# MKLab-ITI/gnn-tf

Measured on AMD Instinct MI355X. Metric: propagated edges/sec (APPNP K=10), higher is better.
Workload: dtype f32; 1 GPU; rmat_n80000000_nnz1000000000_C128_appnp_K10 (BASELINE config5); global_rows=80000000, stored_entries_total=1000000000, rows_per_rank=80000000, stored_entries_per_rank=1000000000, features=128, partition=none, kernel=spmm_group32

## Files before the change

gnn-tf_amd/csrc/gnx_gcnii.hip:

```cpp
#include "gnx_spmm_device.h"

namespace {

__device__ __forceinline__ uint64_t drop_stream(const DropFuse &f) { return f.stream + (f.offset ? *f.offset : 0); }

template <int VEC>
__device__ __forceinline__ void drop_values(const DropFuse &f, uint64_t stream, int64_t row, int64_t c, float (&x)[VEC]) {
#pragma unroll
    for (int v = 0; v < VEC; ++v)
        x[v] = (f.thr == 0 || hash_u24(f.seed, stream, (uint64_t)row, (uint64_t)(c + v), 0) >= f.thr) ? x[v] * f.scale : 0.f;
}

template <bool SPEC> struct SpectralArgs {};
template <> struct SpectralArgs<true> {
    const float *bias;
    uint32_t *gate;
};

template <bool EDGE> struct EdgeArgs {};
template <> struct EdgeArgs<true> {
    DropFuse feat;
};
template <bool EDGE>
__device__ __forceinline__ const DropFuse &feature_mask(const SpmmArgs &p, const EdgeArgs<EDGE> &ed) {
// ... 20 lines not shown
__device__ __forceinline__ void tile_times_Ms(float *__restrict__ T, const float *__restrict__ Ms, int lane, int act,
                                              const float *__restrict__ bias = nullptr) {
    constexpr int C = 16 * NT, STRIDE = C + 4;
    const int cc = lane & 15, g = lane >> 4;
    [[maybe_unused]] float bv[NT];
    if constexpr (BIAS) {
#pragma unroll
        for (int nt = 0; nt < NT; ++nt) bv[nt] = bias[16 * nt + cc];
    }
    f32x4 d[NT];
#pragma unroll
    for (int nt = 0; nt < NT; ++nt) d[nt] = f32x4{0.f, 0.f, 0.f, 0.f};
#pragma unroll 4
    for (int kk = 0; kk < C / 4; ++kk) {
        const float a = T[cc * STRIDE + 4 * kk + g];
        const float *__restrict__ mrow = Ms + (4 * kk + g) * STRIDE + cc;
#pragma unroll
        for (int nt = 0; nt < NT; ++nt) d[nt] = __builtin_amdgcn_mfma_f32_16x16x4f32(a, mrow[16 * nt], d[nt], 0, 0, 0);
    }
    __builtin_amdgcn_wave_barrier();
#pragma unroll
    for (int nt = 0; nt < NT; ++nt)
#pragma unroll
        for (int r = 0; r < 4; ++r) {
            float v = d[nt][r];
            if constexpr (BIAS) v += bv[nt];
            if (act == GNX_ACT_RELU) v = fmaxf(v, 0.f);
            T[(4 * g + r) * STRIDE + 16 * nt + cc] = v;
        }
    __builtin_amdgcn_wave_barrier();
}

template <bool ENTRIES, int G, int U>
__device__ __forceinline__ void edge_gather(const SpmmArgs &p, const float *__restrict__ Xc, int64_t row, int64_t beg, int64_t end,
                                            float (&acc)[4]) {
    static_assert(G % U == 0, "a round of G entries is whole batches of U");
    const int sub = (int)(threadIdx.x % G);
    for (int64_t base = beg; base < end; base += G) {
        int mycol = 0;
        float myw = 0.f;
        if (base + sub < end) {
            mycol = p.colidx[base + sub];
            myw = dropped_weight_at<ENTRIES>(p.fuse, p.vals[base + sub], base + sub, row, mycol);
        }
        const int n = (int)(end - base < G ? end - base : G);
        for (int k = 0; k < n; k += U) {
            float x[U][4];
            float w[U];
#pragma unroll
            for (int u = 0; u < U; ++u) {
                const int j = __shfl(mycol, k + u, G);
                w[u] = __shfl(myw, k + u, G);
                if (w[u] != 0.f) vload<4>(x[u], Xc + (int64_t)j * p.ldx);
                else {
#pragma unroll
                    for (int v = 0; v < 4; ++v) x[u][v] = 0.f;
                }
            }
#pragma unroll
            for (int u = 0; u < U; ++u)
#pragma unroll
                for (int v = 0; v < 4; ++v) acc[v] = fmaf(w[u], x[u][v], acc[v]);
        }
    }
}

template <typename R, int U, bool EDGE = false, bool ENTRIES = false, int G = 0>
__device__ __forceinline__ void mixed_row(const typename R::Args &p, int64_t row, int64_t beg, int64_t end, int c, float (&acc)[4]) {
    const typename R::Elem *__restrict__ Xc = R::X(p) + c;
    if constexpr (EDGE) {
        edge_gather<ENTRIES, G, U>(p, Xc, row, beg, end, acc);
    } else {
        for (int64_t e = beg; e < end; e += U) {
            float x[U][4];
            float w[U];
#pragma unroll
            for (int u = 0; u < U; ++u) {
                if (e + u < end) {
                    const int j = p.colidx[e + u];
                    w[u] = p.vals[e + u];
                    R::template load<4>(x[u], Xc + (int64_t)j * p.ldx);
                } else {
                    w[u] = 0.f;
#pragma unroll
                    for (int v = 0; v < 4; ++v) x[u][v] = 0.f;
                }
            }
#pragma unroll
            for (int u = 0; u < U; ++u)
#pragma unroll
                for (int v = 0; v < 4; ++v) acc[v] = fmaf(w[u], x[u][v], acc[v]);
        }
    }
    float h0[4];
    vload<4>(h0, p.H0 + row * p.ldh0 + c);
#pragma unroll
    for (int v = 0; v < 4; ++v) acc[v] = fmaf(acc[v], p.beta, h0[v] * p.alpha);
}

template <typename R, int NT, int U, int WPB, bool DROP = false, bool SPEC = false, bool EDGE = false, bool ENTRIES = false>
__global__ __launch_bounds__(64 * WPB) void k_spmm_gcnii(const typename R::Args p, const float *__restrict__ M, int64_t ldm, float *__restrict__ mixed,
                                                         const SpectralArgs<SPEC> sp = SpectralArgs<SPEC>{},
                                                         const EdgeArgs<EDGE> ed = EdgeArgs<EDGE>{}) {
    static_assert(!EDGE || (!SPEC && !R::BF16), "the edge-dropout form exists for the plain layer over f32 rows");
    constexpr int C = 16 * NT, G = 4 * NT, RPP = 64 / G, PASSES = 16 / RPP, STRIDE = C + 4;
    __shared__ float Ms[C * STRIDE];
    __shared__ float Ts[WPB][16 * STRIDE];
    const int lane = threadIdx.x & 63;
    const int wave = threadIdx.x >> 6;
    for (int idx = threadIdx.x; idx < C * C; idx += 64 * WPB) Ms[(idx / C) * STRIDE + idx % C] = M[(int64_t)(idx / C) * ldm + idx % C];
    __syncthreads();
    const int64_t tile = (int64_t)blockIdx.x * WPB + wave;
    if (tile * 16 >= p.n_rows) return;
    float *__restrict__ T = Ts[wave];
    const int sub = lane % G, c = sub * 4;
    int64_t rows[PASSES];
    bool live[PASSES];
#pragma unroll
    for (int ps = 0; ps < PASSES; ++ps) {
        const int rr = ps * RPP + lane / G;
        const int64_t slot = tile * 16 + rr;
        int64_t row = -1;
        int64_t beg = 0, end = 0;
        if (slot < p.n_rows) {
            row = p.row_order ? (int64_t)p.row_order[slot] : slot;
            beg = p.rowptr[row]; end = p.rowptr[row + 1];
        }
        live[ps] = row >= 0 && end - beg <= p.long_row;
        rows[ps] = row;
        float acc[4] = {0.f, 0.f, 0.f, 0.f};
        if (live[ps]) {
            mixed_row<R, U, EDGE, ENTRIES, G>(p, row, beg, end, c, acc);
            if (mixed) vstore<4>(mixed + row * (int64_t)C + c, acc);
        }
        vstore<4>(T + rr * STRIDE + c, acc);
    }
    __builtin_amdgcn_wave_barrier();
    if constexpr (SPEC) {
        constexpr int GW = G < 8 ? G : 8, WORDS = (C + 31) / 32;
        tile_times_Ms<NT, true>(T, Ms, lane, p.act, sp.bias);
        float b[4];
        vload<4>(b, sp.bias + c);
        uint64_t stream = 0;
        if constexpr (DROP) stream = drop_stream(p.fuse);
#pragma unroll
        for (int ps = 0; ps < PASSES; ++ps) {
            const int rr = ps * RPP + lane / G;
            float o[4];
            vload<4>(o, T + rr * STRIDE + c);
            uint32_t word = spectral_finish<4, DROP>(p.fuse, stream, rows[ps], c, b, o) << (c & 31);
#pragma unroll
            for (int m = 1; m < GW; m <<= 1) word |= (uint32_t)__shfl_xor((int)word, m);
            if (!live[ps]) continue;
            R::template store<4>(p, rows[ps] * p.ldo, c, o, false);
            if (sp.gate != nullptr && sub % GW == 0) sp.gate[rows[ps] * WORDS + (c >> 5)] = word;
        }
        return;
    }
    tile_times_Ms<NT>(T, Ms, lane, p.act);
#pragma unroll
    for (int ps = 0; ps < PASSES; ++ps) {
        if (!live[ps]) continue;
        const int rr = ps * RPP + lane / G;
        float o[4];
        vload<4>(o, T + rr * STRIDE + c);
        if constexpr (DROP) {
            const DropFuse &fd = feature_mask<EDGE>(p, ed);
            drop_values<4>(fd, drop_stream(fd), rows[ps], c, o);
        }
        R::template store<4>(p, rows[ps] * p.ldo, c, o, false);
    }
}

template <typename R, int NT, int U, int WPB, bool EDGE = false, bool ENTRIES = false>
__global__ __launch_bounds__(64 * WPB) void k_spmm_gcnii_back(const typename R::Args p, const float *__restrict__ N, int64_t ldn, const float *S_in,
                                                              float s_alpha, float *S_out) {
    static_assert(!EDGE || !R::BF16, "the edge-dropout form exists for f32 rows");
    constexpr int C = 16 * NT, G = 4 * NT, RPP = 64 / G, PASSES = 16 / RPP, STRIDE = C + 4;
    __shared__ float Ms[C * STRIDE];
    __shared__ float Ts[WPB][16 * STRIDE];
    const int lane = threadIdx.x & 63;
    const int wave = threadIdx.x >> 6;
    for (int idx = threadIdx.x; idx < C * C; idx += 64 * WPB) Ms[(idx / C) * STRIDE + idx % C] = N[(int64_t)(idx / C) * ldn + idx % C];
    __syncthreads();
    const int64_t tile = (int64_t)blockIdx.x * WPB + wave;
    if (tile * 16 >= p.n_rows) return;
    float *__restrict__ T = Ts[wave];
    const int sub = lane % G, c = sub * 4;
    int64_t rows[PASSES];
    bool live[PASSES];
#pragma unroll
    for (int ps = 0; ps < PASSES; ++ps) {
        const int rr = ps * RPP + lane / G;
        const int64_t slot = tile * 16 + rr;
        int64_t row = -1;
        int64_t beg = 0, end = 0;
        if (slot < p.n_rows) {
            row = p.row_order ? (int64_t)p.row_order[slot] : slot;
            beg = p.rowptr[row]; end = p.rowptr[row + 1];
        }
        live[ps] = row >= 0 && end - beg <= p.long_row;
        rows[ps] = row;
        float acc[4] = {0.f, 0.f, 0.f, 0.f};
        if (live[ps]) {
            const typename R::Elem *__restrict__ Xc;
            if constexpr (R::BF16) Xc = p.Xb + c;
            else Xc = p.X + c;
            if constexpr (EDGE) {
                edge_gather<ENTRIES, G, U>(p, Xc, row, beg, end, acc);
            } else {
                for (int64_t e = beg; e < end; e += U) {
                    float x[U][4];
                    float w[U];
#pragma unroll
                    for (int u = 0; u < U; ++u) {
                        if (e + u < end) {
                            const int j = p.colidx[e + u];
                            w[u] = p.vals[e + u];
                            if constexpr (R::BF16) bload<4>(x[u], Xc + (int64_t)j * p.ldx);
                            else vload<4>(x[u], Xc + (int64_t)j * p.ldx);
                        } else {
                            w[u] = 0.f;
#pragma unroll
                            for (int v = 0; v < 4; ++v) x[u][v] = 0.f;
                        }
                    }
#pragma unroll
                    for (int u = 0; u < U; ++u)
#pragma unroll
                        for (int v = 0; v < 4; ++v) acc[v] = fmaf(w[u], x[u][v], acc[v]);
                }
            }
#pragma unroll
            for (int v = 0; v < 4; ++v) acc[v] *= p.beta;
        }
        vstore<4>(T + rr * STRIDE + c, acc);
    }
    __builtin_amdgcn_wave_barrier();
    tile_times_Ms<NT>(T, Ms, lane, GNX_ACT_NONE);
#pragma unroll
    for (int ps = 0; ps < PASSES; ++ps) {
        if (!live[ps]) continue;
        const int rr = ps * RPP + lane / G;
        float o[4];
        vload<4>(o, T + rr * STRIDE + c);
        vstore<4>(p.out + rows[ps] * p.ldo + c, o);
    }
    if (S_out == nullptr) return;
    __builtin_amdgcn_wave_barrier();
#pragma unroll
    for (int ps = 0; ps < PASSES; ++ps) {
        const int rr = ps * RPP + lane / G;
        float x[4] = {0.f, 0.f, 0.f, 0.f};
        if (rows[ps] >= 0) {
            vload<4>(x, p.X + rows[ps] * p.ldx + c);
#pragma unroll
            for (int v = 0; v < 4; ++v) x[v] *= p.alpha;
        }
        vstore<4>(T + rr * STRIDE + c, x);
    }
    __builtin_amdgcn_wave_barrier();
    tile_times_Ms<NT>(T, Ms, lane, GNX_ACT_NONE);
#pragma unroll
    for (int ps = 0; ps < PASSES; ++ps) {
        if (rows[ps] < 0) continue;
        const int rr = ps * RPP + lane / G;
        const int64_t at = rows[ps] * (int64_t)C + c;
        float o[4];
        vload<4>(o, T + rr * STRIDE + c);
        if (S_in) {
            float s[4];
            vload<4>(s, S_in + at);
#pragma unroll
            for (int v = 0; v < 4; ++v) o[v] = fmaf(s_alpha, s[v], o[v]);
        }
        vstore<4>(S_out + at, o);
    }
}

template <typename R, int NT, int U, int WPB>
__global__ __launch_bounds__(64 * WPB) void k_gcnii_wgrad(const typename R::Args p, const float *__restrict__ Gm, const float *__restrict__ hub,
                                                          float *__restrict__ work) {
    constexpr int C = 16 * NT, G = 4 * NT, RPP = 64 / G, PASSES = 16 / RPP, STRIDE = C + 4;
    static_assert(WPB * 16 * STRIDE >= C * C, "the block's partial reuses the tiles");
    __shared__ __attribute__((aligned(16))) float Ts[WPB * 16 * STRIDE];
    const int lane = threadIdx.x & 63;
    const int wave = threadIdx.x >> 6;
    const int cc = lane & 15, g = lane >> 4, c = (lane % G) * 4;
    float *T = Ts + wave * 16 * STRIDE;
    f32x4 d[NT][NT];
#pragma unroll
    for (int mt = 0; mt < NT; ++mt)
#pragma unroll
        for (int nt = 0; nt < NT; ++nt) d[mt][nt] = f32x4{0.f, 0.f, 0.f, 0.f};
    const int64_t n_tiles = (p.n_rows + 15) / 16, step = (int64_t)gridDim.x * WPB;
    for (int64_t tile = (int64_t)blockIdx.x * WPB + wave; tile < n_tiles; tile += step) {
#pragma unroll
        for (int ps = 0; ps < PASSES; ++ps) {
            const int rr = ps * RPP + lane / G;
            const int64_t slot = tile * 16 + rr;
            float acc[4] = {0.f, 0.f, 0.f, 0.f};
            if (slot < p.n_rows) {
                const int64_t row = p.row_order ? (int64_t)p.row_order[slot] : slot;
                const int64_t beg = p.rowptr[row], end = p.rowptr[row + 1];
                if (end - beg <= p.long_row) mixed_row<R, U>(p, row, beg, end, c, acc);
                else vload<4>(acc, hub + row * (int64_t)C + c);
            }
            vstore<4>(T + rr * STRIDE + c, acc);
        }
        float b[4][NT];
#pragma unroll
        for (int kk = 0; kk < 4; ++kk) {
            const int64_t slot = tile * 16 + 4 * kk + g;
#pragma unroll
            for (int nt = 0; nt < NT; ++nt) b[kk][nt] = 0.f;
            if (slot < p.n_rows) {
                const int64_t row = p.row_order ? (int64_t)p.row_order[slot] : slot;
                vload<NT>(b[kk], Gm + row * (int64_t)C + NT * cc);
            }
        }
        __builtin_amdgcn_wave_barrier();
#pragma unroll
        for (int kk = 0; kk < 4; ++kk) {
// ... 721 lines not shown
```

gnn-tf_amd/csrc/gnx_graph.hip:

```cpp
#include <cstring>
#include <string.h>

#include "gnx_internal.h"
#include <algorithm>
#include <memory>
#include <type_traits>
#include <utility>

#include <rocprim/rocprim.hpp>

namespace gnx {

static thread_local char g_err[512] = "";

void set_error(const char *fmt, ...) {
    va_list ap;
    va_start(ap, fmt);
    vsnprintf(g_err, sizeof(g_err), fmt, ap);
    va_end(ap);
}

static unsigned bits_for(uint64_t max_key_exclusive) {
    unsigned b = 1;
    while (b < 64 && (max_key_exclusive >> b) != 0) ++b;
// ... 45 lines not shown
                                   int64_t *__restrict__ ptr) {
    int64_t r = (int64_t)blockIdx.x * blockDim.x + threadIdx.x;
    if (r > n_rows) return;
    int64_t lo = 0, hi = nnz;
    while (lo < hi) {
        int64_t mid = (lo + hi) >> 1;
        if ((int64_t)sorted_rows[mid] < r) lo = mid + 1; else hi = mid;
    }
    ptr[r] = lo;
}

__global__ void k_rows_from_ptr(const int64_t *__restrict__ rowptr, int64_t n_rows, int32_t *__restrict__ rowidx) {
    int64_t r = (int64_t)blockIdx.x * blockDim.x + threadIdx.x;
    if (r >= n_rows) return;
    for (int64_t e = rowptr[r]; e < rowptr[r + 1]; ++e) rowidx[e] = (int32_t)r;
}

__global__ void k_check_csr(const int64_t *__restrict__ rowptr, const int32_t *__restrict__ colidx, int64_t n_rows,
                            int64_t n_cols, int64_t nnz, int *__restrict__ bad) {
    int64_t r = (int64_t)blockIdx.x * blockDim.x + threadIdx.x;
    if (r >= n_rows) return;
    int64_t b = rowptr[r], e = rowptr[r + 1];
    if (b > e || b < 0 || e > nnz || (r == 0 && b != 0) || (r == n_rows - 1 && e != nnz)) { atomicExch(bad, 1); return; }
    for (int64_t k = b; k < e; ++k) {
        int32_t c = colidx[k];
        if (c < 0 || c >= n_cols || (k > b && colidx[k - 1] >= c)) { atomicExch(bad, 1); return; }
    }
}

__global__ void k_flag_long(const int64_t *__restrict__ rowptr, int64_t n_rows, int long_row, int long_chunk,
                            int32_t *__restrict__ flag, int64_t *__restrict__ cnt) {
    int64_t r = (int64_t)blockIdx.x * blockDim.x + threadIdx.x;
    if (r >= n_rows) return;
    int64_t d = rowptr[r + 1] - rowptr[r];
    bool lg = d > long_row;
    flag[r] = lg ? 1 : 0;
    cnt[r] = lg ? (d + long_chunk - 1) / long_chunk : 0;
}

__global__ void k_order_keys(const int64_t *__restrict__ rowptr, int64_t n_rows, int clamp, uint16_t *__restrict__ keys,
                             int32_t *__restrict__ ids) {
    int64_t r = (int64_t)blockIdx.x * blockDim.x + threadIdx.x;
    if (r >= n_rows) return;
    int64_t d = rowptr[r + 1] - rowptr[r];
    keys[r] = (uint16_t)(clamp - (d < clamp ? d : clamp));
    ids[r] = (int32_t)r;
}

__global__ void k_order_keys_windowed(const int64_t *__restrict__ rowptr, int64_t n_rows, int clamp, int64_t window, uint32_t n_windows,
                                      unsigned bin_bits, uint32_t *__restrict__ keys, int32_t *__restrict__ ids) {
    int64_t r = (int64_t)blockIdx.x * blockDim.x + threadIdx.x;
    if (r >= n_rows) return;
    int64_t d = rowptr[r + 1] - rowptr[r];
    const uint32_t w = d == 0 ? n_windows : (uint32_t)(r / window);
    keys[r] = (w << bin_bits) | (uint32_t)(clamp - (d < clamp ? d : clamp));
    ids[r] = (int32_t)r;
}

__global__ void k_slot_ptrs(const int64_t *__restrict__ rowptr, const int32_t *__restrict__ row_order, int64_t n_rows,
                            int64_t *__restrict__ slot_beg, int32_t *__restrict__ slot_cnt) {
    int64_t sidx = (int64_t)blockIdx.x * blockDim.x + threadIdx.x;
    if (sidx >= n_rows) return;
    const int64_t r = row_order[sidx], b = rowptr[r], e = rowptr[r + 1];
    slot_beg[sidx] = b;
    slot_cnt[sidx] = (int32_t)(e - b < 0x7fffffff ? e - b : 0x7fffffff);
}

__global__ void k_count_nonempty(const int64_t *__restrict__ rowptr, int64_t n_rows, unsigned long long *__restrict__ count) {
    int64_t r = (int64_t)blockIdx.x * blockDim.x + threadIdx.x;
    const bool has = r < n_rows && rowptr[r + 1] > rowptr[r];
    const unsigned long long votes = __popcll(__ballot(has));
    if ((threadIdx.x & 63) == 0 && votes) atomicAdd(count, votes);
}

__global__ void k_mark_referenced(const int32_t *__restrict__ colidx, int64_t nnz, uint8_t *__restrict__ flag) {
    int64_t k = (int64_t)blockIdx.x * blockDim.x + threadIdx.x;
    if (k < nnz) flag[colidx[k]] = 1;
}

__global__ void k_count_empty_referenced(const int64_t *__restrict__ rowptr, int64_t n, const uint8_t *__restrict__ flag, int *__restrict__ count) {
    int64_t r = (int64_t)blockIdx.x * blockDim.x + threadIdx.x;
    if (r < n && rowptr[r + 1] == rowptr[r] && flag[r]) atomicAdd(count, 1);
}

__global__ void k_fill_long(const int64_t *__restrict__ rowptr, int64_t n_rows, int long_row, int long_chunk,
                            const int32_t *__restrict__ pos,
                            const int64_t *__restrict__ cpos, int32_t *__restrict__ long_rows,
                            int64_t *__restrict__ long_chunk_ptr, int32_t *__restrict__ chunk_long) {
    int64_t r = (int64_t)blockIdx.x * blockDim.x + threadIdx.x;
    if (r >= n_rows) return;
    int64_t d = rowptr[r + 1] - rowptr[r];
    if (d <= long_row) return;
    const int32_t p = pos[r];
    const int64_t c0 = cpos[r];
    const int64_t nc = (d + long_chunk - 1) / long_chunk;
    long_rows[p] = (int32_t)r;
    long_chunk_ptr[p] = c0;
    for (int64_t c = 0; c < nc; ++c) chunk_long[c0 + c] = p;
}

__global__ void k_chunk_keys(const int64_t *__restrict__ rowptr, const int32_t *__restrict__ colidx,
                             const int32_t *__restrict__ long_rows, const int64_t *__restrict__ long_chunk_ptr,
                             const int32_t *__restrict__ chunk_long, int64_t n_chunks, int long_chunk,
                             uint32_t *__restrict__ keys, int32_t *__restrict__ ids) {
    int64_t c = (int64_t)blockIdx.x * blockDim.x + threadIdx.x;
    if (c >= n_chunks) return;
    const int32_t li = chunk_long[c];
    const int64_t beg = rowptr[long_rows[li]] + (c - long_chunk_ptr[li]) * long_chunk;
    keys[c] = (uint32_t)colidx[beg];
    ids[c] = (int32_t)c;
}

__global__ void k_make_tkeys(const int32_t *__restrict__ rowidx, const int32_t *__restrict__ colidx, int64_t nnz,
                             int64_t n_rows, uint64_t *__restrict__ keys, int32_t *__restrict__ payload) {
    int64_t k = (int64_t)blockIdx.x * blockDim.x + threadIdx.x;
    if (k >= nnz) return;
    keys[k] = (uint64_t)colidx[k] * (uint64_t)n_rows + (uint64_t)rowidx[k];
    payload[k] = (int32_t)k;
}

__global__ void k_invert_order(const int32_t *__restrict__ order, int64_t n, int32_t *__restrict__ newid) {
    int64_t i = (int64_t)blockIdx.x * blockDim.x + threadIdx.x;
    if (i < n) newid[order[i]] = (int32_t)i;
}

__global__ void k_make_rkeys(const int32_t *__restrict__ rowidx, const int32_t *__restrict__ colidx, const int32_t *__restrict__ newid,
                             int64_t nnz, int64_t n, uint64_t *__restrict__ keys, int32_t *__restrict__ payload) {
    int64_t k = (int64_t)blockIdx.x * blockDim.x + threadIdx.x;
    if (k >= nnz) return;
    keys[k] = (uint64_t)newid[rowidx[k]] * (uint64_t)n + (uint64_t)newid[colidx[k]];
    payload[k] = (int32_t)k;
}

__global__ void k_min_neighbour_rank(const int32_t *__restrict__ rowidx, const int32_t *__restrict__ colidx, const int32_t *__restrict__ rank,
                                     int64_t nnz, int32_t *__restrict__ key) {
    int64_t k = (int64_t)blockIdx.x * blockDim.x + threadIdx.x;
    if (k < nnz) atomicMin(&key[rowidx[k]], rank[colidx[k]]);
}

__global__ void k_relabel_keys(const int64_t *__restrict__ rowptr, const int32_t *__restrict__ key, int64_t n, int clamp,
                               uint64_t *__restrict__ keys, int32_t *__restrict__ ids) {
    int64_t r = (int64_t)blockIdx.x * blockDim.x + threadIdx.x;
    if (r >= n) return;
    const int64_t d = rowptr[r + 1] - rowptr[r];
    const uint64_t bin = (uint64_t)(clamp - (d < clamp ? d : clamp));
    keys[r] = (bin << 32) | (uint64_t)(uint32_t)key[r];
    ids[r] = (int32_t)r;
}

__global__ void k_gather_columns(const int32_t *__restrict__ colidx, const int32_t *__restrict__ rank, int64_t nnz,
                                 int32_t *__restrict__ gcol) {
    int64_t k = (int64_t)blockIdx.x * blockDim.x + threadIdx.x;
    if (k < nnz) gcol[k] = rank[colidx[k]];
}

__global__ void k_permute_vals(const float *__restrict__ vals, const int32_t *__restrict__ perm, int64_t n,
                               float *__restrict__ out) {
    int64_t k = (int64_t)blockIdx.x * blockDim.x + threadIdx.x;
    if (k < n) out[k] = vals[perm[k]];
}

__global__ void k_split_tkeys(const uint64_t *__restrict__ keys, int64_t nnz, int64_t n_rows,
                              int32_t *__restrict__ t_row , int32_t *__restrict__ t_col ) {
    int64_t k = (int64_t)blockIdx.x * blockDim.x + threadIdx.x;
    if (k >= nnz) return;
    t_row[k] = (int32_t)(keys[k] / (uint64_t)n_rows);
    t_col[k] = (int32_t)(keys[k] % (uint64_t)n_rows);
}

#define GNX_TRY(...)                                                                    \
    do {                                                                                \
        const int _rc = (__VA_ARGS__);                                                  \
        if (_rc != GNX_OK) return _rc;                                                  \
    } while (0)

template <class Call>
static int with_temporary(const char *what, Call call, hipStream_t s) {
    DevArray<char> tmp;
    size_t bytes = 0;
    hipError_t e = call(nullptr, bytes);
    if (e == hipSuccess) e = tmp.alloc(bytes);
    if (e == hipSuccess) e = call(tmp.get(), bytes);
    if (e == hipSuccess) e = hipStreamSynchronize(s);
    if (e != hipSuccess) {
        set_error("rocprim::%s failed: %s", what, hipGetErrorString(e));
        return GNX_ERR_HIP;
    }
    return GNX_OK;
}

template <class K, class V>
static int sort_pairs(K *keys_in, K *keys_out, V *vals_in, std::remove_const_t<V> *vals_out, int64_t n, unsigned end_bit, hipStream_t s) {
    return with_temporary("radix_sort_pairs", [&](void *tmp, size_t &bytes) {
        return rocprim::radix_sort_pairs(tmp, bytes, keys_in, keys_out, vals_in, vals_out, (size_t)n, 0u, end_bit, s);
    }, s);
}

static int sort_keys(int32_t *keys_in, int32_t *keys_out, int64_t n, unsigned end_bit, hipStream_t s) {
    return with_temporary("radix_sort_keys", [&](void *tmp, size_t &bytes) {
        return rocprim::radix_sort_keys(tmp, bytes, keys_in, keys_out, (size_t)n, 0u, end_bit, s);
    }, s);
}

template <class T>
static int exclusive_scan(T *in, T *out, int64_t n, hipStream_t s) {
    return with_temporary("exclusive_scan", [&](void *tmp, size_t &bytes) {
        return rocprim::exclusive_scan(tmp, bytes, in, out, (T)0, (size_t)n, rocprim::plus<T>(), s);
    }, s);
}

static int inclusive_scan(int32_t *in, int32_t *out, int64_t n, hipStream_t s) {
    return with_temporary("inclusive_scan", [&](void *tmp, size_t &bytes) {
        return rocprim::inclusive_scan(tmp, bytes, in, out, (size_t)n, rocprim::plus<int32_t>(), s);
    }, s);
}

template <class T>
static int fetch(T &host, const T *dev, hipStream_t s) {
    GNX_HIP(hipMemcpyAsync(&host, dev, sizeof(T), hipMemcpyDeviceToHost, s));
    GNX_HIP(hipStreamSynchronize(s));
    return GNX_OK;
}

template <class K, class MakeKeys>
static int order_rows(Csr &m, unsigned key_bits, MakeKeys make_keys, hipStream_t s) {
    DevArray<K> k0, k1;
    DevArray<int32_t> ids;
    GNX_HIP(k0.alloc(m.n_rows)); GNX_HIP(k1.alloc(m.n_rows)); GNX_HIP(ids.alloc(m.n_rows));
    GNX_HIP(m.row_order.alloc(m.n_rows));
    make_keys(k0.get(), ids.get());
    return sort_pairs<K, int32_t>(k0, k1, ids, m.row_order, m.n_rows, key_bits, s);
}

int build_long_plan(Csr &m, hipStream_t s) {
    m.n_long = 0; m.n_chunks = 0;
    const bool small = m.n_rows >= TINY_ROWS && m.n_rows < SMALL_ROWS;
    m.long_row = small ? SMALL_LONG_ROW : LONG_ROW;
    m.long_chunk = small ? SMALL_LONG_ROW : LONG_CHUNK;
    const int order_clamp = m.long_row < 65535 ? m.long_row : 65535;
    if (m.n_rows == 0) return GNX_OK;
    const dim3 row_blocks(blocks_for(m.n_rows)), threads(256);
    const unsigned bin_bits = bits_for((uint64_t)order_clamp + 1);
    if (m.order_window > 0) {
        const uint64_t n_windows = (uint64_t)((m.n_rows + m.order_window - 1) / m.order_window);
        const unsigned key_bits = bin_bits + bits_for(n_windows + 1);
        GNX_CHECK_ARG(key_bits <= 32, "row window: %lld windows of %lld rows do not fit the order key", (long long)n_windows,
                      (long long)m.order_window);
        GNX_TRY(order_rows<uint32_t>(m, key_bits, [&](uint32_t *keys, int32_t *ids) {
            hipLaunchKernelGGL(k_order_keys_windowed, row_blocks, threads, 0, s, m.rowptr, m.n_rows, order_clamp, m.order_window,
                               (uint32_t)n_windows, bin_bits, keys, ids);
        }, s));
    } else {
        GNX_TRY(order_rows<uint16_t>(m, bin_bits, [&](uint16_t *keys, int32_t *ids) {
            hipLaunchKernelGGL(k_order_keys, row_blocks, threads, 0, s, m.rowptr, m.n_rows, order_clamp, keys, ids);
        }, s));
    }
    if (m.n_rows >= SMALL_ROWS) {
        GNX_HIP(m.slot_beg.alloc(m.n_rows));
        GNX_HIP(m.slot_cnt.alloc(m.n_rows));
        hipLaunchKernelGGL(k_slot_ptrs, row_blocks, threads, 0, s, m.rowptr, m.row_order, m.n_rows, m.slot_beg, m.slot_cnt);
    }
    {
        DevArray<unsigned long long> count;
        GNX_HIP(count.alloc(1));
        GNX_HIP(hipMemsetAsync(count, 0, sizeof(unsigned long long), s));
        hipLaunchKernelGGL(k_count_nonempty, row_blocks, threads, 0, s, m.rowptr, m.n_rows, count);
        unsigned long long host = 0;
        GNX_TRY(fetch(host, count.get(), s));
        m.n_nonempty = (int64_t)host;
    }
    m.empty_rows_unreferenced = false;
    if (m.n_nonempty < m.n_rows) {
        if (m.n_nonempty > 0) {
            GNX_HIP(m.nonempty_rows.alloc(m.n_nonempty));
            GNX_TRY(sort_keys(m.row_order, m.nonempty_rows, m.n_nonempty, bits_for((uint64_t)m.n_rows), s));
        }
        if (m.n_rows == m.n_cols) {
            DevArray<uint8_t> flag;
            DevArray<int> count;
            GNX_HIP(flag.alloc(m.n_rows)); GNX_HIP(count.alloc(1));
            GNX_HIP(hipMemsetAsync(flag, 0, m.n_rows, s));
            GNX_HIP(hipMemsetAsync(count, 0, sizeof(int), s));
            if (m.nnz > 0) hipLaunchKernelGGL(k_mark_referenced, dim3(blocks_for(m.nnz)), threads, 0, s, m.colidx, m.nnz, flag);
            hipLaunchKernelGGL(k_count_empty_referenced, row_blocks, threads, 0, s, m.rowptr, m.n_rows, flag, count);
            int host_count = 1;
            GNX_TRY(fetch(host_count, count.get(), s));
            m.empty_rows_unreferenced = host_count == 0;
        }
    }
    if (m.nnz == 0) return GNX_OK;
    DevArray<int32_t> flag, pos;
    DevArray<int64_t> cnt, cpos;
    GNX_HIP(flag.alloc(m.n_rows));
    GNX_HIP(cnt.alloc(m.n_rows));
    GNX_HIP(pos.alloc(m.n_rows));
    GNX_HIP(cpos.alloc(m.n_rows));
    hipLaunchKernelGGL(k_flag_long, row_blocks, threads, 0, s, m.rowptr, m.n_rows, m.long_row, m.long_chunk, flag, cnt);
    GNX_TRY(exclusive_scan<int32_t>(flag, pos, m.n_rows, s));
    GNX_TRY(exclusive_scan<int64_t>(cnt, cpos, m.n_rows, s));
    int32_t last_flag = 0, last_pos = 0;
    int64_t last_cnt = 0, last_cpos = 0;
    GNX_TRY(fetch(last_flag, flag + (m.n_rows - 1), s));
    GNX_TRY(fetch(last_pos, pos + (m.n_rows - 1), s));
    GNX_TRY(fetch(last_cnt, cnt + (m.n_rows - 1), s));
    GNX_TRY(fetch(last_cpos, cpos + (m.n_rows - 1), s));
    m.n_long = (int64_t)last_flag + last_pos;
    m.n_chunks = last_cnt + last_cpos;
    if (m.n_long == 0) return GNX_OK;
    GNX_HIP(m.long_rows.alloc(m.n_long));
    GNX_HIP(m.long_chunk_ptr.alloc(m.n_long + 1));
    GNX_HIP(m.chunk_long.alloc(m.n_chunks));
    hipLaunchKernelGGL(k_fill_long, row_blocks, threads, 0, s, m.rowptr, m.n_rows, m.long_row, m.long_chunk, pos, cpos, m.long_rows,
                       m.long_chunk_ptr, m.chunk_long);
    GNX_HIP(hipMemcpyAsync(m.long_chunk_ptr + m.n_long, &m.n_chunks, 8, hipMemcpyHostToDevice, s));
    DevArray<uint32_t> k0, k1;
    DevArray<int32_t> ids;
    GNX_HIP(k0.alloc(m.n_chunks)); GNX_HIP(k1.alloc(m.n_chunks)); GNX_HIP(ids.alloc(m.n_chunks));
    GNX_HIP(m.chunk_order.alloc(m.n_chunks));
    hipLaunchKernelGGL(k_chunk_keys, dim3(blocks_for(m.n_chunks)), threads, 0, s, m.rowptr, m.colidx, m.long_rows, m.long_chunk_ptr,
                       m.chunk_long, m.n_chunks, m.long_chunk, k0, ids);
    return sort_pairs<uint32_t, int32_t>(k0, k1, ids, m.chunk_order, m.n_chunks, 32u, s);
}

bool stream_is_capturing(hipStream_t s) {
    hipStreamCaptureStatus st = hipStreamCaptureStatusNone;
    if (hipStreamIsCapturing(s, &st) != hipSuccess) { (void)hipGetLastError(); return false; }
    return st != hipStreamCaptureStatusNone;
}

#define GNX_NOT_WHILE_CAPTURING(s, what)                                                                                         \
    do {                                                                                                                         \
        if (stream_is_capturing(s)) {                                                                                            \
            set_error("%s would have to be allocated while the stream is being captured into a hipGraph: call "                  \
                      "gnx_graph_reserve(handle, C, flags) -- or run the same call once eagerly -- before the capture begins", what); \
            return GNX_ERR_UNSUPPORTED;                                                                                          \
        }                                                                                                                        \
    } while (0)

static int grow_slab(DevArray<float> &slab, size_t &held_bytes, size_t bytes) {
    held_bytes = 0;
    GNX_HIP(slab.alloc((bytes + sizeof(float) - 1) / sizeof(float)));
    held_bytes = bytes;
    return GNX_OK;
}

int ensure_partial(gnx_graph *g, size_t bytes, hipStream_t s) {
    if (bytes <= g->partial_bytes) return GNX_OK;
    GNX_NOT_WHILE_CAPTURING(s, "the long-row slab of this handle");
    return grow_slab(g->partial, g->partial_bytes, bytes);
}

int ensure_relabel_features(gnx_graph *g, size_t bytes, hipStream_t s) {
    if (bytes <= g->r_feat_bytes) return GNX_OK;
    GNX_NOT_WHILE_CAPTURING(s, "the feature scratch of this handle's relabelled copy");
    return grow_slab(g->r_feat, g->r_feat_bytes, bytes);
}

static void drop_transpose(gnx_graph *g) { static_cast<TransposedPart &>(*g) = TransposedPart(); }
static void drop_relabel(gnx_graph *g) { static_cast<RelabelledPart &>(*g) = RelabelledPart(); }
static void drop_gather_order(gnx_graph *g) { static_cast<GatherOrderPart &>(*g) = GatherOrderPart(); }

int ensure_transpose(gnx_graph *g, hipStream_t s) {
    if (g->has_t) return GNX_OK;
    GNX_NOT_WHILE_CAPTURING(s, "the transposed structure of this handle");
    const Csr &a = g->a;
    TransposedPart part;
    Csr &t = part.t;
    t.n_rows = a.n_cols; t.n_cols = a.n_rows; t.nnz = a.nnz;
    t.order_window = a.n_rows == a.n_cols ? a.order_window : 0;
    GNX_HIP(t.rowptr.alloc(t.n_rows + 1));
    GNX_HIP(t.colidx.alloc(t.nnz));
    GNX_HIP(part.t_perm.alloc(t.nnz));
    GNX_HIP(part.t_vals.alloc(t.nnz));
    GNX_HIP(part.t_raw.alloc(t.nnz));
    DevArray<uint64_t> k0, k1;
    DevArray<int32_t> p0;
    if (t.nnz == 0) {
        GNX_HIP(hipMemsetAsync(t.rowptr, 0, (t.n_rows + 1) * sizeof(int64_t), s));
    } else {
        const dim3 entry_blocks(blocks_for(t.nnz)), threads(256);
        GNX_HIP(k0.alloc(t.nnz)); GNX_HIP(k1.alloc(t.nnz));
        GNX_HIP(p0.alloc(t.nnz));
        GNX_HIP(part.t_rowidx.alloc(t.nnz));
        hipLaunchKernelGGL(k_make_tkeys, entry_blocks, threads, 0, s, g->rowidx, a.colidx, a.nnz, a.n_rows, k0, p0);
        GNX_TRY(sort_pairs<uint64_t, int32_t>(k0, k1, p0, part.t_perm, t.nnz, bits_for((uint64_t)a.n_rows * (uint64_t)a.n_cols), s));
        hipLaunchKernelGGL(k_split_tkeys, entry_blocks, threads, 0, s, k1, t.nnz, a.n_rows, part.t_rowidx, t.colidx);
        hipLaunchKernelGGL(k_lower_bound_rows, dim3(blocks_for(t.n_rows + 1)), threads, 0, s, part.t_rowidx, t.nnz, t.n_rows, t.rowptr);
        hipLaunchKernelGGL(k_permute_vals, entry_blocks, threads, 0, s, g->raw_vals, part.t_perm, t.nnz, part.t_raw);
    }
    GNX_HIP(hipStreamSynchronize(s));
    GNX_TRY(build_long_plan(t, s));
    part.has_t = true;
    static_cast<TransposedPart &>(*g) = std::move(part);
    return GNX_OK;
}

int ensure_gather_order(gnx_graph *g, hipStream_t s) {
    if (g->go_order) return GNX_OK;
    GNX_NOT_WHILE_CAPTURING(s, "the gather order of this handle");
    const Csr &a = g->a;
    GNX_CHECK_ARG(a.n_rows == a.n_cols && a.row_order != nullptr && a.n_rows > 0, "the gather order needs a non-empty square graph");
    const int64_t n = a.n_rows, nnz = a.nnz;
    const dim3 row_blocks(blocks_for(n)), threads(256);
    DevArray<int32_t> order, rank, key, ids;
    DevArray<uint64_t> k0, k1;
    GNX_HIP(order.alloc(n)); GNX_HIP(rank.alloc(n)); GNX_HIP(key.alloc(n)); GNX_HIP(ids.alloc(n));
    GNX_HIP(k0.alloc(n)); GNX_HIP(k1.alloc(n));
    hipLaunchKernelGGL(k_invert_order, row_blocks, threads, 0, s, a.row_order, n, rank);
    GNX_HIP(hipMemsetAsync(key, 0x7f, n * 4, s));
    if (nnz > 0)
        hipLaunchKernelGGL(k_min_neighbour_rank, dim3(blocks_for(nnz)), threads, 0, s, g->rowidx, a.colidx, rank, nnz, key);
    const int clamp = a.long_row < 65535 ? a.long_row : 65535;
    hipLaunchKernelGGL(k_relabel_keys, row_blocks, threads, 0, s, a.rowptr, key, n, clamp, k0, ids);
    GNX_TRY(sort_pairs<uint64_t, int32_t>(k0, k1, ids, order, n, 32u + bits_for((uint64_t)clamp + 1), s));
    hipLaunchKernelGGL(k_invert_order, row_blocks, threads, 0, s, order, n, rank);
    GNX_HIP(hipStreamSynchronize(s));
    GNX_HIP(hipGetLastError());
    g->go_order = std::move(order);
    g->go_rank = std::move(rank);
    return GNX_OK;
}

int ensure_relabel(gnx_graph *g, hipStream_t s) {
    if (g->has_r) return GNX_OK;
    GNX_NOT_WHILE_CAPTURING(s, "the relabelled copy of this handle");
    const Csr &a = g->a;
    GNX_CHECK_ARG(a.n_rows == a.n_cols && a.row_order != nullptr && a.nnz > 0, "relabelling needs a non-empty square graph");
    GNX_TRY(ensure_gather_order(g, s));
    const int64_t n = a.n_rows, nnz = a.nnz;
    const dim3 entry_blocks(blocks_for(nnz)), threads(256);
    RelabelledPart part;
    Csr &r = part.r;
    r.n_rows = n; r.n_cols = n; r.nnz = nnz;
    GNX_HIP(r.rowptr.alloc(n + 1));
    GNX_HIP(r.colidx.alloc(nnz));
    GNX_HIP(part.r_perm.alloc(nnz));
    GNX_HIP(part.r_vals.alloc(nnz));
    DevArray<uint64_t> k0, k1;
    DevArray<int32_t> p0, rrow;
    GNX_HIP(k0.alloc(nnz)); GNX_HIP(k1.alloc(nnz)); GNX_HIP(p0.alloc(nnz)); GNX_HIP(rrow.alloc(nnz));
    hipLaunchKernelGGL(k_make_rkeys, entry_blocks, threads, 0, s, g->rowidx, a.colidx, g->go_rank, nnz, n, k0, p0);
    GNX_TRY(sort_pairs<uint64_t, int32_t>(k0, k1, p0, part.r_perm, nnz, bits_for((uint64_t)n * (uint64_t)n), s));
    hipLaunchKernelGGL(k_split_tkeys, entry_blocks, threads, 0, s, k1, nnz, n, rrow, r.colidx);
    hipLaunchKernelGGL(k_lower_bound_rows, dim3(blocks_for(n + 1)), threads, 0, s, rrow, nnz, n, r.rowptr);
    GNX_HIP(hipStreamSynchronize(s));
    GNX_TRY(build_long_plan(r, s));
    part.has_r = true;
    static_cast<RelabelledPart &>(*g) = std::move(part);
    return GNX_OK;
}

int ensure_train_gather(gnx_graph *g, const char *fn, hipStream_t s) {
    if (g->blk_col_gid != nullptr) {
        set_error("%s: the handle is a vertex block (gnx_graph_set_block): the gather order exists for stand-alone graphs only", fn);
        return GNX_ERR_UNSUPPORTED;
    }
    if (g->has_dups) {
        set_error("%s: the graph holds duplicate COO entries: the gather order exists for handles without duplicates only", fn);
        return GNX_ERR_UNSUPPORTED;
    }
    if (g->a.order_window != 0) {
        set_error("%s: the handle has a row window (gnx_graph_set_row_window): its numbering carries locality already, the gather "
                  "order is not built", fn);
        return GNX_ERR_UNSUPPORTED;
    }
    GNX_CHECK_ARG(g->a.n_rows == g->a.n_cols, "%s: needs a square graph", fn);
    if (g->a_gcol != nullptr) return GNX_OK;
    if (g->a.n_rows == 0) return GNX_OK;
    GNX_NOT_WHILE_CAPTURING(s, "the gather-order columns of this handle (GNX_RESERVE_TRAIN_GATHER)");
    GNX_TRY(ensure_transpose(g, s));
    GNX_TRY(ensure_gather_order(g, s));
    const int64_t nnz = g->a.nnz;
    DevArray<int32_t> ac, tc;
    GNX_HIP(ac.alloc(nnz)); GNX_HIP(tc.alloc(nnz));
    if (nnz > 0) {
        hipLaunchKernelGGL(k_gather_columns, dim3(blocks_for(nnz)), dim3(256), 0, s, g->a.colidx, g->go_rank, nnz, ac);
        hipLaunchKernelGGL(k_gather_columns, dim3(blocks_for(nnz)), dim3(256), 0, s, g->t.colidx, g->go_rank, nnz, tc);
    }
    GNX_HIP(hipStreamSynchronize(s));
    GNX_HIP(hipGetLastError());
    g->t_gcol = std::move(tc);
    g->a_gcol = std::move(ac);
    return GNX_OK;
}

static int finish_graph(gnx_graph *g, hipStream_t s) {
    GNX_TRY(build_long_plan(g->a, s));
    GNX_HIP(hipGetLastError());
    return GNX_OK;
}

}

using namespace gnx;

extern "C" {

const char *gnx_last_error(void) { return g_err; }
int gnx_version(void) { return GNX_VERSION_NUM; }

int gnx_graph_destroy(gnx_graph_t g) {
    delete g;
    return GNX_OK;
}

int gnx_graph_reserve(gnx_graph_t g, int64_t C, int flags, void *stream) {
    GNX_CHECK_ARG(g != nullptr, "gnx_graph_reserve: NULL handle");
    GNX_CHECK_ARG(C >= 1 && (flags & ~(GNX_RESERVE_TRANSPOSED | GNX_RESERVE_K_LOOP | GNX_RESERVE_TRAIN_GATHER)) == 0,
                  "gnx_graph_reserve: bad width / flags");
    if (flags & GNX_RESERVE_TRAIN_GATHER) flags |= GNX_RESERVE_TRANSPOSED;
    hipStream_t s = (hipStream_t)stream;
    GNX_CHECK_ARG(!stream_is_capturing(s), "gnx_graph_reserve: the stream is being captured -- reserve before the capture begins");
    int64_t chunks = g->a.n_chunks;
    if (flags & GNX_RESERVE_TRANSPOSED) {
        GNX_TRY(ensure_transpose(g, s));
        chunks = std::max(chunks, g->t.n_chunks);
        if (!g->t_mask && !g->has_dups && g->t.nnz > 0)
            GNX_HIP(g->t_mask.alloc(g->t.nnz));
    }
    if ((flags & GNX_RESERVE_K_LOOP) && g->a.order_window == 0 && C <= RELABEL_MAX_C && g->a.n_rows == g->a.n_cols &&
        g->a.n_rows >= (1 << 20) && g->a.nnz >= g->a.n_rows) {
        GNX_TRY(ensure_relabel(g, s));
        GNX_TRY(ensure_relabel_features(g, (size_t)g->a.n_rows * (size_t)C * sizeof(float), s));
        chunks = std::max(chunks, g->r.n_chunks);
    }
    if (flags & GNX_RESERVE_TRAIN_GATHER) GNX_TRY(ensure_train_gather(g, "gnx_graph_reserve(GNX_RESERVE_TRAIN_GATHER)", s));
    if (chunks > 0) return ensure_partial(g, (size_t)chunks * (size_t)C * sizeof(float), s);
    return GNX_OK;
}

int gnx_graph_gather_order(gnx_graph_t g, const int32_t **d_order, const int32_t **d_rank) {
    GNX_CHECK_ARG(g != nullptr, "gnx_graph_gather_order: NULL handle");
    if (g->a.order_window != 0) {
        set_error("gnx_graph_gather_order: the handle has a row window (gnx_graph_set_row_window): the gather order is not built");
        return GNX_ERR_UNSUPPORTED;
    }
    GNX_TRY(ensure_gather_order(g, nullptr));
    if (d_order) *d_order = g->go_order;
    if (d_rank) *d_rank = g->go_rank;
    return GNX_OK;
}

int gnx_graph_set_row_window(gnx_graph_t g, int64_t window_rows, void *stream) {
    GNX_CHECK_ARG(g != nullptr, "gnx_graph_set_row_window: NULL handle");
    GNX_CHECK_ARG(window_rows >= 0, "gnx_graph_set_row_window: negative window");
    hipStream_t s = (hipStream_t)stream;
    GNX_CHECK_ARG(!stream_is_capturing(s), "gnx_graph_set_row_window: the stream is being captured -- set the window before the capture begins");
    if (g->a.order_window == window_rows) return GNX_OK;
    GNX_HIP(hipDeviceSynchronize());
    const int64_t before = g->a.order_window;
    g->a.drop_plan();
    g->a.order_window = window_rows;
    int rc = build_long_plan(g->a, s);
    if (rc != GNX_OK) {
        g->a.drop_plan();
        g->a.order_window = before;
        const int rc2 = build_long_plan(g->a, s);
        return rc2 != GNX_OK ? rc2 : rc;
    }
    if (g->has_t) {
        g->t.drop_plan();
        g->t.order_window = g->a.n_rows == g->a.n_cols ? window_rows : 0;
        rc = build_long_plan(g->t, s);
        if (rc != GNX_OK) {
            drop_transpose(g);
            return rc;
        }
    }
    if (g->has_r) drop_relabel(g);
    drop_gather_order(g);
    GNX_HIP(hipGetLastError());
    return GNX_OK;
}

int gnx_graph_create_coo(int64_t n_rows, int64_t n_cols, int64_t nnz, const int64_t *d_indices, const float *d_values,
                         void *stream, gnx_graph_t *out) {
    GNX_CHECK_ARG(out != nullptr, "gnx_graph_create_coo: out is NULL");
    *out = nullptr;
    GNX_CHECK_ARG(n_rows >= 0 && n_cols >= 0 && nnz >= 0, "gnx_graph_create_coo: negative size");
    GNX_CHECK_ARG(n_rows < INT32_MAX && n_cols < INT32_MAX, "gnx_graph_create_coo: more than 2^31-1 rows/cols per handle");
    GNX_CHECK_ARG(nnz < INT32_MAX, "gnx_graph_create_coo: more than 2^31-1 entries per handle");
    GNX_CHECK_ARG(nnz == 0 || (d_indices && d_values), "gnx_graph_create_coo: NULL indices/values");
    hipStream_t s = (hipStream_t)stream;
    std::unique_ptr<gnx_graph> g(new gnx_graph());
    Csr &a = g->a;
    a.n_rows = n_rows; a.n_cols = n_cols;
    g->nnz_entries = nnz;
    GNX_HIP(a.rowptr.alloc(n_rows + 1));
    if (nnz == 0) {
        a.nnz = 0;
        GNX_HIP(hipMemsetAsync(a.rowptr, 0, (n_rows + 1) * sizeof(int64_t), s));
        GNX_HIP(a.colidx.alloc(0));
        GNX_HIP(g->raw_vals.alloc(0));
        GNX_HIP(g->rowidx.alloc(0));
        GNX_HIP(hipStreamSynchronize(s));
        GNX_TRY(finish_graph(g.get(), s));
        *out = g.release();
        return GNX_OK;
    }
    const dim3 entry_blocks(blocks_for(nnz)), threads(256);
    DevArray<uint64_t> k0, k1;
    DevArray<float> v1;
    DevArray<int> bad;
    GNX_HIP(k0.alloc(nnz)); GNX_HIP(k1.alloc(nnz));
    GNX_HIP(v1.alloc(nnz));
    GNX_HIP(bad.alloc(1));
    GNX_HIP(hipMemsetAsync(bad, 0, 4, s));
    hipLaunchKernelGGL(k_make_keys, entry_blocks, threads, 0, s, d_indices, nnz, n_rows, n_cols, k0, bad);
    GNX_TRY(sort_pairs<uint64_t, const float>(k0, k1, d_values, v1, nnz, bits_for((uint64_t)n_rows * (uint64_t)n_cols), s));
    int32_t *d_head = reinterpret_cast<int32_t *>(k0.get());
    int32_t *d_scan = d_head + nnz;
    hipLaunchKernelGGL(k_heads, entry_blocks, threads, 0, s, k1, nnz, d_head);
    GNX_TRY(inclusive_scan(d_head, d_scan, nnz, s));
    int h_bad = 0; int32_t h_nslots = 0;
    GNX_TRY(fetch(h_bad, bad.get(), s));
    GNX_TRY(fetch(h_nslots, d_scan + (nnz - 1), s));
    GNX_CHECK_ARG(h_bad == 0, "gnx_graph_create_coo: an index lies outside the %lld x %lld shape", (long long)n_rows,
                  (long long)n_cols);
    a.nnz = h_nslots;
    g->has_dups = (a.nnz != nnz);
    GNX_HIP(a.colidx.alloc(a.nnz));
    GNX_HIP(g->rowidx.alloc(a.nnz));
    if (g->has_dups) GNX_HIP(g->slot_ptr.alloc(a.nnz + 1));
    hipLaunchKernelGGL(k_fill_slots, entry_blocks, threads, 0, s, k1, d_scan, nnz, n_cols, a.colidx, g->rowidx, g->slot_ptr);
    if (g->has_dups) {
        GNX_HIP(hipMemcpyAsync(g->slot_ptr + a.nnz, &nnz, 8, hipMemcpyHostToDevice, s));
        g->e_vals = std::move(v1);
        GNX_HIP(g->raw_vals.alloc(a.nnz));
        hipLaunchKernelGGL(k_sum_slots, dim3(blocks_for(a.nnz)), threads, 0, s, g->e_vals, g->slot_ptr, a.nnz, g->raw_vals);
    } else {
        g->raw_vals = std::move(v1);
    }
    hipLaunchKernelGGL(k_lower_bound_rows, dim3(blocks_for(n_rows + 1)), threads, 0, s, g->rowidx, a.nnz, n_rows, a.rowptr);
    GNX_HIP(hipStreamSynchronize(s));
    GNX_TRY(finish_graph(g.get(), s));
    *out = g.release();
    return GNX_OK;
}

int gnx_graph_create_csr(int64_t n_rows, int64_t n_cols, int64_t nnz, const int64_t *d_rowptr, const int32_t *d_colidx,
                         const float *d_values, void *stream, gnx_graph_t *out) {
    GNX_CHECK_ARG(out != nullptr, "gnx_graph_create_csr: out is NULL");
    *out = nullptr;
    GNX_CHECK_ARG(n_rows >= 0 && n_cols >= 0 && nnz >= 0, "gnx_graph_create_csr: negative size");
    GNX_CHECK_ARG(n_rows < INT32_MAX && n_cols < INT32_MAX && nnz < INT32_MAX, "gnx_graph_create_csr: size over 2^31-1");
    GNX_CHECK_ARG(d_rowptr && (nnz == 0 || (d_colidx && d_values)), "gnx_graph_create_csr: NULL array");
    hipStream_t s = (hipStream_t)stream;
    std::unique_ptr<gnx_graph> g(new gnx_graph());
    Csr &a = g->a;
    a.n_rows = n_rows; a.n_cols = n_cols; a.nnz = nnz; g->nnz_entries = nnz;
    GNX_HIP(a.rowptr.alloc(n_rows + 1));
    GNX_HIP(a.colidx.alloc(nnz));
    GNX_HIP(g->raw_vals.alloc(nnz));
    GNX_HIP(g->rowidx.alloc(nnz));
    GNX_HIP(hipMemcpyAsync(a.rowptr, d_rowptr, (n_rows + 1) * sizeof(int64_t), hipMemcpyDeviceToDevice, s));
    if (nnz) {
        GNX_HIP(hipMemcpyAsync(a.colidx, d_colidx, nnz * sizeof(int32_t), hipMemcpyDeviceToDevice, s));
        GNX_HIP(hipMemcpyAsync(g->raw_vals, d_values, nnz * sizeof(float), hipMemcpyDeviceToDevice, s));
    }
    DevArray<int> bad;
    GNX_HIP(bad.alloc(1));
    GNX_HIP(hipMemsetAsync(bad, 0, 4, s));
    if (n_rows) {
        hipLaunchKernelGGL(k_check_csr, dim3(blocks_for(n_rows)), dim3(256), 0, s, a.rowptr, a.colidx, n_rows, n_cols, nnz, bad);
        hipLaunchKernelGGL(k_rows_from_ptr, dim3(blocks_for(n_rows)), dim3(256), 0, s, a.rowptr, n_rows, g->rowidx);
    }
    int h_bad = 0;
    GNX_TRY(fetch(h_bad, bad.get(), s));
    GNX_CHECK_ARG(h_bad == 0, "gnx_graph_create_csr: rowptr/colidx are not a valid sorted CSR for this shape");
    GNX_TRY(finish_graph(g.get(), s));
    *out = g.release();
    return GNX_OK;
}

int gnx_graph_info(gnx_graph_t g, int64_t *n_rows, int64_t *n_cols, int64_t *nnz_entries, int64_t *nnz_coalesced) {
    GNX_CHECK_ARG(g != nullptr, "gnx_graph_info: NULL handle");
    if (n_rows) *n_rows = g->a.n_rows;
    if (n_cols) *n_cols = g->a.n_cols;
    if (nnz_entries) *nnz_entries = g->nnz_entries;
    if (nnz_coalesced) *nnz_coalesced = g->a.nnz;
    return GNX_OK;
}

int gnx_graph_hub_rows(gnx_graph_t g, int64_t *n_hub_rows, int64_t *threshold) {
    GNX_CHECK_ARG(g != nullptr, "gnx_graph_hub_rows: NULL handle");
    if (n_hub_rows) *n_hub_rows = g->a.n_long;
    if (threshold) *threshold = g->a.long_row;
    return GNX_OK;
}

int gnx_graph_csr(gnx_graph_t g, const int64_t **d_rowptr, const int32_t **d_colidx, const float **d_raw_values) {
    GNX_CHECK_ARG(g != nullptr, "gnx_graph_csr: NULL handle");
    if (d_rowptr) *d_rowptr = g->a.rowptr;
    if (d_colidx) *d_colidx = g->a.colidx;
    if (d_raw_values) *d_raw_values = g->raw_vals;
    return GNX_OK;
}

int gnx_graph_export(gnx_graph_t g, int64_t *d_rowptr_out, int32_t *d_colidx_out, float *d_raw_values_out,
                     int32_t *d_rowidx_out, void *stream) {
    GNX_CHECK_ARG(g != nullptr, "gnx_graph_export: NULL handle");
    hipStream_t s = (hipStream_t)stream;
    const Csr &a = g->a;
    if (d_rowptr_out) GNX_HIP(hipMemcpyAsync(d_rowptr_out, a.rowptr, (a.n_rows + 1) * sizeof(int64_t), hipMemcpyDeviceToDevice, s));
    if (a.nnz > 0) {
        if (d_colidx_out) GNX_HIP(hipMemcpyAsync(d_colidx_out, a.colidx, a.nnz * sizeof(int32_t), hipMemcpyDeviceToDevice, s));
        if (d_raw_values_out) GNX_HIP(hipMemcpyAsync(d_raw_values_out, g->raw_vals, a.nnz * sizeof(float), hipMemcpyDeviceToDevice, s));
        if (d_rowidx_out) GNX_HIP(hipMemcpyAsync(d_rowidx_out, g->rowidx, a.nnz * sizeof(int32_t), hipMemcpyDeviceToDevice, s));
    }
    return GNX_OK;
}

const char *gnx_graph_last_kernel(gnx_graph_t g) { return g ? g->last_kernel : ""; }

}
```

gnn-tf_amd/csrc/gnx_internal.h:

```cpp
#pragma once

#include <hip/hip_runtime.h>
#include <atomic>
#include <stdint.h>
#include <stdarg.h>
#include <stdio.h>

#include "../../include/gnx.h"

#define GNX_VERSION_NUM GNX_ABI_VERSION

namespace gnx {

void set_error(const char *fmt, ...);

#define GNX_HIP(expr)                                                                   \
    do {                                                                                \
        hipError_t _e = (expr);                                                         \
        if (_e != hipSuccess) {                                                         \
            gnx::set_error("%s failed: %s (%s:%d)", #expr, hipGetErrorString(_e), __FILE__, __LINE__); \
            return GNX_ERR_HIP;                                                         \
        }                                                                               \
    } while (0)

#define GNX_CHECK_ARG(cond, ...)                                                        \
    do {                                                                                \
        if (!(cond)) {                                                                  \
            gnx::set_error(__VA_ARGS__);                                                \
            return GNX_ERR_INVALID;                                                     \
        }                                                                               \
    } while (0)

#ifndef GNX_LONG_ROW
#define GNX_LONG_ROW 512
#endif
#ifndef GNX_LONG_CHUNK
#define GNX_LONG_CHUNK GNX_LONG_ROW
#endif
constexpr int LONG_ROW = GNX_LONG_ROW;
constexpr int LONG_CHUNK = GNX_LONG_CHUNK;
constexpr int SMALL_ROWS = 1 << 20;
constexpr int TINY_ROWS = 1 << 15;
constexpr int RELABEL_MAX_C = 16;
constexpr int SMALL_LONG_ROW = GNX_LONG_ROW < 128 ? GNX_LONG_ROW : 128;

template <class T>
struct DevArray {
    DevArray() = default;
    DevArray(DevArray &&o) noexcept : p(o.release()) {}
    DevArray &operator=(DevArray &&o) noexcept {
        if (this != &o) { reset(); p = o.release(); }
        return *this;
    }
    ~DevArray() { reset(); }
    hipError_t alloc(size_t count) {
        reset();
        const size_t bytes = count * sizeof(T);
        const hipError_t e = hipMalloc((void **)&p, bytes < 16 ? 16 : bytes);
        if (e != hipSuccess) p = nullptr;
        return e;
    }
    void reset() {
        if (p) (void)hipFree(p);
        p = nullptr;
    }
    T *release() { T *q = p; p = nullptr; return q; }
    T *get() const { return p; }
    operator T *() const { return p; }
private:
    T *p = nullptr;
};

struct Plan {
    int64_t n_long = 0, n_chunks = 0;
    int long_row = LONG_ROW, long_chunk = LONG_CHUNK;
    DevArray<int32_t> long_rows;
    DevArray<int64_t> long_chunk_ptr;
    DevArray<int32_t> chunk_long;
    DevArray<int32_t> chunk_order;
    DevArray<int32_t> row_order;
    DevArray<int64_t> slot_beg;
    DevArray<int32_t> slot_cnt;
    int64_t n_nonempty = 0;
    DevArray<int32_t> nonempty_rows;
    bool empty_rows_unreferenced = false;
};

struct Csr : Plan {
    int64_t n_rows = 0, n_cols = 0, nnz = 0;
    DevArray<int64_t> rowptr;
    DevArray<int32_t> colidx;
    int64_t order_window = 0;
    void drop_plan() { static_cast<Plan &>(*this) = Plan(); }
};


struct TransposedPart {
    bool has_t = false;
    Csr t;
    DevArray<int32_t> t_perm;
    DevArray<float> t_vals;
    DevArray<float> t_raw;
    DevArray<int32_t> t_rowidx;
    DevArray<uint16_t> t_mask;
};

struct RelabelledPart {
    bool has_r = false;
    Csr r;
    DevArray<int32_t> r_perm;
    DevArray<float> r_vals;
};

struct GatherOrderPart {
    DevArray<int32_t> go_order;
    DevArray<int32_t> go_rank;
    DevArray<int32_t> a_gcol;
    DevArray<int32_t> t_gcol;
};

}

struct gnx_graph : gnx::TransposedPart, gnx::RelabelledPart, gnx::GatherOrderPart {
    gnx::Csr a;
    gnx::DevArray<float> raw_vals;
    gnx::DevArray<int32_t> rowidx;
    int64_t nnz_entries = 0;
    bool has_dups = false;
    gnx::DevArray<float> e_vals;
    gnx::DevArray<int64_t> slot_ptr;
    bool entry_drop = false;
    gnx::DevArray<uint8_t> ed_mult, t_ed_mult;
    gnx::DevArray<float> ed_vals, t_ed_vals;
    gnx::DevArray<float> partial;
    size_t partial_bytes = 0;
    gnx::DevArray<float> deg;
    const uint64_t *stream_offset = nullptr;
    int64_t blk_row0_global = 0, blk_row0_buf = 0;
    gnx::DevArray<int32_t> blk_col_gid;
    gnx::DevArray<float> r_feat;
    size_t r_feat_bytes = 0;
    const char *last_kernel = "";
};

namespace gnx {

int build_long_plan(Csr &m, hipStream_t s);
int ensure_transpose(gnx_graph *g, hipStream_t s);
int ensure_partial(gnx_graph *g, size_t bytes, hipStream_t s);
bool stream_is_capturing(hipStream_t s);
int ensure_relabel(gnx_graph *g, hipStream_t s);
int ensure_gather_order(gnx_graph *g, hipStream_t s);
int ensure_train_gather(gnx_graph *g, const char *fn, hipStream_t s);
int ensure_relabel_features(gnx_graph *g, size_t bytes, hipStream_t s);

inline unsigned blocks_for(int64_t n, int per_block = 256) { return (unsigned)((n + per_block - 1) / per_block); }

inline uint32_t drop_threshold(double p) { return (uint32_t)(p * 16777216.0); }
inline float drop_scale(float p) { return 1.0f / (1.0f - p); }

__device__ __forceinline__ uint64_t rng_fin(uint64_t z) {
    z ^= z >> 30; z *= 0xBF58476D1CE4E5B9ull;
    z ^= z >> 27; z *= 0x94D049BB133111EBull;
    z ^= z >> 31;
    return z;
}
__device__ __forceinline__ uint64_t hash_key(uint64_t seed, uint64_t stream, uint64_t row, uint64_t col) {
    const uint64_t k = seed ^ (stream * 0xD1342543DE82EF95ull);
    uint64_t x = rng_fin(k + row * 0x9E3779B97F4A7C15ull);
    return x ^ (col * 0xC2B2AE3D27D4EB4Full);
}
__device__ __forceinline__ uint32_t hash_rank(uint64_t key, uint64_t dup) {
    return (uint32_t)(rng_fin(key + dup * 0x165667B19E3779F9ull) >> 40);
}
__device__ __forceinline__ uint32_t hash_u24(uint64_t seed, uint64_t stream, uint64_t row, uint64_t col, uint64_t dup) {
    return hash_rank(hash_key(seed, stream, row, col), dup);
}

__device__ __forceinline__ float kept_term(float acc, float value, float scale) {
#pragma clang fp contract(off)
    const float term = value * scale;
    return acc + term;
}

constexpr uint32_t ENTRY_GENERAL = 255;

__device__ __forceinline__ float slot_kept_sum(uint64_t key, uint32_t thr, float scale, uint32_t m, float uval,
                                               const float *__restrict__ e_vals, const int64_t *__restrict__ slot_ptr, int64_t slot) {
    float acc = 0.f;
    if (m != ENTRY_GENERAL) {
        for (uint32_t i = 0; i < m; ++i)
            if (hash_rank(key, i) >= thr) acc = kept_term(acc, uval, scale);
    } else {
        const int64_t b = slot_ptr[slot], e = slot_ptr[slot + 1];
        for (int64_t i = b; i < e; ++i)
            if (hash_rank(key, (uint64_t)(i - b)) >= thr) acc = kept_term(acc, e_vals[i], scale);
    }
    return acc;
}

struct DropFuse {
    const float *D;
    uint64_t seed, stream;
    const uint64_t *offset;
    uint32_t thr;
    float scale;
    int transposed;
    int col_prescaled;
    int64_t row0_key, row0_D;
    const int32_t *gid;
    const uint8_t *mult;
    const float *e_vals;
    const int64_t *slot_ptr;
    const int32_t *perm;
};

__device__ __forceinline__ float dropped_weight(const DropFuse &f, float raw, int64_t r, int64_t c) {
    const int64_t ar = f.transposed ? c : r, ac = f.transposed ? r : c;
    const uint64_t stream = f.stream + (f.offset ? *f.offset : 0);
    const uint64_t kc = f.gid ? (uint64_t)f.gid[ac] : (uint64_t)ac;
    if (hash_u24(f.seed, stream, (uint64_t)(ar + f.row0_key), kc, 0) < f.thr) return 0.f;
    if (f.col_prescaled && f.transposed)
        return (raw * f.scale) * f.D[ac];
    const float w = f.D[ar + f.row0_D] * (raw * f.scale);
    return f.col_prescaled ? w : w * f.D[ac];
}

__device__ __forceinline__ float dropped_weight_entries(const DropFuse &f, float uval, int64_t pos, int64_t r, int64_t c) {
    const int64_t ar = f.transposed ? c : r, ac = f.transposed ? r : c;
    const uint64_t stream = f.stream + (f.offset ? *f.offset : 0);
    const uint64_t kc = f.gid ? (uint64_t)f.gid[ac] : (uint64_t)ac;
    const uint32_t m = f.mult[pos];
    const int64_t slot = (m == ENTRY_GENERAL && f.perm) ? (int64_t)f.perm[pos] : pos;
    const float v = slot_kept_sum(hash_key(f.seed, stream, (uint64_t)(ar + f.row0_key), kc), f.thr, f.scale, m, uval, f.e_vals,
                                  f.slot_ptr, slot);
    if (v == 0.f) return 0.f;
    if (f.col_prescaled && f.transposed) return v * f.D[ac];
    const float w = f.D[ar + f.row0_D] * v;
    return f.col_prescaled ? w : w * f.D[ac];
}

template <bool ENTRIES>
__device__ __forceinline__ float dropped_weight_at(const DropFuse &f, float raw, int64_t pos, int64_t r, int64_t c) {
    if constexpr (ENTRIES) return dropped_weight_entries(f, raw, pos, r, c);
    else return dropped_weight(f, raw, r, c);
}

struct SpmmArgs {
    const int64_t *rowptr;
    const int32_t *colidx;
    const float *vals;
    const float *diag;
    const float *X;
    int64_t ldx;
    const float *H0;
    int64_t ldh0;
    float beta, alpha;
    int act;
    float *out;
    int64_t ldo;
    const int32_t *out_rows;
    bool map_h0;
    const float *out_scale;
    float *out2;
    int64_t ldo2;
    float beta2;
    const float *out2_scale;
    int64_t n_rows;
    int64_t n_nonempty;
    int64_t slot0;
    int C;
    const int32_t *long_rows;
    const int64_t *long_chunk_ptr;
    const int32_t *chunk_long;
    const int32_t *chunk_order;
    const int32_t *row_order;
    const int64_t *slot_beg;
    const int32_t *slot_cnt;
    const int32_t *nonempty_rows;
    const int32_t *row_list;
    float *partial;
    int64_t n_long, n_chunks;
    int long_row, long_chunk;
    int tune;
    bool skip_empty;
    int64_t xcd_rows;
    uint32_t xcd_chunk;
    DropFuse fuse;
};

struct PerDeviceOnce {
    std::atomic<uint64_t> done{0};
    static int device() { int d = 0; if (hipGetDevice(&d) != hipSuccess) { (void)hipGetLastError(); d = -1; } return d; }
    bool need(int dev) const { return dev < 0 || dev >= 64 || !((done.load(std::memory_order_acquire) >> dev) & 1u); }
    void set(int dev) { if (dev >= 0 && dev < 64) done.fetch_or(uint64_t(1) << dev, std::memory_order_release); }
};

int launch_spmm(gnx_graph *g, const Csr &m, SpmmArgs &p, hipStream_t s);
void launch_long_rows(const SpmmArgs &p, hipStream_t s);
int launch_spmm_bf16_f32_order(gnx_graph *g, const Csr &m, const SpmmArgs &p, const uint16_t *Xb, float *out, hipStream_t s);
void launch_long_rows_bf16(const SpmmArgs &p, const uint16_t *Xb, float *out, hipStream_t s);
const char *launch_spmm_dropped(const SpmmArgs &p, int vec, hipStream_t s);
void launch_long_rows_dropped(const SpmmArgs &p, hipStream_t s);
int refuse_duplicates(const gnx_graph *g, const char *fn);
void set_values(const gnx_graph *g, bool transposed, SpmmArgs &p);
void set_drop_fuse(const gnx_graph *g, float dropout_p, uint64_t seed, uint64_t stream_id, const float *d_D, int transposed,
                   int x_prescaled, SpmmArgs &p);
// ... 9 lines not shown
```

gnn-tf_amd/csrc/gnx_spmm.hip:

```cpp
#include "gnx_spmm_eval.h"

namespace {

__global__ void k_gather_vals(const float *__restrict__ vals, const int32_t *__restrict__ perm, int64_t n,
                              float *__restrict__ out) {
    const int64_t k = (int64_t)blockIdx.x * blockDim.x + threadIdx.x;
    if (k < n) out[k] = vals[perm[k]];
}

__global__ __launch_bounds__(256) void k_gather_rows32(const float *__restrict__ X, int64_t ldx, const int32_t *__restrict__ idx, int64_t n_idx,
                                                        int C, float *__restrict__ out, int64_t ldo) {
    const int64_t total = n_idx * C, stride = (int64_t)gridDim.x * blockDim.x;
    for (int64_t e = (int64_t)blockIdx.x * blockDim.x + threadIdx.x; e < total; e += stride) {
        const int64_t r = e / C;
        const int c = (int)(e % C);
        out[r * ldo + c] = X[(int64_t)idx[r] * ldx + c];
    }
}

}

namespace gnx {

#ifdef GNX_TUNING
int tune_override = -1;
#endif

int launch_spmm(gnx_graph *g, const Csr &m, SpmmArgs &p, hipStream_t s) {
    return launch_bound(g, m, p, s, [&](SpmmArgs &q) {
#ifdef GNX_TUNING
        static const int tune = [] { const char *e = getenv("GNX_TUNE"); return e ? atoi(e) : 0; }();
        q.tune = tune_override >= 0 ? tune_override : tune;
        if (q.tune & 16384) q.ldx = 0;
#endif
        return q.fuse.D != nullptr ? launch_spmm_dropped(q, F32Rows::vec(q), s) : launch_eval<F32Rows>(q, s);
    });
}

void launch_long_rows(const SpmmArgs &p, hipStream_t s) {
    with_vec<F32Rows>(F32Rows::vec(p), [&](auto V) { launch_long<F32Rows, V()>(p, s); });
}

}

extern "C" {

#ifdef GNX_TUNING
int gnx_debug_set_tune(int t) { tune_override = t; return 0; }
#endif

int gnx_spmm(gnx_graph_t g, const float *d_vals, const float *d_diag, const float *d_X, int64_t ldx, int64_t C,
             const float *d_H0, int64_t ldh0, float beta, float alpha, int act, float *d_out, int64_t ldo, void *stream) {
    int rc = check_common("gnx_spmm", g, d_X, ldx, C, d_H0, ldh0, d_out, ldo);
    if (rc != GNX_OK) return rc;
    GNX_CHECK_ARG((act & ~GNX_ACT_SKIP_EMPTY) == GNX_ACT_NONE || (act & ~GNX_ACT_SKIP_EMPTY) == GNX_ACT_RELU, "gnx_spmm: invalid activation %d", act);
    GNX_CHECK_ARG(d_diag == nullptr || g->a.n_rows == g->a.n_cols, "gnx_spmm: diag needs a square graph");
    SpmmArgs p{};
    p.vals = d_vals ? d_vals : g->raw_vals;
    p.diag = d_diag;
    set_operands<F32Rows>(p, d_X, ldx, d_H0, ldh0, beta, alpha, act, d_out, 0, ldo, C);
    return launch_spmm(g, g->a, p, (hipStream_t)stream);
}

int gnx_spmm_t(gnx_graph_t g, const float *d_vals, const float *d_diag, const float *d_X, int64_t ldx, int64_t C,
               const float *d_H0, int64_t ldh0, float beta, float alpha, int act, float *d_out, int64_t ldo, void *stream) {
    int rc = check_common("gnx_spmm_t", g, d_X, ldx, C, d_H0, ldh0, d_out, ldo);
    if (rc != GNX_OK) return rc;
    GNX_CHECK_ARG(act == GNX_ACT_NONE || act == GNX_ACT_RELU, "gnx_spmm_t: invalid activation %d", act);
    GNX_CHECK_ARG(d_diag == nullptr || g->a.n_rows == g->a.n_cols, "gnx_spmm_t: diag needs a square graph");
    hipStream_t s = (hipStream_t)stream;
    rc = ensure_transpose(g, s);
    if (rc != GNX_OK) return rc;
    const float *src = d_vals ? d_vals : g->raw_vals;
    if (g->a.nnz > 0)
        hipLaunchKernelGGL(k_gather_vals, dim3(blocks_for(g->a.nnz, 256)), dim3(256), 0, s, src, g->t_perm, g->a.nnz, g->t_vals);
    SpmmArgs p{};
    p.vals = g->t_vals;
    p.diag = d_diag;
    set_operands<F32Rows>(p, d_X, ldx, d_H0, ldh0, beta, alpha, act, d_out, 0, ldo, C);
    return launch_spmm(g, g->t, p, s);
}

int gnx_spmm_scatter(gnx_graph_t g, const float *d_vals, const float *d_diag, const float *d_X, int64_t ldx, int64_t C,
                     const float *d_H0, int64_t ldh0, float beta, float alpha, int act, const int32_t *d_out_rows,
                     float *d_out, int64_t ldo, void *stream) {
    int rc = check_common("gnx_spmm_scatter", g, d_X, ldx, C, d_H0, ldh0, d_out, ldo);
    if (rc != GNX_OK) return rc;
    GNX_CHECK_ARG(act == GNX_ACT_NONE || act == GNX_ACT_RELU, "gnx_spmm_scatter: invalid activation %d", act);
    GNX_CHECK_ARG(d_diag == nullptr || g->a.n_rows == g->a.n_cols, "gnx_spmm_scatter: diag needs a square graph");
    SpmmArgs p{};
    p.vals = d_vals ? d_vals : g->raw_vals;
    p.diag = d_diag; p.out_rows = d_out_rows;
    set_operands<F32Rows>(p, d_X, ldx, d_H0, ldh0, beta, alpha, act, d_out, 0, ldo, C);
    return launch_spmm(g, g->a, p, (hipStream_t)stream);
}

int gnx_spmm_rows(gnx_graph_t g, const float *d_vals, const float *d_X, int64_t ldx, int64_t C, const float *d_H0, int64_t ldh0,
                  float beta, float alpha, int act, const int32_t *d_rows, float *d_out, int64_t ldo, void *stream) {
    int rc = check_common("gnx_spmm_rows", g, d_X, ldx, C, d_H0, ldh0, d_out, ldo);
    if (rc != GNX_OK) return rc;
    GNX_CHECK_ARG((act & ~GNX_ACT_SKIP_EMPTY) == GNX_ACT_NONE || (act & ~GNX_ACT_SKIP_EMPTY) == GNX_ACT_RELU, "gnx_spmm_rows: invalid activation %d", act);
    GNX_CHECK_ARG(d_rows != nullptr || g->a.n_rows == 0, "gnx_spmm_rows: NULL row map");
    SpmmArgs p{};
    p.vals = d_vals ? d_vals : g->raw_vals;
    p.out_rows = d_rows; p.map_h0 = true;
    set_operands<F32Rows>(p, d_X, ldx, d_H0, ldh0, beta, alpha, act, d_out, 0, ldo, C);
    return launch_spmm(g, g->a, p, (hipStream_t)stream);
}

int gnx_graph_permute_values_t(gnx_graph_t g, const float *d_vals, float *d_vals_t_out, void *stream) {
    GNX_CHECK_ARG(g != nullptr, "gnx_graph_permute_values_t: NULL handle");
    hipStream_t s = (hipStream_t)stream;
    int rc = ensure_transpose(g, s);
    if (rc != GNX_OK) return rc;
    if (g->a.nnz == 0) return GNX_OK;
    GNX_CHECK_ARG(d_vals_t_out != nullptr, "gnx_graph_permute_values_t: NULL output");
    hipLaunchKernelGGL(k_gather_vals, dim3(blocks_for(g->a.nnz, 256)), dim3(256), 0, s, d_vals ? d_vals : g->raw_vals, g->t_perm,
                       g->a.nnz, d_vals_t_out);
    GNX_HIP(hipGetLastError());
    return GNX_OK;
}

int gnx_spmm_tv(gnx_graph_t g, const float *d_vals_t, const float *d_diag, const float *d_X, int64_t ldx, int64_t C,
                const float *d_H0, int64_t ldh0, float beta, float alpha, int act, float *d_out, int64_t ldo, void *stream) {
    int rc = check_common("gnx_spmm_tv", g, d_X, ldx, C, d_H0, ldh0, d_out, ldo);
    if (rc != GNX_OK) return rc;
    GNX_CHECK_ARG(act == GNX_ACT_NONE || act == GNX_ACT_RELU, "gnx_spmm_tv: invalid activation %d", act);
    GNX_CHECK_ARG(d_diag == nullptr || g->a.n_rows == g->a.n_cols, "gnx_spmm_tv: diag needs a square graph");
    GNX_CHECK_ARG(g->a.nnz == 0 || d_vals_t != nullptr, "gnx_spmm_tv: NULL values");
    hipStream_t s = (hipStream_t)stream;
    rc = ensure_transpose(g, s);
    if (rc != GNX_OK) return rc;
    SpmmArgs p{};
    p.vals = d_vals_t;
    p.diag = d_diag;
    set_operands<F32Rows>(p, d_X, ldx, d_H0, ldh0, beta, alpha, act, d_out, 0, ldo, C);
    return launch_spmm(g, g->t, p, s);
}

int gnx_ppr_step(gnx_graph_t g, const float *d_vals, const float *d_diag, const float *d_H, const float *d_H0, float a,
                 int64_t C, int act, float *d_out, void *stream) {
    GNX_CHECK_ARG(d_H0 != nullptr, "gnx_ppr_step: NULL H0");
    return gnx_spmm(g, d_vals, d_diag, d_H, C, C, d_H0, C, (float)(1.0 - (double)a), a, act, d_out, C, stream);
}

int gnx_appnp_propagate(gnx_graph_t g, const float *d_vals, const float *d_diag, const float *d_H0, float a, int K,
                        int64_t C, float *d_out, float *d_work, void *stream) {
    return gnx_appnp_propagate_act(g, d_vals, d_diag, d_H0, a, K, C, GNX_ACT_NONE, d_out, d_work, stream);
}

int gnx_appnp_propagate_act(gnx_graph_t g, const float *d_vals, const float *d_diag, const float *d_H0, float a, int K,
                            int64_t C, int act, float *d_out, float *d_work, void *stream) {
    GNX_CHECK_ARG(g != nullptr, "gnx_appnp_propagate: NULL handle");
    GNX_CHECK_ARG(act == GNX_ACT_NONE || act == GNX_ACT_RELU, "gnx_appnp_propagate: invalid activation %d", act);
    GNX_CHECK_ARG(K >= 0, "gnx_appnp_propagate: negative iteration count");
    GNX_CHECK_ARG(g->a.n_rows == g->a.n_cols, "gnx_appnp_propagate: needs a square graph");
    GNX_CHECK_ARG(d_H0 && d_out && (K < 2 || d_work), "gnx_appnp_propagate: NULL buffer");
    GNX_CHECK_ARG(d_out != d_H0 && d_work != d_H0 && d_out != d_work, "gnx_appnp_propagate: H0, out and work must be distinct");
    if (K == 0) {
        GNX_HIP(hipMemcpyAsync(d_out, d_H0, (size_t)g->a.n_rows * C * sizeof(float), hipMemcpyDeviceToDevice, (hipStream_t)stream));
        return GNX_OK;
    }
    const int64_t n = g->a.n_rows;
    hipStream_t s = (hipStream_t)stream;
    if (C <= RELABEL_MAX_C && n >= (1 << 20) && g->a.nnz >= n && d_diag == nullptr && g->a.order_window == 0) {
        int rc = ensure_relabel(g, s);
        if (rc != GNX_OK) return rc;
        rc = ensure_relabel_features(g, (size_t)n * C * sizeof(float), s);
        if (rc != GNX_OK) return rc;
        hipLaunchKernelGGL(k_gather_vals, dim3(blocks_for(g->a.nnz, 256)), dim3(256), 0, s, d_vals ? d_vals : g->raw_vals, g->r_perm, g->a.nnz,
                           g->r_vals);
        GNX_HIP(hipGetLastError());
        hipLaunchKernelGGL(k_gather_rows32, dim3((unsigned)std::min<int64_t>(blocks_for(n * C, 256), 1 << 22)), dim3(256), 0, s, d_H0, C,
                           g->go_order, n, (int)C, g->r_feat, C);
        GNX_HIP(hipGetLastError());
        const float *src = g->r_feat;
        for (int k = 0; k < K; ++k) {
            const bool last = k == K - 1;
            float *dst = last ? d_out : (((K - 2 - k) % 2 == 0) ? d_work : d_out);
            SpmmArgs p{};
            p.vals = g->r_vals;
            const int act_k = (!last && (k >= 2 || g->r.empty_rows_unreferenced)) ? (act | GNX_ACT_SKIP_EMPTY) : act;
            set_operands<F32Rows>(p, src, C, g->r_feat, C, (float)(1.0 - (double)a), a, act_k, dst, 0, C, C);
            p.out_rows = last ? g->go_order : nullptr;
            rc = launch_spmm(g, g->r, p, s);
            if (rc != GNX_OK) return rc;
            src = dst;
// ... 17 lines not shown
```

gnn-tf_amd/csrc/gnx_spmm_device.h:

```cpp
#pragma once
#include <stdlib.h>
#include <algorithm>
#include <type_traits>

#include "gnx_internal.h"

using namespace gnx;

namespace {

template <int VEC> struct VecT;
template <> struct VecT<1> { using type = float; };
template <> struct VecT<2> { using type = float2; };
template <> struct VecT<4> { using type = float4; };

template <int VEC>
__device__ __forceinline__ void vload(float (&x)[VEC], const float *__restrict__ p) {
    if constexpr (VEC == 8) {
        vload<4>(*reinterpret_cast<float(*)[4]>(&x[0]), p);
        vload<4>(*reinterpret_cast<float(*)[4]>(&x[4]), p + 4);
    } else {
        using T = typename VecT<VEC>::type;
        const T v = *reinterpret_cast<const T *>(p);
        __builtin_memcpy(x, &v, sizeof(T));
    }
}
template <int VEC>
__device__ __forceinline__ void vstore(float *__restrict__ p, const float (&x)[VEC]) {
    if constexpr (VEC == 8) {
        vstore<4>(p, *reinterpret_cast<const float(*)[4]>(&x[0]));
        vstore<4>(p + 4, *reinterpret_cast<const float(*)[4]>(&x[4]));
    } else {
        using T = typename VecT<VEC>::type;
        T v;
        __builtin_memcpy(&v, x, sizeof(T));
        *reinterpret_cast<T *>(p) = v;
    }
}

typedef float f32x4 __attribute__((ext_vector_type(4)));
typedef float f32x2 __attribute__((ext_vector_type(2)));
template <int VEC> struct NatT;
template <> struct NatT<1> { using type = float; };
template <> struct NatT<2> { using type = f32x2; };
template <> struct NatT<4> { using type = f32x4; };

template <int VEC>
__device__ __forceinline__ void vload_nt(float (&x)[VEC], const float *__restrict__ p) {
    if constexpr (VEC == 8) {
        vload_nt<4>(*reinterpret_cast<float(*)[4]>(&x[0]), p);
        vload_nt<4>(*reinterpret_cast<float(*)[4]>(&x[4]), p + 4);
    } else {
        using T = typename NatT<VEC>::type;
        const T v = __builtin_nontemporal_load(reinterpret_cast<const T *>(p));
        __builtin_memcpy(x, &v, sizeof(T));
    }
}
template <int VEC>
__device__ __forceinline__ void vstore_nt(float *__restrict__ p, const float (&x)[VEC]) {
    if constexpr (VEC == 8) {
        vstore_nt<4>(p, *reinterpret_cast<const float(*)[4]>(&x[0]));
        vstore_nt<4>(p + 4, *reinterpret_cast<const float(*)[4]>(&x[4]));
    } else {
        using T = typename NatT<VEC>::type;
        T v;
        __builtin_memcpy(&v, x, sizeof(T));
        __builtin_nontemporal_store(v, reinterpret_cast<T *>(p));
    }
}

template <int VEC> struct BfRaw;
template <> struct BfRaw<1> { using type = uint16_t; };
template <> struct BfRaw<2> { using type = uint32_t; };
template <> struct BfRaw<4> { using type = uint2; };
template <> struct BfRaw<8> { using type = uint4; };

template <int VEC>
__device__ __forceinline__ void bload(float (&x)[VEC], const uint16_t *__restrict__ p) {
    if constexpr (VEC == 1) {
        x[0] = __uint_as_float((uint32_t)*p << 16);
    } else {
        using T = typename BfRaw<VEC>::type;
        const T v = *reinterpret_cast<const T *>(p);
        uint32_t w[VEC / 2];
        __builtin_memcpy(w, &v, sizeof(T));
#pragma unroll
        for (int i = 0; i < VEC / 2; ++i) {
            x[2 * i] = __uint_as_float(w[i] << 16);
            x[2 * i + 1] = __uint_as_float(w[i] & 0xFFFF0000u);
        }
    }
}

__device__ __forceinline__ uint16_t to_bf16(float x) { return __builtin_bit_cast(uint16_t, (__bf16)x); }

template <int VEC>
__device__ __forceinline__ void bstore(uint16_t *__restrict__ p, const float (&x)[VEC]) {
    uint16_t h[VEC];
#pragma unroll
    for (int v = 0; v < VEC; ++v) h[v] = to_bf16(x[v]);
    using T = typename BfRaw<VEC>::type;
    T t;
    __builtin_memcpy(&t, h, sizeof(T));
    *reinterpret_cast<T *>(p) = t;
}

inline bool aligned(const void *p, size_t a) { return p == nullptr || ((uintptr_t)p % a) == 0; }

[[maybe_unused]] int pick_vec(const SpmmArgs &p, int max_vec, const void *X, size_t x_size, const void *out, size_t out_size, const void *out2,
             size_t out2_size) {
    for (int vec = max_vec; vec > 1; vec >>= 1) {
        if (p.C % vec == 0 && p.ldx % vec == 0 && p.ldo % vec == 0 && (p.H0 == nullptr || p.ldh0 % vec == 0) &&
            (out2 == nullptr || p.ldo2 % vec == 0) && aligned(X, std::min<size_t>(x_size * vec, 16)) &&
            aligned(out, std::min<size_t>(out_size * vec, 16)) && aligned(p.H0, std::min<size_t>(4 * vec, 16)) &&
            aligned(out2, std::min<size_t>(out2_size * vec, 16)))
            return vec;
    }
    return 1;
}

struct F32Rows {
    using Args = SpmmArgs;
    using Elem = float;
    using Out = float;
    using Out2 = float;
    static constexpr int MAX_VEC = 4;
    static constexpr bool EXPERIMENTS = true;
    static constexpr int BF16 = 0;
    static constexpr bool NAMES_LONG = false;
    static constexpr bool GATHER_ORDER = false;
    __device__ static const float *X(const Args &p) { return p.X; }
    template <int VEC>
    __device__ static void load(float (&x)[VEC], const float *__restrict__ q) { vload<VEC>(x, q); }
    __device__ static const float *diag(const Args &p) { return p.diag; }
    __device__ static const int32_t *out_rows(const Args &p) { return p.out_rows; }
    __device__ static bool has_out2(const Args &p) { return p.out2 != nullptr; }
    __device__ static const float *out_scale(const Args &p) { return p.out_scale; }
    template <int VEC>
    __device__ static void store(const Args &p, int64_t at, int c, const float (&o)[VEC], bool nt) {
        if (nt) vstore_nt<VEC>(p.out + at + c, o);
        else vstore<VEC>(p.out + at + c, o);
    }
    template <int VEC>
    __device__ static void store2(const Args &p, int64_t at, int c, const float (&o)[VEC]) { vstore<VEC>(p.out2 + at + c, o); }
    static int vec(const Args &p) { return pick_vec(p, MAX_VEC, p.X, 4, p.out, 4, nullptr, 0); }
    static void bind_X(Args &p, const float *X) { p.X = X; }
    static void bind_out(Args &p, float *out, int ) { p.out = out; }
    static void bind_out2(Args &p, float *out2) { p.out2 = out2; }
};

struct OrdArgs : SpmmArgs {
    const int32_t *gcol;
    const int32_t *out2_rows;
};

struct F32RowsOrd : F32Rows {
    using Args = OrdArgs;
    static constexpr bool EXPERIMENTS = false;
    static constexpr bool NAMES_LONG = true;
    static constexpr bool GATHER_ORDER = true;
};

struct BfArgs : SpmmArgs {
    const uint16_t *Xb;
    void *outv;
    int out_bf16;
    uint16_t *out2b;
};

template <bool TRAIN>
struct Bf16RowsT {
    using Args = BfArgs;
    using Elem = uint16_t;
    using Out = void;
    using Out2 = uint16_t;
    static constexpr int MAX_VEC = 8;
    static constexpr bool EXPERIMENTS = false;
    static constexpr int BF16 = 1;
    static constexpr bool NAMES_LONG = true;
    static constexpr bool GATHER_ORDER = false;
    __device__ static const uint16_t *X(const Args &p) { return p.Xb; }
    template <int VEC>
    __device__ static void load(float (&x)[VEC], const uint16_t *__restrict__ q) { bload<VEC>(x, q); }
    __device__ static const float *diag(const Args &p) { return TRAIN ? nullptr : p.diag; }
    __device__ static const int32_t *out_rows(const Args &p) { return TRAIN ? nullptr : p.out_rows; }
    __device__ static bool has_out2(const Args &p) { return TRAIN && p.out2b != nullptr; }
    __device__ static const float *out_scale(const Args &p) { return TRAIN ? p.out_scale : nullptr; }
    template <int VEC>
    __device__ static void store(const Args &p, int64_t at, int c, const float (&o)[VEC], bool) {
        if (p.out_bf16) bstore<VEC>(static_cast<uint16_t *>(p.outv) + at + c, o);
        else vstore<VEC>(static_cast<float *>(p.outv) + at + c, o);
    }
    template <int VEC>
    __device__ static void store2(const Args &p, int64_t at, int c, const float (&o)[VEC]) { bstore<VEC>(p.out2b + at + c, o); }
    static int vec(const Args &p) { return pick_vec(p, MAX_VEC, p.Xb, 2, p.outv, p.out_bf16 ? 2 : 4, p.out2b, 2); }
    static void bind_X(Args &p, const uint16_t *X) { p.Xb = X; }
    static void bind_out(Args &p, void *out, int out_bf16) { p.outv = out; p.out_bf16 = out_bf16; }
    static void bind_out2(Args &p, uint16_t *out2) { p.out2b = out2; }
};

__device__ __forceinline__ int readlane_i(int v, int lane) { return __builtin_amdgcn_readlane(v, lane); }
__device__ __forceinline__ float readlane_f(float v, int lane) {
    return __int_as_float(__builtin_amdgcn_readlane(__float_as_int(v), lane));
}

template <typename R>
__device__ __forceinline__ const int32_t *gather_cols(const typename R::Args &p) {
    if constexpr (R::GATHER_ORDER) return p.gcol ? p.gcol : p.colidx;
    else return nullptr;
}

template <typename R, int VEC, int U, bool FUSE = false, bool ENTRIES = false, bool GCOL = false>
__device__ __forceinline__ void wave_accumulate(const int32_t *__restrict__ colidx, const float *__restrict__ vals,
                                                const typename R::Elem *__restrict__ X, int64_t ldx, int64_t beg, int64_t end,
                                                int c, int lane, float (&acc)[VEC], bool nt_index = false,
                                                const DropFuse *fuse = nullptr, int64_t row = 0,
                                                const int32_t *__restrict__ gcol = nullptr) {
    for (int64_t base = beg; base < end; base += 64) {
        const int n = (int)((end - base) < 64 ? (end - base) : 64);
        int mycol = 0;
        [[maybe_unused]] int mygcol = 0;
        float myval = 0.f;
        if (lane < n) {
            if (nt_index) {
                mycol = __builtin_nontemporal_load(colidx + base + lane);
                myval = __builtin_nontemporal_load(vals + base + lane);
            } else {
                mycol = colidx[base + lane];
                myval = vals[base + lane];
            }
            if constexpr (GCOL) mygcol = gcol[base + lane];
            if (FUSE) myval = dropped_weight_at<ENTRIES>(*fuse, myval, base + lane, row, mycol);
        }
        int i = 0;
        if (FUSE) {
            uint64_t keep = __ballot(myval != 0.f);
            while (keep) {
                float x[U][VEC];
                int idx[U];
#pragma unroll
                for (int u = 0; u < U; ++u) {
                    idx[u] = keep ? (int)__builtin_ctzll(keep) : -1;
                    if (keep) keep &= keep - 1;
                    if (idx[u] >= 0) {
                        int j;
                        if constexpr (GCOL) j = readlane_i(mygcol, idx[u]);
                        else j = readlane_i(mycol, idx[u]);
                        R::template load<VEC>(x[u], X + (int64_t)j * ldx + c);
                    }
                }
#pragma unroll
                for (int u = 0; u < U; ++u) {
                    if (idx[u] >= 0) {
                        const float w = readlane_f(myval, idx[u]);
#pragma unroll
                        for (int v = 0; v < VEC; ++v) acc[v] = fmaf(w, x[u][v], acc[v]);
                    }
                }
            }
            continue;
        }
        for (; i + U <= n; i += U) {
            float x[U][VEC];
#pragma unroll
            for (int u = 0; u < U; ++u) {
                const int j = readlane_i(mycol, i + u);
                R::template load<VEC>(x[u], X + (int64_t)j * ldx + c);
            }
#pragma unroll
            for (int u = 0; u < U; ++u) {
                const float w = readlane_f(myval, i + u);
#pragma unroll
                for (int v = 0; v < VEC; ++v) acc[v] = fmaf(w, x[u][v], acc[v]);
            }
        }
        if (i < n) {
            float x[U][VEC];
#pragma unroll
            for (int u = 0; u < U - 1; ++u) {
                if (i + u < n) {
                    const int j = readlane_i(mycol, i + u);
                    R::template load<VEC>(x[u], X + (int64_t)j * ldx + c);
                }
            }
#pragma unroll
            for (int u = 0; u < U - 1; ++u) {
                if (i + u < n) {
                    const float w = readlane_f(myval, i + u);
#pragma unroll
                    for (int v = 0; v < VEC; ++v) acc[v] = fmaf(w, x[u][v], acc[v]);
                }
            }
        }
    }
}

template <typename R, int VEC>
__device__ __forceinline__ void epilogue_store(const typename R::Args &p, int64_t row, int c, bool active, float (&acc)[VEC],
                                               bool nt = false) {
    if (!active) return;
    if (R::diag(p)) {
        const float d = R::diag(p)[row];
        float xr[VEC];
        R::template load<VEC>(xr, R::X(p) + row * p.ldx + c);
#pragma unroll
        for (int v = 0; v < VEC; ++v) acc[v] = fmaf(d, xr[v], acc[v]);
    }
    if (R::has_out2(p)) {
        const float f2 = p.out2_scale ? p.out2_scale[row] : 1.f;
        float o2[VEC];
#pragma unroll
        for (int v = 0; v < VEC; ++v) o2[v] = (acc[v] * p.beta2) * f2;
        int64_t row2 = row;
        if constexpr (R::GATHER_ORDER) {
            if (p.out2_rows) row2 = (int64_t)p.out2_rows[row];
        }
        R::template store2<VEC>(p, row2 * p.ldo2, c, o2);
    }
    float o[VEC];
    const int64_t orow = R::out_rows(p) ? (int64_t)R::out_rows(p)[row] : row;
    if (p.H0) {
        const int64_t hrow = p.map_h0 ? orow : row;
        float h0[VEC];
        if (nt) vload_nt<VEC>(h0, p.H0 + hrow * p.ldh0 + c);
        else vload<VEC>(h0, p.H0 + hrow * p.ldh0 + c);
#pragma unroll
        for (int v = 0; v < VEC; ++v) o[v] = fmaf(acc[v], p.beta, h0[v] * p.alpha);
    } else {
#pragma unroll
        for (int v = 0; v < VEC; ++v) o[v] = acc[v] * p.beta;
    }
    if (p.act == GNX_ACT_RELU) {
#pragma unroll
        for (int v = 0; v < VEC; ++v) o[v] = fmaxf(o[v], 0.f);
    }
    if (R::out_scale(p)) {
        const float os = R::out_scale(p)[row];
#pragma unroll
        for (int v = 0; v < VEC; ++v) o[v] *= os;
    }
    R::template store<VEC>(p, orow * p.ldo, c, o, nt);
}

__device__ __forceinline__ int64_t xcd_block(const SpmmArgs &p) {
    const uint32_t b = blockIdx.x;
    if (p.xcd_rows <= 0) return (int64_t)b;
    const uint32_t x = b & 7u, i = b >> 3, ch = p.xcd_chunk;
    return ((int64_t)(i / ch) * 8 + x) * ch + i % ch;
}

struct RowSpan { int64_t row, beg, end; };
template <bool WAVE>
__device__ __forceinline__ RowSpan slot_row(const SpmmArgs &p, int64_t slot, bool degree_order = false) {
    if (WAVE) {
        const int64_t row = p.row_list ? (int64_t)__builtin_amdgcn_readfirstlane(p.row_list[slot])
                                       : (degree_order ? (int64_t)__builtin_amdgcn_readfirstlane(p.row_order[slot]) : slot);
        return {row, p.rowptr[row], p.rowptr[row + 1]};
    }
    const int64_t row = p.row_order ? (int64_t)p.row_order[slot] : slot;
    if (p.slot_beg) { const int64_t beg = p.slot_beg[slot]; return {row, beg, beg + p.slot_cnt[slot]}; }
    return {row, p.rowptr[row], p.rowptr[row + 1]};
}

struct ChunkSpan { int64_t chunk, row, beg, end; };
__device__ __forceinline__ ChunkSpan slot_chunk(const SpmmArgs &p, int64_t cslot) {
    const int64_t chunk = p.chunk_order ? (int64_t)p.chunk_order[cslot] : cslot;
    const int32_t li = p.chunk_long[chunk];
    const int64_t row = p.long_rows[li];
    const int64_t beg = p.rowptr[row] + (chunk - p.long_chunk_ptr[li]) * p.long_chunk;
    const int64_t rend = p.rowptr[row + 1];
    return {chunk, row, beg, beg + p.long_chunk < rend ? beg + p.long_chunk : rend};
}

template <typename R, int VEC>
__global__ __launch_bounds__(256) void k_spmm_long_reduce(const typename R::Args p) {
    const int lane = threadIdx.x & 63;
    const int wib = __builtin_amdgcn_readfirstlane((int)(threadIdx.x >> 6));
    const int64_t li = (int64_t)blockIdx.x * 4 + wib;
    if (li >= p.n_long) return;
    const int64_t row = p.long_rows[li];
    const int64_t cb = p.long_chunk_ptr[li], ce = p.long_chunk_ptr[li + 1];
    for (int c0 = 0; c0 < p.C; c0 += 64 * VEC) {
        const int c = c0 + lane * VEC;
        const bool active = c < p.C;
        float acc[VEC];
#pragma unroll
        for (int v = 0; v < VEC; ++v) acc[v] = 0.f;
        if (active) {
            for (int64_t k = cb; k < ce; ++k) {
                float x[VEC];
                vload<VEC>(x, p.partial + k * (int64_t)p.C + c);
#pragma unroll
                for (int v = 0; v < VEC; ++v) acc[v] += x[v];
            }
        }
        epilogue_store<R, VEC>(p, row, c, active, acc);
    }
}

#define GNX_LAUNCH(kern, grid, ...) hipLaunchKernelGGL(kern, dim3(grid), dim3(256), 0, s, __VA_ARGS__)

template <typename Args, typename Kern>
void launch_row_pieces(Kern kern, const Args &p, int rows_per_block, int threads, hipStream_t s) {
    const int64_t per_launch = (((int64_t)1 << 31) / threads) * rows_per_block;
    for (int64_t r0 = 0; r0 < p.n_rows; r0 += per_launch) {
        Args q = p;
        q.slot0 = r0;
        const int64_t rows = p.n_rows - r0 < per_launch ? p.n_rows - r0 : per_launch;
        q.n_rows = r0 + rows;
        unsigned grid = blocks_for(rows, rows_per_block);
        if (q.xcd_rows > 0 && rows < 64 * q.xcd_rows) q.xcd_rows = 0;
        if (q.xcd_rows > 0) {
            q.xcd_chunk = (uint32_t)((q.xcd_rows + rows_per_block - 1) / rows_per_block);
            const unsigned span = 8u * q.xcd_chunk;
            grid = (grid + span - 1) / span * span;
        }
        hipLaunchKernelGGL(kern, dim3(grid), dim3(threads), 0, s, q);
    }
}
#define GNX_ROW_PIECES(kern, rows_per_block, threads) launch_row_pieces(kern, p, rows_per_block, threads, s)

[[maybe_unused]] int bind_csr(gnx_graph *g, const Csr &m, SpmmArgs &p, hipStream_t s) {
    p.rowptr = m.rowptr; p.colidx = m.colidx; p.n_rows = m.n_rows; p.n_nonempty = m.n_nonempty; p.nonempty_rows = m.nonempty_rows; p.row_list = nullptr;
    p.slot_beg = m.slot_beg; p.slot_cnt = m.slot_cnt;
    p.long_rows = m.long_rows; p.long_chunk_ptr = m.long_chunk_ptr; p.chunk_long = m.chunk_long;
    p.row_order = m.row_order;
    p.xcd_rows = m.order_window;
    p.chunk_order = m.chunk_order;
    p.tune = 0;
    p.n_long = m.n_long; p.n_chunks = m.n_chunks; p.long_row = m.long_row; p.long_chunk = m.long_chunk;
    p.partial = nullptr;
    p.skip_empty = (p.act & GNX_ACT_SKIP_EMPTY) != 0 && p.diag == nullptr;
    p.act &= ~GNX_ACT_SKIP_EMPTY;
    if (m.n_rows > 0 && m.n_long > 0) {
        int rc = ensure_partial(g, (size_t)m.n_chunks * (size_t)p.C * sizeof(float), s);
        if (rc != GNX_OK) return rc;
        p.partial = g->partial;
    }
    return GNX_OK;
}

template <typename Args, typename Pick>
int launch_bound(gnx_graph *g, const Csr &m, Args &p, hipStream_t s, Pick pick) {
    int rc = bind_csr(g, m, p, s);
    if (rc != GNX_OK) return rc;
    if (m.n_rows == 0) return GNX_OK;
    g->last_kernel = pick(p);
    GNX_HIP(hipGetLastError());
    return GNX_OK;
}

[[maybe_unused]] void trim_empty_rows(SpmmArgs &p, int lanes) {
    if (!p.skip_empty || p.n_nonempty >= p.n_rows) return;
    if (lanes <= 32 && p.row_order != nullptr) p.n_rows = p.n_nonempty;
    else if (lanes > 32 && p.nonempty_rows != nullptr) { p.row_list = p.nonempty_rows; p.n_rows = p.n_nonempty; }
}

template <int N> using IntC = std::integral_constant<int, N>;

template <typename R, typename F>
auto with_vec(int vec, F &&f) {
    if constexpr (R::MAX_VEC == 8) {
        if (vec == 8) return f(IntC<8>{});
    }
    if (vec == 4) return f(IntC<4>{});
    if (vec == 2) return f(IntC<2>{});
    return f(IntC<1>{});
}

enum RowClass { ROWS_NONE, ROWS_WAVE, ROWS_G32, ROWS_G16, ROWS_G8, ROWS_G4 };

template <bool G4, typename F>
RowClass with_group(int lanes, F &&f) {
    if (lanes > 16) { f(IntC<32>{}); return ROWS_G32; }
    if (lanes > 8)  { f(IntC<16>{}); return ROWS_G16; }
    if constexpr (G4) {
        if (lanes <= 4) { f(IntC<4>{}); return ROWS_G4; }
    }
    f(IntC<8>{});
    return ROWS_G8;
}

enum NameHubs { HUBS_NONE, HUBS_LONG, HUBS_CHUNKS };
enum NameMode { MODE_EVAL, MODE_DROP, MODE_DROP_ENTRIES };
#define GNX_NAMES6(mid, tail) {"spmm_none" mid tail, "spmm_wave" mid tail, "spmm_group32" mid tail, "spmm_group16" mid tail, "spmm_group8" mid tail, "spmm_group4" mid tail}
#define GNX_NAMES3(tail) {GNX_NAMES6("", tail), GNX_NAMES6("+long", tail), GNX_NAMES6("+chunks", tail)}
#define GNX_NAMES(tail) {GNX_NAMES3(tail), GNX_NAMES3("_drop" tail), GNX_NAMES3("_drop_entries" tail)}
[[maybe_unused]] const char *const kKernelNames[3][3][3][6] = {GNX_NAMES(""), GNX_NAMES("_bf16"), GNX_NAMES("_ord")};
#undef GNX_NAMES
#undef GNX_NAMES3
#undef GNX_NAMES6

template <typename R>
const char *kernel_name(RowClass rows, NameMode mode, NameHubs hubs) {
    if (hubs == HUBS_LONG && !R::NAMES_LONG) hubs = HUBS_NONE;
    return kKernelNames[R::GATHER_ORDER ? 2 : R::BF16][mode][hubs][rows];
}

template <typename R>
void set_operands(typename R::Args &p, const typename R::Elem *X, int64_t ldx, const float *H0, int64_t ldh0, float beta, float alpha, int act,
                  typename R::Out *out, int out_bf16, int64_t ldo, int64_t C) {
    R::bind_X(p, X); p.ldx = ldx; p.H0 = H0; p.ldh0 = ldh0; p.beta = beta; p.alpha = alpha; p.act = act;
    R::bind_out(p, out, out_bf16); p.ldo = ldo; p.C = (int)C;
}

[[maybe_unused]] int check_operands(const char *fn, const void *X, int64_t ldx, int64_t C, const float *H0, int64_t ldh0, const void *out,
                                    int64_t ldo) {
    GNX_CHECK_ARG(C >= 1 && C <= (1 << 20), "%s: feature width %lld not in [1, 2^20]", fn, (long long)C);
    GNX_CHECK_ARG(X != nullptr && out != nullptr, "%s: NULL X/out", fn);
    GNX_CHECK_ARG(ldx >= C && ldo >= C && (H0 == nullptr || ldh0 >= C || ldh0 == 0), "%s: leading dimension smaller than C", fn);
    GNX_CHECK_ARG(X != out, "%s: out must not alias X", fn);
    return GNX_OK;
}

[[maybe_unused]] int check_common(const char *fn, gnx_graph *g, const void *X, int64_t ldx, int64_t C, const float *H0, int64_t ldh0,
                                  const void *out, int64_t ldo) {
    GNX_CHECK_ARG(g != nullptr, "%s: NULL handle", fn);
    return check_operands(fn, X, ldx, C, H0, ldh0, out, ldo);
}

}
```

gnn-tf_amd/csrc/gnx_spmm_eval.h:

```cpp
#pragma once
#include "gnx_spmm_device.h"

namespace {

template <typename R, int VEC, int U, int WPB>
__global__ __launch_bounds__(64 * WPB) void k_spmm_wave(const typename R::Args p) {
    const int lane = threadIdx.x & 63;
    const int wib = __builtin_amdgcn_readfirstlane((int)(threadIdx.x >> 6));
    const int tune = R::EXPERIMENTS ? p.tune : 0;
    const int64_t slot = p.slot0 + xcd_block(p) * WPB + wib;
    if (slot >= p.n_rows) return;
    const auto [row, beg, end] = slot_row<true>(p, slot, (tune & 1) != 0);
    if (end - beg > p.long_row) return;
    if (p.skip_empty && beg == end) return;
    for (int c0 = 0; c0 < p.C; c0 += 64 * VEC) {
        const int c = c0 + lane * VEC;
        const bool active = c < p.C;
        float acc[VEC];
#pragma unroll
        for (int v = 0; v < VEC; ++v) acc[v] = 0.f;
        wave_accumulate<R, VEC, U>(p.colidx, p.vals, R::X(p), p.ldx, beg, end, active ? c : 0, lane, acc, (tune & 4) != 0);
        epilogue_store<R, VEC>(p, row, c, active, acc, (tune & 2) != 0);
    }
}

template <typename R, int VEC, int G, int U, bool PIPE>
__device__ __forceinline__ void group_rows(const typename R::Args &p, int64_t block) {
    constexpr int RPB = 256 / G;
    const int sub = threadIdx.x % G;
    const int64_t slot = p.slot0 + block * RPB + threadIdx.x / G;
    if (slot >= p.n_rows) return;
    const auto [row, beg, end] = slot_row<false>(p, slot);
    if (end - beg > p.long_row) return;
    if (p.skip_empty && beg == end) return;
    for (int c0 = 0; c0 < p.C; c0 += G * VEC) {
        const int c = c0 + sub * VEC;
        const bool active = c < p.C;
        const typename R::Elem *__restrict__ Xc = R::X(p) + (active ? c : 0);
        float acc[VEC];
#pragma unroll
        for (int v = 0; v < VEC; ++v) acc[v] = 0.f;
        if (PIPE) {
            int jn[U];
            float wn[U];
#pragma unroll
            for (int u = 0; u < U; ++u) {
                const bool ok = beg + u < end;
                jn[u] = ok ? p.colidx[beg + u] : -1;
                wn[u] = ok ? p.vals[beg + u] : 0.f;
            }
            for (int64_t e = beg; e < end; e += U) {
                float x[U][VEC];
                float w[U];
#pragma unroll
                for (int u = 0; u < U; ++u) {
                    w[u] = wn[u];
                    if (jn[u] >= 0) R::template load<VEC>(x[u], Xc + (int64_t)jn[u] * p.ldx);
                    else {
#pragma unroll
                        for (int v = 0; v < VEC; ++v) x[u][v] = 0.f;
                    }
                }
#pragma unroll
                for (int u = 0; u < U; ++u) {
                    const bool ok = e + U + u < end;
                    jn[u] = ok ? p.colidx[e + U + u] : -1;
                    wn[u] = ok ? p.vals[e + U + u] : 0.f;
                }
#pragma unroll
                for (int u = 0; u < U; ++u)
#pragma unroll
                    for (int v = 0; v < VEC; ++v) acc[v] = fmaf(w[u], x[u][v], acc[v]);
            }
        } else {
            for (int64_t e = beg; e < end; e += U) {
                float x[U][VEC];
                float w[U];
#pragma unroll
                for (int u = 0; u < U; ++u) {
                    if (e + u < end) {
                        const int j = p.colidx[e + u];
                        w[u] = p.vals[e + u];
                        R::template load<VEC>(x[u], Xc + (int64_t)j * p.ldx);
                    } else {
                        w[u] = 0.f;
#pragma unroll
                        for (int v = 0; v < VEC; ++v) x[u][v] = 0.f;
                    }
                }
#pragma unroll
                for (int u = 0; u < U; ++u)
#pragma unroll
                    for (int v = 0; v < VEC; ++v) acc[v] = fmaf(w[u], x[u][v], acc[v]);
            }
        }
        epilogue_store<R, VEC>(p, row, c, active, acc);
    }
}

template <typename R, int VEC, int G, int B>
__device__ __forceinline__ void group_rows_coop(const typename R::Args &p, int64_t block) {
    constexpr int RPB = 256 / G;
    const int sub = threadIdx.x % G;
    const int64_t slot = p.slot0 + block * RPB + threadIdx.x / G;
    if (slot >= p.n_rows) return;
    const auto [row, beg, end] = slot_row<false>(p, slot);
    if (end - beg > p.long_row) return;
    if (p.skip_empty && beg == end) return;
    for (int c0 = 0; c0 < p.C; c0 += G * VEC) {
        const int c = c0 + sub * VEC;
        const bool active = c < p.C;
        const typename R::Elem *__restrict__ Xc = R::X(p) + (active ? c : 0);
        float acc[VEC];
#pragma unroll
        for (int v = 0; v < VEC; ++v) acc[v] = 0.f;
        int myj = -1;
        float myw = 0.f;
        if (sub < B && beg + sub < end) { myj = p.colidx[beg + sub]; myw = p.vals[beg + sub]; }
        for (int64_t e = beg; e < end; e += B) {
            float x[B][VEC];
            float w[B];
#pragma unroll
            for (int u = 0; u < B; ++u) {
                const int j = __shfl(myj, u, G);
                w[u] = __shfl(myw, u, G);
                if (j >= 0) R::template load<VEC>(x[u], Xc + (int64_t)j * p.ldx);
                else {
#pragma unroll
                    for (int v = 0; v < VEC; ++v) x[u][v] = 0.f;
                }
            }
            myj = -1; myw = 0.f;
            if (sub < B && e + B + sub < end) { myj = p.colidx[e + B + sub]; myw = p.vals[e + B + sub]; }
#pragma unroll
            for (int u = 0; u < B; ++u)
#pragma unroll
                for (int v = 0; v < VEC; ++v) acc[v] = fmaf(w[u], x[u][v], acc[v]);
        }
        epilogue_store<R, VEC>(p, row, c, active, acc);
    }
}

template <typename R, int VEC, int G, int U, bool PIPE>
__global__ __launch_bounds__(256) void k_spmm_group(const typename R::Args p) {
    if (G <= 8) group_rows_coop<R, VEC, G, 4>(p, xcd_block(p));
    else group_rows<R, VEC, G, U, PIPE>(p, xcd_block(p));
}

template <typename R, int VEC, int U>
__global__ __launch_bounds__(256) void k_spmm_long_partial(const typename R::Args p) {
    const int lane = threadIdx.x & 63;
    const int wib = __builtin_amdgcn_readfirstlane((int)(threadIdx.x >> 6));
    const int64_t cslot = (int64_t)blockIdx.x * 4 + wib;
    if (cslot >= p.n_chunks) return;
    const auto [chunk, row, beg, end] = slot_chunk(p, cslot);
    for (int c0 = 0; c0 < p.C; c0 += 64 * VEC) {
        const int c = c0 + lane * VEC;
        const bool active = c < p.C;
        float acc[VEC];
#pragma unroll
        for (int v = 0; v < VEC; ++v) acc[v] = 0.f;
        wave_accumulate<R, VEC, U>(p.colidx, p.vals, R::X(p), p.ldx, beg, end, active ? c : 0, lane, acc);
        if (active) vstore<VEC>(p.partial + chunk * (int64_t)p.C + c, acc);
    }
}

template <typename R, int VEC, int G, int U>
__device__ __forceinline__ void long_chunks_group(const typename R::Args &p, int64_t block) {
    constexpr int NS = 64 / G;
    const int lane = threadIdx.x & 63;
    const int wib = __builtin_amdgcn_readfirstlane((int)(threadIdx.x >> 6));
    const int64_t cslot = block * 4 + wib;
    if (cslot >= p.n_chunks) return;
    const auto [chunk, row, beg, end] = slot_chunk(p, cslot);
    const int sub = lane / G;
    const int c = (lane % G) * VEC;
    const bool active = c < p.C;
    const typename R::Elem *__restrict__ Xc = R::X(p) + (active ? c : 0);
    float acc[VEC];
#pragma unroll
    for (int v = 0; v < VEC; ++v) acc[v] = 0.f;
    for (int64_t e = beg + sub; e < end; e += (int64_t)NS * U) {
        float x[U][VEC];
        float w[U];
#pragma unroll
        for (int u = 0; u < U; ++u) {
            const int64_t eu = e + (int64_t)u * NS;
            if (eu < end) {
                const int j = p.colidx[eu];
                w[u] = p.vals[eu];
                R::template load<VEC>(x[u], Xc + (int64_t)j * p.ldx);
            } else {
                w[u] = 0.f;
#pragma unroll
                for (int v = 0; v < VEC; ++v) x[u][v] = 0.f;
            }
        }
#pragma unroll
        for (int u = 0; u < U; ++u)
#pragma unroll
            for (int v = 0; v < VEC; ++v) acc[v] = fmaf(w[u], x[u][v], acc[v]);
    }
#pragma unroll
    for (int off = G; off < 64; off <<= 1)
#pragma unroll
        for (int v = 0; v < VEC; ++v) acc[v] += __shfl_xor(acc[v], off);
    if (sub == 0 && active) vstore<VEC>(p.partial + chunk * (int64_t)p.C + c, acc);
}

template <typename R, int VEC, int G, int U>
__global__ __launch_bounds__(256) void k_spmm_long_partial_group(const typename R::Args p) {
    long_chunks_group<R, VEC, G, U>(p, blockIdx.x);
}

template <typename R, int VEC, int G>
__global__ __launch_bounds__(256) void k_spmm_group_and_chunks(const typename R::Args p, int chunk_blocks) {
    if ((int)blockIdx.x < chunk_blocks) long_chunks_group<R, VEC, G, 4>(p, blockIdx.x);
    else if (G <= 8) group_rows_coop<R, VEC, G, 4>(p, (int64_t)blockIdx.x - chunk_blocks);
    else group_rows<R, VEC, G, 4, false>(p, (int64_t)blockIdx.x - chunk_blocks);
}

template <typename R, int VEC>
RowClass launch_rows(const typename R::Args &p0, hipStream_t s) {
    typename R::Args p = p0;
    const int lanes = (p.C + VEC - 1) / VEC;
    bool trim = true;
#ifdef GNX_TUNING
    if ((p.tune & (1 << 21)) || (lanes > 32 && (p.tune & 1))) trim = false;
#endif
    if (trim) trim_empty_rows(p, lanes);
    if (p.n_rows == 0) return ROWS_NONE;
    if (lanes > 32) {
        if (p.C <= 64 * VEC) GNX_ROW_PIECES((k_spmm_wave<R, VEC, 8, 8>), 8, 512);
        else                 GNX_ROW_PIECES((k_spmm_wave<R, VEC, 8, 4>), 4, 256);
        return ROWS_WAVE;
    }
    return with_group<false>(lanes, [&](auto G) {
#ifdef GNX_TUNING
        if constexpr (R::EXPERIMENTS) {
            if (((p.tune >> 8) & 3) == 2) {
                GNX_ROW_PIECES((k_spmm_group<R, VEC, G(), 4, true>), 256 / G(), 256);
                return;
            }
        }
#endif
        GNX_ROW_PIECES((k_spmm_group<R, VEC, G(), 4, false>), 256 / G(), 256);
    });
}

template <typename R, int VEC>
RowClass launch_rows_and_chunks(const typename R::Args &p, hipStream_t s) {
    const int lanes = (p.C + VEC - 1) / VEC;
    if (lanes > 32 || p.n_long == 0 || (p.n_rows >= SMALL_ROWS && !(p.tune & 65536)) || ((p.tune >> 8) & 3) != 0 || (p.tune & 4096)) return ROWS_NONE;
    const unsigned cb = blocks_for(p.n_chunks, 4);
    const RowClass rows = with_group<true>(lanes, [&](auto G) {
        hipLaunchKernelGGL((k_spmm_group_and_chunks<R, VEC, G()>), dim3(cb + blocks_for(p.n_rows, 256 / G())), dim3(256), 0, s, p, (int)cb);
    });
    GNX_LAUNCH((k_spmm_long_reduce<R, VEC>), blocks_for(p.n_long, 4), p);
    return rows;
}

template <typename R, int VEC>
void launch_long(const typename R::Args &p, hipStream_t s) {
    const int lanes = (p.C + VEC - 1) / VEC;
    if (lanes > 32) GNX_LAUNCH((k_spmm_long_partial<R, VEC, 8>), blocks_for(p.n_chunks, 4), p);
    else with_group<true>(lanes, [&](auto G) { GNX_LAUNCH((k_spmm_long_partial_group<R, VEC, G(), 4>), blocks_for(p.n_chunks, 4), p); });
    GNX_LAUNCH((k_spmm_long_reduce<R, VEC>), blocks_for(p.n_long, 4), p);
}

template <typename R>
const char *launch_eval(const typename R::Args &p, hipStream_t s) {
    return with_vec<R>(R::vec(p), [&](auto V) {
        RowClass rows = launch_rows_and_chunks<R, V()>(p, s);
        if (rows != ROWS_NONE) return kernel_name<R>(rows, MODE_EVAL, HUBS_CHUNKS);
        rows = launch_rows<R, V()>(p, s);
        if (p.n_long > 0) launch_long<R, V()>(p, s);
        return kernel_name<R>(rows, MODE_EVAL, p.n_long > 0 ? HUBS_LONG : HUBS_NONE);
    });
}

}
```

gnn-tf_amd/gnntf/_native.py:

```python
from __future__ import annotations

import ctypes
import os
from ctypes import POINTER, c_char_p, c_double, c_float, c_int, c_int64, c_uint64, c_void_p

_HERE = os.path.dirname(os.path.abspath(__file__))
ABI_VERSION = 900
LIB_PATH = os.environ.get("GNX_LIBRARY") or os.path.join(os.path.dirname(_HERE), "lib", "libgnx.so")

NORM = {"none": 0, "symmetric": 1, "bipartite": 2}
EYE = {"none": 0, "before": 1, "after": 2}
ACT_NONE, ACT_RELU, ACT_SKIP_EMPTY = 0, 1, 256
HALO_ALL, HALO_PULL, HALO_PUSH = 0, 1, 2
RESERVE_TRANSPOSED, RESERVE_K_LOOP, RESERVE_TRAIN_GATHER = 1, 2, 4
ORD_X, ORD_OUT = 1, 2

SIGNATURES = {
    "gnx_last_error": (c_char_p, []),
    "gnx_version": (c_int, []),
    "gnx_graph_create_coo": (c_int, [c_int64, c_int64, c_int64, c_void_p, c_void_p, c_void_p, POINTER(c_void_p)]),
    "gnx_graph_create_csr": (c_int, [c_int64, c_int64, c_int64, c_void_p, c_void_p, c_void_p, c_void_p, POINTER(c_void_p)]),
    "gnx_graph_destroy": (c_int, [c_void_p]),
    "gnx_graph_info": (c_int, [c_void_p, POINTER(c_int64), POINTER(c_int64), POINTER(c_int64), POINTER(c_int64)]),
    "gnx_graph_hub_rows": (c_int, [c_void_p, POINTER(c_int64), POINTER(c_int64)]),
    "gnx_graph_csr": (c_int, [c_void_p, POINTER(c_void_p), POINTER(c_void_p), POINTER(c_void_p)]),
    "gnx_graph_export": (c_int, [c_void_p, c_void_p, c_void_p, c_void_p, c_void_p, c_void_p]),
    "gnx_graph_normalize": (c_int, [c_void_p, c_int, c_int, c_float, c_uint64, c_uint64, c_void_p, c_void_p, c_void_p]),
    "gnx_graph_normalize_t": (c_int, [c_void_p, c_int, c_int, c_float, c_uint64, c_uint64, c_void_p, c_void_p, c_void_p]),
    "gnx_graph_reserve": (c_int, [c_void_p, c_int64, c_int, c_void_p]),
    "gnx_graph_enable_entry_dropout": (c_int, [c_void_p, c_void_p]),
    "gnx_graph_set_row_window": (c_int, [c_void_p, c_int64, c_void_p]),
    "gnx_graph_set_dropout_counter": (c_int, [c_void_p, c_void_p]),
    "gnx_graph_set_block": (c_int, [c_void_p, c_int64, c_int64, c_void_p, c_void_p]),
    "gnx_graph_colsum": (c_int, [c_void_p, c_float, c_uint64, c_uint64, c_void_p, c_void_p]),
    "gnx_graph_colsum_streams": (c_int, [c_void_p, c_float, c_uint64, c_uint64, c_int, c_void_p, c_void_p]),
    "gnx_degree_scale": (c_int, [c_void_p, c_int64, c_int, c_int, c_void_p]),
    "gnx_graph_scale_values": (c_int, [c_void_p, c_float, c_uint64, c_uint64, c_void_p, c_void_p, c_void_p, c_void_p]),
    "gnx_spmm": (c_int, [c_void_p, c_void_p, c_void_p, c_void_p, c_int64, c_int64, c_void_p, c_int64, c_float, c_float,
                         c_int, c_void_p, c_int64, c_void_p]),
    "gnx_spmm_t": (c_int, [c_void_p, c_void_p, c_void_p, c_void_p, c_int64, c_int64, c_void_p, c_int64, c_float, c_float,
                           c_int, c_void_p, c_int64, c_void_p]),
    "gnx_spmm_scatter": (c_int, [c_void_p, c_void_p, c_void_p, c_void_p, c_int64, c_int64, c_void_p, c_int64, c_float, c_float,
                                 c_int, c_void_p, c_void_p, c_int64, c_void_p]),
    "gnx_spmm_dropped": (c_int, [c_void_p, c_void_p, c_float, c_uint64, c_uint64, c_int, c_void_p, c_int64, c_int64, c_void_p, c_int64,
                                 c_float, c_float, c_int, c_void_p, c_int64, c_void_p]),
    "gnx_spmm_dropped_chained": (c_int, [c_void_p, c_void_p, c_float, c_uint64, c_uint64, c_int, c_void_p, c_void_p, c_int64, c_int64, c_void_p,
                                         c_int64, c_float, c_float, c_int, c_void_p, c_int64, c_void_p]),
    "gnx_spmm_dropped_back": (c_int, [c_void_p, c_void_p, c_float, c_uint64, c_uint64, c_int, c_void_p, c_void_p, c_int64, c_int64, c_void_p,
                                      c_int64, c_float, c_float, c_void_p, c_int64, c_float, c_void_p, c_int64, c_int, c_void_p]),
    "gnx_graph_gather_order": (c_int, [c_void_p, POINTER(c_void_p), POINTER(c_void_p)]),
    "gnx_spmm_dropped_chained_ord": (c_int, [c_void_p, c_void_p, c_float, c_uint64, c_uint64, c_int, c_void_p, c_void_p, c_int64, c_int64,
                                             c_void_p, c_int64, c_float, c_float, c_int, c_void_p, c_int64, c_int, c_void_p]),
    "gnx_spmm_dropped_back_ord": (c_int, [c_void_p, c_void_p, c_float, c_uint64, c_uint64, c_int, c_void_p, c_void_p, c_int64, c_int64,
                                          c_void_p, c_int64, c_float, c_float, c_void_p, c_int64, c_float, c_void_p, c_int64, c_int, c_int,
                                          c_void_p]),
    "gnx_spmm_rows": (c_int, [c_void_p, c_void_p, c_void_p, c_int64, c_int64, c_void_p, c_int64, c_float, c_float, c_int,
                              c_void_p, c_void_p, c_int64, c_void_p]),
    "gnx_spmm_tv": (c_int, [c_void_p, c_void_p, c_void_p, c_void_p, c_int64, c_int64, c_void_p, c_int64, c_float, c_float,
                            c_int, c_void_p, c_int64, c_void_p]),
    "gnx_graph_permute_values_t": (c_int, [c_void_p, c_void_p, c_void_p, c_void_p]),
    "gnx_ppr_step": (c_int, [c_void_p, c_void_p, c_void_p, c_void_p, c_void_p, c_float, c_int64, c_int, c_void_p, c_void_p]),
    "gnx_appnp_propagate": (c_int, [c_void_p, c_void_p, c_void_p, c_void_p, c_float, c_int, c_int64, c_void_p, c_void_p,
                                    c_void_p]),
    "gnx_appnp_propagate_act": (c_int, [c_void_p, c_void_p, c_void_p, c_void_p, c_float, c_int, c_int64, c_int, c_void_p, c_void_p,
                                        c_void_p]),
    "gnx_cast_bf16": (c_int, [c_void_p, c_int64, c_int64, c_int64, c_void_p, c_int64, c_void_p]),
    "gnx_spmm_bf16": (c_int, [c_void_p, c_void_p, c_void_p, c_void_p, c_int64, c_int64, c_void_p, c_int64, c_float, c_float,
                              c_int, c_void_p, c_int, c_int64, c_void_p]),
    "gnx_spmm_rows_bf16": (c_int, [c_void_p, c_void_p, c_void_p, c_int64, c_int64, c_void_p, c_int64, c_float, c_float, c_int,
                                   c_void_p, c_void_p, c_int, c_int64, c_void_p]),
    "gnx_halo_pack_bf16": (c_int, [c_void_p, c_int, c_void_p, c_int64, c_int64, c_void_p, c_int64, c_void_p]),
    "gnx_halo_exchange_bf16": (c_int, [c_void_p, c_int, c_void_p, c_void_p, c_void_p, c_int64, c_void_p]),
    "gnx_appnp_propagate_bf16": (c_int, [c_void_p, c_void_p, c_void_p, c_void_p, c_float, c_int, c_int64, c_int, c_void_p, c_void_p,
                                         c_void_p]),
    "gnx_spmm_dropped_chained_bf16": (c_int, [c_void_p, c_void_p, c_float, c_uint64, c_uint64, c_int, c_void_p, c_void_p, c_int64, c_int64,
                                              c_void_p, c_int64, c_float, c_float, c_int, c_void_p, c_int, c_int64, c_void_p]),
    "gnx_spmm_dropped_back_bf16": (c_int, [c_void_p, c_void_p, c_float, c_uint64, c_uint64, c_int, c_void_p, c_void_p, c_int64, c_int64,
                                           c_void_p, c_int64, c_float, c_float, c_void_p, c_int64, c_float, c_void_p, c_int64, c_int,
                                           c_void_p]),
    "gnx_halo_plan_create": (c_int, [c_int, c_int, c_int64, c_void_p, c_void_p, c_void_p, c_void_p, c_void_p, c_void_p, POINTER(c_void_p)]),
    "gnx_halo_plan_destroy": (c_int, [c_void_p]),
    "gnx_halo_plan_layout": (c_int, [c_void_p, POINTER(c_int64), POINTER(c_int64), POINTER(c_int64), POINTER(c_int64), c_void_p, c_void_p,
                                     c_void_p]),
    "gnx_halo_pack": (c_int, [c_void_p, c_int, c_void_p, c_int64, c_int64, c_void_p, c_int64, c_void_p]),
    "gnx_halo_exchange": (c_int, [c_void_p, c_int, c_void_p, c_void_p, c_void_p, c_int64, c_void_p]),
    "gnx_halo_bind_rccl": (c_int, [c_void_p, c_void_p, c_void_p, c_void_p]),
    "gnx_gather_rows32": (c_int, [c_void_p, c_int64, c_void_p, c_int64, c_int64, c_void_p, c_int64, c_void_p]),
    "gnx_gather_rows": (c_int, [c_void_p, c_int64, c_void_p, c_int64, c_int64, c_void_p, c_int64, c_void_p]),
    "gnx_gcnii_step": (c_int, [c_void_p, c_void_p, c_void_p, c_void_p, c_float, c_int64, c_void_p, c_int64, c_int, c_void_p,
                               c_void_p, c_void_p]),
    "gnx_gcnii_step_bf16": (c_int, [c_void_p, c_void_p, c_void_p, c_void_p, c_float, c_int64, c_void_p, c_int64, c_int, c_void_p,
                                    c_int, c_void_p, c_void_p]),
    "gnx_gcnii_step_back": (c_int, [c_void_p, c_void_p, c_void_p, c_float, c_int64, c_void_p, c_int64, c_void_p, c_void_p, c_float,
                                    c_void_p, c_void_p, c_void_p]),
    "gnx_gcnii_step_drop": (c_int, [c_void_p, c_void_p, c_void_p, c_void_p, c_float, c_int64, c_void_p, c_int64, c_int, c_double, c_uint64,
                                    c_uint64, c_void_p, c_void_p, c_void_p]),
    "gnx_feature_dropout": (c_int, [c_void_p, c_void_p, c_int64, c_int64, c_int64, c_void_p, c_double, c_uint64, c_uint64, c_void_p, c_int64,
                                    c_void_p]),
    "gnx_feature_dropout_back": (c_int, [c_void_p, c_void_p, c_int64, c_void_p, c_int64, c_int64, c_int64, c_double, c_uint64, c_uint64,
                                         c_int, c_void_p, c_int64, c_void_p]),
    "gnx_gcnii_step_train_bf16": (c_int, [c_void_p, c_void_p, c_void_p, c_void_p, c_float, c_int64, c_void_p, c_int64, c_int, c_double,
                                          c_uint64, c_uint64, c_void_p, c_int, c_void_p, c_void_p, c_void_p]),
    "gnx_feature_dropout_back_bf16": (c_int, [c_void_p, c_void_p, c_int64, c_void_p, c_int64, c_int64, c_int64, c_double, c_uint64, c_uint64,
                                              c_int, c_void_p, c_int64, c_void_p, c_int64, c_void_p]),
    "gnx_gcnii_step_back_bf16": (c_int, [c_void_p, c_void_p, c_void_p, c_void_p, c_float, c_int64, c_void_p, c_int64, c_void_p, c_void_p,
                                         c_float, c_void_p, c_void_p, c_void_p]),
    "gnx_gcnii_wgrad": (c_int, [c_void_p, c_void_p, c_void_p, c_void_p, c_float, c_int64, c_void_p, c_void_p, c_void_p, c_void_p, c_int64,
                                c_void_p]),
    "gnx_gcnii_wgrad_bf16": (c_int, [c_void_p, c_void_p, c_void_p, c_void_p, c_float, c_int64, c_void_p, c_void_p, c_void_p, c_void_p, c_int64,
                                     c_void_p]),
    "gnx_gcnii_step_drop_bf16": (c_int, [c_void_p, c_void_p, c_void_p, c_void_p, c_float, c_int64, c_void_p, c_int64, c_int, c_double,
                                         c_uint64, c_uint64, c_void_p, c_int, c_void_p, c_void_p]),
    "gnx_gcnii_step_spectral": (c_int, [c_void_p, c_void_p, c_void_p, c_void_p, c_float, c_int64, c_void_p, c_int64, c_void_p, c_int, c_double,
                                        c_uint64, c_uint64, c_void_p, c_void_p, c_void_p, c_void_p]),
    "gnx_gcnii_spectral_back": (c_int, [c_void_p, c_void_p, c_int64, c_void_p, c_int64, c_int64, c_int, c_double, c_uint64, c_uint64, c_void_p,
                                        c_int64, c_void_p, c_void_p, c_int64, c_void_p]),
    "gnx_gcnii_step_dropped": (c_int, [c_void_p, c_void_p, c_float, c_uint64, c_uint64, c_void_p, c_void_p, c_float, c_int64, c_void_p, c_int64,
                                       c_int, c_double, c_uint64, c_uint64, c_void_p, c_void_p, c_void_p]),
    "gnx_gcnii_step_back_dropped": (c_int, [c_void_p, c_void_p, c_float, c_uint64, c_uint64, c_void_p, c_float, c_int64, c_void_p, c_int64,
                                            c_void_p, c_void_p, c_float, c_void_p, c_void_p, c_void_p]),
    "gnx_dense": (c_int, [c_void_p, c_int64, c_int64, c_int64, c_void_p, c_int64, c_int64, c_void_p, c_int, c_void_p, c_int64,
                          c_void_p]),
    "gnx_dense_wgrad": (c_int, [c_void_p, c_int64, c_void_p, c_int64, c_int64, c_int64, c_int64, c_void_p, c_void_p, c_int64, c_void_p]),
    "gnx_node_ce": (c_int, [c_void_p, c_int64, c_int64, c_int64, c_void_p, c_void_p, c_int64, c_void_p, c_void_p, c_void_p]),
    "gnx_node_ce_backward": (c_int, [c_void_p, c_int64, c_int64, c_int64, c_void_p, c_void_p, c_int64, c_void_p, c_void_p, c_int64,
                                     c_void_p]),
    "gnx_node_argmax": (c_int, [c_void_p, c_int64, c_int64, c_int64, c_void_p, c_int64, c_void_p, c_void_p]),
    "gnx_edge_scores": (c_int, [c_void_p, c_int64, c_int64, c_int64, c_void_p, c_int64, c_void_p, c_void_p, c_void_p]),
    "gnx_edge_scores_backward": (c_int, [c_void_p, c_int64, c_int64, c_int64, c_void_p, c_int64, c_void_p, c_void_p, c_void_p, c_int64,
                                         c_void_p]),
    "gnx_linear_combination": (c_int, [c_int, c_void_p, c_void_p, c_int64, c_void_p, c_void_p]),
    "gnx_stream_read": (c_int, [c_void_p, c_int64, c_void_p, c_void_p]),
    "gnx_stream_copy": (c_int, [c_void_p, c_void_p, c_int64, c_void_p]),
    "gnx_probe_block_xcd": (c_int, [c_int64, c_void_p, c_void_p]),
    "gnx_graph_last_kernel": (c_char_p, [c_void_p]),
}

_lib = None


def lib():
    global _lib
    if _lib is None:
        if not os.path.exists(LIB_PATH):
            raise Exception(f"gnntf: the HIP library {LIB_PATH} is missing -- build it with "
                            f"`make -C gnn-tf_amd/csrc` (or __graft_entry__.build()); there is no CPU fallback")
        handle = ctypes.CDLL(LIB_PATH)
        for name, (restype, argtypes) in SIGNATURES.items():
            fn = getattr(handle, name)
            fn.restype = restype
            fn.argtypes = argtypes
        version = int(handle.gnx_version())
        if version // 100 != ABI_VERSION // 100:
            raise Exception(f"gnntf: {LIB_PATH} implements ABI {version}, this package binds ABI {ABI_VERSION}: rebuild the library "
                            f"(make -C gnn-tf_amd/csrc)")
        _lib = handle
    return _lib


def check(rc: int):
    if rc != 0:
        msg = lib().gnx_last_error()
        raise Exception((msg.decode() if msg else "") or f"libgnx error {rc}")


def ptr(t):
    return None if t is None else c_void_p(t.data_ptr())


def current_stream():
    import torch
    return c_void_p(torch._C._cuda_getCurrentRawStream(torch.cuda.current_device()))


class on_device:

    __slots__ = ("index", "prev")

    def __init__(self, device):
        self.index = device.index

    def __enter__(self):
        import torch
        self.prev = torch.cuda.current_device()
# ... 17 lines not shown
```

gnn-tf_amd/gnntf/sparse.py:

```python
from __future__ import annotations

import math
from ctypes import byref, c_float, c_int64, c_void_p

import numpy as np
import torch

from . import _native as nat


class SparseCOO:

    def __init__(self, indices, values, dense_shape):
        if isinstance(indices, torch.Tensor):
            self.indices = indices.to(torch.int64).reshape(-1, 2)
            self.values = torch.as_tensor(values, dtype=torch.float32, device=self.indices.device).reshape(-1)
        else:
            self.indices = torch.from_numpy(np.ascontiguousarray(np.asarray(indices, dtype=np.int64).reshape(-1, 2)))
            self.values = torch.from_numpy(np.ascontiguousarray(np.asarray(values, dtype=np.float32).reshape(-1)))
        if self.indices.shape[0] != self.values.shape[0]:
            raise Exception("SparseCOO: indices and values disagree on the number of entries")
        self.dense_shape = (int(dense_shape[0]), int(dense_shape[1]))

    @property
    def shape(self):
        return self.dense_shape

    def to(self, device):
        return SparseCOO(self.indices.to(device), self.values.to(device), self.dense_shape)


def as_coo(graph) -> SparseCOO:
    if isinstance(graph, SparseCOO):
        return graph
    if isinstance(graph, torch.Tensor) and graph.is_sparse:
        return SparseCOO(graph._indices().t().contiguous(), graph._values(), graph.shape)
    if hasattr(graph, "tocoo"):
        m = graph.tocoo()
        return SparseCOO(np.stack([m.row, m.col], axis=1), m.data, m.shape)
    if isinstance(graph, (tuple, list)) and len(graph) == 3:
        return SparseCOO(*graph)
    raise Exception("Unsupported graph container: " + str(type(graph)))


class _BorrowedInt32:

    def __init__(self, pointer, n):
        self.__cuda_array_interface__ = dict(shape=(int(n),), typestr="<i4", data=(int(pointer or 0), False), version=2)


class DeviceGraph:

    def __init__(self, coo: SparseCOO = None, device=None, csr=None):
        self._h = c_void_p()
        lib = nat.lib()
        if csr is not None:
            rowptr, colidx, vals, shape = csr
            nat.require_cuda(rowptr, colidx, vals)
            if (rowptr.dtype, colidx.dtype, vals.dtype) != (torch.int64, torch.int32, torch.float32):
                raise Exception("DeviceGraph: a CSR needs int64 rowptr, int32 colidx and float32 values")
            if not (rowptr.device == colidx.device == vals.device):
                raise Exception("DeviceGraph: the CSR arrays live on different devices")
            if rowptr.numel() != shape[0] + 1 or colidx.numel() != vals.numel():
                raise Exception("DeviceGraph: CSR array lengths do not match the shape")
            self.device = rowptr.device
            self._keep = (rowptr.contiguous(), colidx.contiguous(), vals.contiguous())
            with nat.on_device(self.device):
                nat.check(lib.gnx_graph_create_csr(shape[0], shape[1], self._keep[1].numel(), nat.ptr(self._keep[0]),
                                                   nat.ptr(self._keep[1]), nat.ptr(self._keep[2]), nat.current_stream(),
                                                   byref(self._h)))
            self._keep = None
        else:
            device = torch.device(device if device is not None else "cuda")
            if device.type != "cuda":
                raise Exception("gnntf: graphs live on the GPU only; there is no CPU fallback")
            self.device = device
            idx = coo.indices.to(device).contiguous()
            val = coo.values.to(device).contiguous()
            self.device = idx.device
            with nat.on_device(device):
                nat.check(lib.gnx_graph_create_coo(coo.dense_shape[0], coo.dense_shape[1], idx.shape[0], nat.ptr(idx),
                                                   nat.ptr(val), nat.current_stream(), byref(self._h)))
        n_rows, n_cols, nnz_e, nnz_c = c_int64(), c_int64(), c_int64(), c_int64()
        nat.check(lib.gnx_graph_info(self._h, byref(n_rows), byref(n_cols), byref(nnz_e), byref(nnz_c)))
        self.n_rows, self.n_cols = n_rows.value, n_cols.value
        self.nnz_entries, self.nnz = nnz_e.value, nnz_c.value
        n_hub, threshold = c_int64(), c_int64()
        nat.check(lib.gnx_graph_hub_rows(self._h, byref(n_hub), byref(threshold)))
        self.n_hub_rows, self.long_row_threshold = n_hub.value, threshold.value
        self._entry_dropout = False

    @property
    def handle(self):
        return self._h

    @property
    def entry_dropout(self) -> bool:
        return getattr(self, "_entry_dropout", False)

    def enable_entry_dropout(self):
        with nat.on_device(self.device):
            nat.check(nat.lib().gnx_graph_enable_entry_dropout(self._h, nat.current_stream()))
        self._entry_dropout = True

    def csr_arrays(self, with_rows=False):
        rowptr = torch.empty(self.n_rows + 1, dtype=torch.int64, device=self.device)
        colidx = torch.empty(self.nnz, dtype=torch.int32, device=self.device)
        vals = torch.empty(self.nnz, dtype=torch.float32, device=self.device)
        rows = torch.empty(self.nnz, dtype=torch.int32, device=self.device) if with_rows else None
        with nat.on_device(self.device):
            nat.check(nat.lib().gnx_graph_export(self._h, nat.ptr(rowptr), nat.ptr(colidx), nat.ptr(vals), nat.ptr(rows),
                                                 nat.current_stream()))
        return (rowptr, colidx, vals, rows) if with_rows else (rowptr, colidx, vals)

    def last_kernel(self) -> str:
        return (nat.lib().gnx_graph_last_kernel(self._h) or b"").decode()

    def reserve(self, C, transposed=False, k_loop=False, train_gather=False):
        flags = ((nat.RESERVE_TRANSPOSED if transposed else 0) | (nat.RESERVE_K_LOOP if k_loop else 0)
                 | (nat.RESERVE_TRAIN_GATHER if train_gather else 0))
        with nat.on_device(self.device):
            nat.check(nat.lib().gnx_graph_reserve(self._h, int(C), flags, nat.current_stream()))

    def gather_order(self):
        order, rank = c_void_p(), c_void_p()
        with nat.on_device(self.device):
            nat.check(nat.lib().gnx_graph_gather_order(self._h, byref(order), byref(rank)))
            return tuple(torch.as_tensor(_BorrowedInt32(p.value, self.n_rows), device=self.device).clone() for p in (order, rank))

    def set_row_window(self, window_rows):
        with nat.on_device(self.device):
            nat.check(nat.lib().gnx_graph_set_row_window(self._h, int(window_rows), nat.current_stream()))
        self.row_window = int(window_rows)

    def set_dropout_counter(self, counter):
        if counter is not None and (counter.dtype != torch.int64 or counter.numel() != 1 or counter.device != self.device):
            raise Exception("set_dropout_counter: needs a one-element int64 tensor on the graph's device")
        self._counter = counter
        nat.check(nat.lib().gnx_graph_set_dropout_counter(self._h, nat.ptr(counter)))

    def __del__(self):
        try:
            if self._h:
                nat.lib().gnx_graph_destroy(self._h)
                self._h = c_void_p()
        except Exception:
            pass


class Adjacency:

    def __init__(self, graph: DeviceGraph, vals: torch.Tensor = None, diag: torch.Tensor = None, vals_t: torch.Tensor = None):
        self.graph = graph
        self.vals = vals
        self.diag = diag
        self.vals_t = vals_t

    def transposed_values(self):
        if self.vals_t is None:
            out = torch.empty(self.graph.nnz, dtype=torch.float32, device=self.graph.device)
            with nat.on_device(self.graph.device):
                nat.check(nat.lib().gnx_graph_permute_values_t(self.graph.handle, nat.ptr(self.vals), nat.ptr(out), nat.current_stream()))
            self.vals_t = out
        return self.vals_t

    @property
    def shape(self):
        return (self.graph.n_rows, self.graph.n_cols)


class DroppedAdjacency(Adjacency):

    def __init__(self, graph: DeviceGraph, p, seed, stream_id, D=None):
        super().__init__(graph, None, None, None)
        self.p, self.seed, self.stream_id = float(p), int(seed) & 0xFFFFFFFFFFFFFFFF, int(stream_id) & 0xFFFFFFFFFFFFFFFF
        self.D = D if D is not None else dropped_degree_scales(graph, self.p, self.seed, self.stream_id, 1)[0]
        self._vals = None

    @property
    def vals(self):
        if self._vals is None:
            self._vals = normalize(self.graph, "symmetric", "none", self.p, self.seed, self.stream_id).vals
        return self._vals

    @vals.setter
    def vals(self, value):
        self._vals = value

    def transposed_values(self):
        if self.vals_t is None:
            self.vals_t = normalize(self.graph, "symmetric", "none", self.p, self.seed, self.stream_id, transposed_only=True).vals_t
        return self.vals_t


def dropped_degree_scales(graph: DeviceGraph, p, seed, first_stream, n_streams) -> torch.Tensor:
    D = torch.empty((n_streams, graph.n_cols), dtype=torch.float32, device=graph.device)
    with nat.on_device(graph.device):
        nat.check(nat.lib().gnx_graph_colsum_streams(graph.handle, float(p), int(seed) & 0xFFFFFFFFFFFFFFFF,
                                                     int(first_stream) & 0xFFFFFFFFFFFFFFFF, int(n_streams), nat.ptr(D), nat.current_stream()))
        nat.check(nat.lib().gnx_degree_scale(nat.ptr(D), D.numel(), nat.NORM["symmetric"], 0, nat.current_stream()))
    return D


def can_fuse_dropout(graph: DeviceGraph, p) -> bool:
    return graph.n_rows == graph.n_cols and p > 0 and (graph.nnz_entries == graph.nnz or graph.entry_dropout)


def dropped_adjacency(graph: DeviceGraph, p, seed, stream_id, D=None) -> Adjacency:
    if can_fuse_dropout(graph, p):
        return DroppedAdjacency(graph, p, seed, stream_id, D=D)
    return normalize(graph, "symmetric", "none", p, seed, stream_id)


def normalize(graph: DeviceGraph, normalized="symmetric", add_eye="none", dropout=0.0, seed=0, stream_id=0,
              transposed_only=False) -> Adjacency:
    if normalized not in nat.NORM:
        raise Exception("Invalid matrix normalization")
    if add_eye not in nat.EYE:
        raise Exception("Invalid add_eye option")
    vals = torch.empty(graph.nnz, dtype=torch.float32, device=graph.device)
    diag = torch.empty(graph.n_rows, dtype=torch.float32, device=graph.device) if add_eye != "none" else None
    fn = nat.lib().gnx_graph_normalize_t if transposed_only else nat.lib().gnx_graph_normalize
    with nat.on_device(graph.device):
        nat.check(fn(graph.handle, nat.NORM[normalized], nat.EYE[add_eye], float(dropout), int(seed) & 0xFFFFFFFFFFFFFFFF,
                     int(stream_id) & 0xFFFFFFFFFFFFFFFF, nat.ptr(vals), nat.ptr(diag), nat.current_stream()))
    return Adjacency(graph, None, diag, vals_t=vals) if transposed_only else Adjacency(graph, vals, diag)


def _as_f32_rows(x: torch.Tensor) -> torch.Tensor:
    if x.dtype != torch.float32:
        x = x.float()
    if x.dim() != 2:
        raise Exception("propagation expects a 2-D feature matrix")
    if x.stride(1) != 1 or x.stride(0) < x.shape[1]:
        x = x.contiguous()
    return x


def _same_device(g, *tensors):
    for t in tensors:
        if t is not None and t.device != g.device:
            raise Exception(f"spmm: operand on {t.device}, the graph lives on {g.device}")


def _mix_operand(H0, shape, bias=False):
    if H0 is None:
        return None, 0
    H0 = _as_f32_rows(H0)
    if bias and tuple(H0.shape) == (1, shape[1]) and shape[0] != 1:
        return H0.contiguous(), 0
    if tuple(H0.shape) != tuple(shape):
        raise Exception("spmm: H0 shape mismatch")
    return H0, H0.stride(0)


def _launch(adj: Adjacency, X, H0, beta, alpha, act, transposed=False, out=None, out_rows=None):
    g = adj.graph
    nat.require_cuda(X, H0)
    _same_device(g, X, H0, out, out_rows, adj.diag)
    X = _as_f32_rows(X)
    rows_in = g.n_rows if transposed else g.n_cols
    rows_out = g.n_cols if transposed else g.n_rows
    if X.shape[0] != rows_in:
        raise Exception(f"spmm: features have {X.shape[0]} rows, adjacency expects {rows_in}")
    C = X.shape[1]
    if out is None:
        out = torch.empty((rows_out, C), dtype=torch.float32, device=X.device)
    elif (tuple(out.shape) != (rows_out, C) or out.dtype != torch.float32 or out.stride(1) != 1 or not out.is_cuda):
        raise Exception("spmm: bad output buffer")
    H0, ldh0 = _mix_operand(H0, (rows_out, C), bias=True)
    if isinstance(adj, DroppedAdjacency) and out_rows is None:
        with nat.on_device(X.device):
            nat.check(nat.lib().gnx_spmm_dropped(g.handle, nat.ptr(adj.D), adj.p, adj.seed, adj.stream_id, 1 if transposed else 0,
                                                 nat.ptr(X), X.stride(0), C, nat.ptr(H0), ldh0, float(beta), float(alpha), int(act),
                                                 nat.ptr(out), out.stride(0), nat.current_stream()))
        return out
    if transposed:
        fn, values = nat.lib().gnx_spmm_tv, adj.transposed_values()
    else:
        if adj.vals is None and adj.vals_t is not None:
            raise Exception("spmm: this adjacency only holds transposed-order values")
# ... 1241 lines not shown
```

include/gnx.h:

```cpp
#ifndef GNX_H
#define GNX_H

#include <stdint.h>

#ifdef __cplusplus
extern "C" {
#endif

typedef struct gnx_graph *gnx_graph_t;
typedef struct gnx_halo_plan *gnx_halo_plan_t;

enum { GNX_OK = 0, GNX_ERR_INVALID = -1, GNX_ERR_HIP = -2, GNX_ERR_ALLOC = -3, GNX_ERR_UNSUPPORTED = -4 };

enum { GNX_NORM_NONE = 0, GNX_NORM_SYMMETRIC = 1, GNX_NORM_BIPARTITE = 2 };
enum { GNX_EYE_NONE = 0, GNX_EYE_BEFORE = 1, GNX_EYE_AFTER = 2 };
enum { GNX_ACT_NONE = 0, GNX_ACT_RELU = 1 };
enum { GNX_ACT_SKIP_EMPTY = 256 };

const char *gnx_last_error(void);
#define GNX_ABI_VERSION 900
int gnx_version(void);

int gnx_graph_create_coo(int64_t n_rows, int64_t n_cols, int64_t nnz, const int64_t *d_indices,
                         const float *d_values, void *stream, gnx_graph_t *out);

int gnx_graph_create_csr(int64_t n_rows, int64_t n_cols, int64_t nnz, const int64_t *d_rowptr,
                         const int32_t *d_colidx, const float *d_values, void *stream, gnx_graph_t *out);

int gnx_graph_destroy(gnx_graph_t g);

int gnx_graph_info(gnx_graph_t g, int64_t *n_rows, int64_t *n_cols, int64_t *nnz_entries,
                   int64_t *nnz_coalesced);
int gnx_graph_hub_rows(gnx_graph_t g, int64_t *n_hub_rows, int64_t *threshold);

int gnx_graph_csr(gnx_graph_t g, const int64_t **d_rowptr, const int32_t **d_colidx,
                  const float **d_raw_values);
int gnx_graph_export(gnx_graph_t g, int64_t *d_rowptr_out, int32_t *d_colidx_out, float *d_raw_values_out,
                     int32_t *d_rowidx_out, void *stream);

int gnx_graph_normalize(gnx_graph_t g, int normalized, int add_eye, float dropout_p, uint64_t seed,
                        uint64_t stream_id, float *d_vals_out, float *d_diag_out, void *stream);

enum { GNX_RESERVE_TRANSPOSED = 1, GNX_RESERVE_K_LOOP = 2, GNX_RESERVE_TRAIN_GATHER = 4 };
int gnx_graph_reserve(gnx_graph_t g, int64_t C, int flags, void *stream);

int gnx_graph_enable_entry_dropout(gnx_graph_t g, void *stream);

int gnx_graph_set_row_window(gnx_graph_t g, int64_t window_rows, void *stream);

int gnx_graph_set_dropout_counter(gnx_graph_t g, const uint64_t *d_counter);

int gnx_graph_set_block(gnx_graph_t g, int64_t row0_global, int64_t row0_buf, const int32_t *d_col_gid, void *stream);

int gnx_graph_normalize_t(gnx_graph_t g, int normalized, int add_eye, float dropout_p, uint64_t seed,
                          uint64_t stream_id, float *d_vals_t_out, float *d_diag_out, void *stream);

int gnx_graph_colsum(gnx_graph_t g, float dropout_p, uint64_t seed, uint64_t stream_id,
                     float *d_colsum_out, void *stream);
int gnx_graph_colsum_streams(gnx_graph_t g, float dropout_p, uint64_t seed, uint64_t first_stream, int n_streams,
                             float *d_colsum_out, void *stream);
int gnx_degree_scale(float *d_deg, int64_t n, int normalized, int add_eye_before, void *stream);
int gnx_graph_scale_values(gnx_graph_t g, float dropout_p, uint64_t seed, uint64_t stream_id,
                           const float *d_row_scale, const float *d_col_scale, float *d_vals_out,
                           void *stream);

int gnx_spmm(gnx_graph_t g, const float *d_vals, const float *d_diag, const float *d_X, int64_t ldx,
             int64_t C, const float *d_H0, int64_t ldh0, float beta, float alpha, int act,
             float *d_out, int64_t ldo, void *stream);
int gnx_spmm_t(gnx_graph_t g, const float *d_vals, const float *d_diag, const float *d_X, int64_t ldx,
               int64_t C, const float *d_H0, int64_t ldh0, float beta, float alpha, int act,
               float *d_out, int64_t ldo, void *stream);

int gnx_spmm_tv(gnx_graph_t g, const float *d_vals_t, const float *d_diag, const float *d_X, int64_t ldx,
                int64_t C, const float *d_H0, int64_t ldh0, float beta, float alpha, int act,
                float *d_out, int64_t ldo, void *stream);
int gnx_graph_permute_values_t(gnx_graph_t g, const float *d_vals, float *d_vals_t_out, void *stream);

int gnx_spmm_scatter(gnx_graph_t g, const float *d_vals, const float *d_diag, const float *d_X, int64_t ldx,
                     int64_t C, const float *d_H0, int64_t ldh0, float beta, float alpha, int act,
                     const int32_t *d_out_rows, float *d_out, int64_t ldo, void *stream);

int gnx_spmm_dropped(gnx_graph_t g, const float *d_D, float dropout_p, uint64_t seed, uint64_t stream_id, int transposed,
                     const float *d_X, int64_t ldx, int64_t C, const float *d_H0, int64_t ldh0, float beta, float alpha,
                     int act, float *d_out, int64_t ldo, void *stream);

int gnx_spmm_dropped_chained(gnx_graph_t g, const float *d_D, float dropout_p, uint64_t seed, uint64_t stream_id, int x_prescaled,
                             const float *d_D_next, const float *d_X, int64_t ldx, int64_t C, const float *d_H0, int64_t ldh0,
                             float beta, float alpha, int act, float *d_out, int64_t ldo, void *stream);

int gnx_spmm_dropped_back(gnx_graph_t g, const float *d_D, float dropout_p, uint64_t seed, uint64_t stream_id, int x_prescaled,
                          const float *d_D_next, const float *d_X, int64_t ldx, int64_t C, const float *d_S_in, int64_t lds_in,
                          float s_alpha, float s_beta, float *d_S_out, int64_t lds_out, float y_beta, float *d_Y_out, int64_t ldy,
                          int act, void *stream);

enum { GNX_ORD_X = 1, GNX_ORD_OUT = 2 };
int gnx_graph_gather_order(gnx_graph_t g, const int32_t **d_order, const int32_t **d_rank);
int gnx_spmm_dropped_chained_ord(gnx_graph_t g, const float *d_D, float dropout_p, uint64_t seed, uint64_t stream_id, int x_prescaled,
                                 const float *d_D_next, const float *d_X, int64_t ldx, int64_t C, const float *d_H0, int64_t ldh0,
                                 float beta, float alpha, int act, float *d_out, int64_t ldo, int order, void *stream);
int gnx_spmm_dropped_back_ord(gnx_graph_t g, const float *d_D, float dropout_p, uint64_t seed, uint64_t stream_id, int x_prescaled,
                              const float *d_D_next, const float *d_X, int64_t ldx, int64_t C, const float *d_S_in, int64_t lds_in,
                              float s_alpha, float s_beta, float *d_S_out, int64_t lds_out, float y_beta, float *d_Y_out, int64_t ldy,
                              int act, int order, void *stream);

int gnx_spmm_rows(gnx_graph_t g, const float *d_vals, const float *d_X, int64_t ldx, int64_t C, const float *d_H0,
                  int64_t ldh0, float beta, float alpha, int act, const int32_t *d_rows, float *d_out, int64_t ldo,
                  void *stream);

int gnx_ppr_step(gnx_graph_t g, const float *d_vals, const float *d_diag, const float *d_H,
                 const float *d_H0, float a, int64_t C, int act, float *d_out, void *stream);

int gnx_appnp_propagate(gnx_graph_t g, const float *d_vals, const float *d_diag, const float *d_H0,
                        float a, int K, int64_t C, float *d_out, float *d_work, void *stream);

int gnx_appnp_propagate_act(gnx_graph_t g, const float *d_vals, const float *d_diag, const float *d_H0,
                            float a, int K, int64_t C, int act, float *d_out, float *d_work, void *stream);

int gnx_cast_bf16(const float *d_src, int64_t n_rows, int64_t C, int64_t lds, uint16_t *d_dst, int64_t ldd, void *stream);
int gnx_spmm_bf16(gnx_graph_t g, const float *d_vals, const float *d_diag, const uint16_t *d_X, int64_t ldx, int64_t C,
                  const float *d_H0, int64_t ldh0, float beta, float alpha, int act, void *d_out, int out_bf16, int64_t ldo,
                  void *stream);
int gnx_appnp_propagate_bf16(gnx_graph_t g, const float *d_vals, const float *d_diag, const float *d_H0, float a, int K, int64_t C,
                             int act, float *d_out, uint16_t *d_work, void *stream);
int gnx_spmm_rows_bf16(gnx_graph_t g, const float *d_vals, const uint16_t *d_X, int64_t ldx, int64_t C, const float *d_H0,
                       int64_t ldh0, float beta, float alpha, int act, const int32_t *d_rows, void *d_out, int out_bf16, int64_t ldo,
                       void *stream);

int gnx_spmm_dropped_chained_bf16(gnx_graph_t g, const float *d_D, float dropout_p, uint64_t seed, uint64_t stream_id,
                                  int x_prescaled, const float *d_D_next, const uint16_t *d_X, int64_t ldx, int64_t C,
                                  const float *d_H0, int64_t ldh0, float beta, float alpha, int act,
                                  void *d_out, int out_bf16, int64_t ldo, void *stream);
int gnx_spmm_dropped_back_bf16(gnx_graph_t g, const float *d_D, float dropout_p, uint64_t seed, uint64_t stream_id,
                               int x_prescaled, const float *d_D_next, const uint16_t *d_X, int64_t ldx, int64_t C,
                               const float *d_S_in, int64_t lds_in, float s_alpha, float s_beta, float *d_S_out, int64_t lds_out,
                               float y_beta, uint16_t *d_Y_out, int64_t ldy, int act, void *stream);

int gnx_gcnii_step(gnx_graph_t g, const float *d_vals, const float *d_H, const float *d_H0, float a, int64_t C,
                   const float *d_M, int64_t ldm, int act, float *d_out, float *d_mixed, void *stream);
int gnx_gcnii_step_bf16(gnx_graph_t g, const float *d_vals, const uint16_t *d_H, const float *d_H0, float a, int64_t C,
                        const float *d_M, int64_t ldm, int act, void *d_out, int out_bf16, float *d_work, void *stream);

int gnx_gcnii_step_back(gnx_graph_t g, const float *d_vals_t, const float *d_G, float a, int64_t C,
                        const float *d_Mt, int64_t ldmt, float *d_dH,
                        const float *d_S_in, float s_alpha, float *d_S_out,
                        float *d_work, void *stream);

int gnx_gcnii_step_drop(gnx_graph_t g, const float *d_vals, const float *d_H, const float *d_H0, float a, int64_t C,
                        const float *d_M, int64_t ldm, int act, double dropout_p, uint64_t seed, uint64_t stream_id,
                        float *d_out, float *d_mixed, void *stream);
int gnx_feature_dropout(gnx_graph_t g, const float *d_X, int64_t ldx, int64_t n_rows, int64_t C, const int32_t *d_rows,
                        double dropout_p, uint64_t seed, uint64_t stream_id, float *d_out, int64_t ldo, void *stream);
int gnx_feature_dropout_back(gnx_graph_t g, const float *d_g, int64_t ldg, const float *d_y, int64_t ldy, int64_t n_rows, int64_t C,
                             double dropout_p, uint64_t seed, uint64_t stream_id, int act, float *d_G, int64_t ldG, void *stream);

int gnx_gcnii_step_train_bf16(gnx_graph_t g, const float *d_vals, const uint16_t *d_H, const float *d_H0, float a, int64_t C,
                              const float *d_M, int64_t ldm, int act, double dropout_p, uint64_t seed, uint64_t stream_id,
                              void *d_out, int out_bf16, float *d_mixed, float *d_work, void *stream);
int gnx_feature_dropout_back_bf16(gnx_graph_t g, const float *d_g, int64_t ldg, const uint16_t *d_y, int64_t ldy, int64_t n_rows,
                                  int64_t C, double dropout_p, uint64_t seed, uint64_t stream_id, int act, float *d_G, int64_t ldG,
                                  uint16_t *d_Gb, int64_t ldGb, void *stream);
int gnx_gcnii_step_back_bf16(gnx_graph_t g, const float *d_vals_t, const uint16_t *d_Gb, const float *d_G, float a, int64_t C,
                             const float *d_Mt, int64_t ldmt, float *d_dH, const float *d_S_in, float s_alpha, float *d_S_out,
                             float *d_work, void *stream);

int gnx_gcnii_wgrad(gnx_graph_t g, const float *d_vals, const float *d_H, const float *d_H0, float a, int64_t C,
                    const float *d_G, float *d_dM, float *d_hub_rows, float *d_work, int64_t work_floats, void *stream);
int gnx_gcnii_wgrad_bf16(gnx_graph_t g, const float *d_vals, const uint16_t *d_H, const float *d_H0, float a, int64_t C,
                         const float *d_G, float *d_dM, float *d_hub_rows, float *d_work, int64_t work_floats, void *stream);
int gnx_gcnii_step_drop_bf16(gnx_graph_t g, const float *d_vals, const uint16_t *d_H, const float *d_H0, float a, int64_t C,
                             const float *d_M, int64_t ldm, int act, double dropout_p, uint64_t seed, uint64_t stream_id,
                             void *d_out, int out_bf16, float *d_work, void *stream);

int gnx_gcnii_step_spectral(gnx_graph_t g, const float *d_vals, const float *d_H, const float *d_H0, float a, int64_t C,
                            const float *d_M, int64_t ldm, const float *d_bias, int act, double dropout_p, uint64_t seed,
                            uint64_t stream_id, float *d_out, float *d_mixed, uint32_t *d_gate, void *stream);
int gnx_gcnii_spectral_back(gnx_graph_t g, const float *d_g, int64_t ldg, const uint32_t *d_gate, int64_t n_rows, int64_t C, int act,
                            double dropout_p, uint64_t seed, uint64_t stream_id, float *d_G, int64_t ldG, float *d_dbias,
                            float *d_work, int64_t work_floats, void *stream);

int gnx_gcnii_step_dropped(gnx_graph_t g, const float *d_D, float edge_p, uint64_t edge_seed, uint64_t edge_stream, const float *d_H,
                           const float *d_H0, float a, int64_t C, const float *d_M, int64_t ldm, int act, double feat_p,
                           uint64_t feat_seed, uint64_t feat_stream, float *d_out, float *d_mixed, void *stream);
int gnx_gcnii_step_back_dropped(gnx_graph_t g, const float *d_D, float edge_p, uint64_t edge_seed, uint64_t edge_stream,
                                const float *d_G, float a, int64_t C, const float *d_Mt, int64_t ldmt, float *d_dH,
                                const float *d_S_in, float s_alpha, float *d_S_out, float *d_work, void *stream);

int gnx_dense(const float *d_X, int64_t ldx, int64_t n, int64_t F, const float *d_W, int64_t ldw, int64_t O,
              const float *d_bias, int act, float *d_out, int64_t ldo, void *stream);

int gnx_dense_wgrad(const float *d_X, int64_t ldx, const float *d_G, int64_t ldg, int64_t n, int64_t F, int64_t O, float *d_dW,
                    float *d_work, int64_t work_floats, void *stream);

int gnx_node_ce(const float *d_logits, int64_t ldl, int64_t n_rows, int64_t C, const int64_t *d_nodes,
                const int64_t *d_labels, int64_t m, float *d_loss_per_node, float *d_mean_loss, void *stream);
int gnx_node_ce_backward(const float *d_logits, int64_t ldl, int64_t n_rows, int64_t C, const int64_t *d_nodes,
                         const int64_t *d_labels, int64_t m, const float *d_grad_loss, float *d_grad_logits, int64_t ldg,
                         void *stream);
// ... 41 lines not shown
```

Before: 12.95 billion edges/s.

## Tag cold gather columns so their feature loads bypass cache with nontemporal hints

```diff
diff --git a/gnn-tf_amd/csrc/gnx_gcnii.hip b/gnn-tf_amd/csrc/gnx_gcnii.hip
--- a/gnn-tf_amd/csrc/gnx_gcnii.hip
+++ b/gnn-tf_amd/csrc/gnx_gcnii.hip
@@ -196,7 +196,7 @@
 #pragma unroll
             for (int m = 1; m < GW; m <<= 1) word |= (uint32_t)__shfl_xor((int)word, m);
             if (!live[ps]) continue;
-            R::template store<4>(p, rows[ps] * p.ldo, c, o, false);
+            R::template store<4>(p, rows[ps] * p.ldo, c, o);
             if (sp.gate != nullptr && sub % GW == 0) sp.gate[rows[ps] * WORDS + (c >> 5)] = word;
         }
         return;
@@ -212,7 +212,7 @@
             const DropFuse &fd = feature_mask<EDGE>(p, ed);
             drop_values<4>(fd, drop_stream(fd), rows[ps], c, o);
         }
-        R::template store<4>(p, rows[ps] * p.ldo, c, o, false);
+        R::template store<4>(p, rows[ps] * p.ldo, c, o);
     }
 }
 
diff --git a/gnn-tf_amd/csrc/gnx_graph.hip b/gnn-tf_amd/csrc/gnx_graph.hip
--- a/gnn-tf_amd/csrc/gnx_graph.hip
+++ b/gnn-tf_amd/csrc/gnx_graph.hip
@@ -221,6 +221,21 @@
                                  int32_t *__restrict__ gcol) {
     int64_t k = (int64_t)blockIdx.x * blockDim.x + threadIdx.x;
     if (k < nnz) gcol[k] = rank[colidx[k]];
+}
+
+__global__ void k_hint_keys(const int64_t *__restrict__ rowptr, int64_t n, uint64_t *__restrict__ keys, int32_t *__restrict__ ids) {
+    int64_t r = (int64_t)blockIdx.x * blockDim.x + threadIdx.x;
+    if (r >= n) return;
+    keys[r] = (uint64_t)(0x7fffffff - (rowptr[r + 1] - rowptr[r]));
+    ids[r] = (int32_t)r;
+}
+
+__global__ void k_hint_columns(const int32_t *__restrict__ colidx, const int32_t *__restrict__ rank, int64_t nnz, int64_t hot,
+                               int32_t *__restrict__ hint_cols) {
+    int64_t k = (int64_t)blockIdx.x * blockDim.x + threadIdx.x;
+    if (k >= nnz) return;
+    const int32_t c = colidx[k];
+    hint_cols[k] = rank[c] < hot ? c : (int32_t)((uint32_t)c | 0x80000000u);
 }
 
 __global__ void k_permute_vals(const float *__restrict__ vals, const int32_t *__restrict__ perm, int64_t n,
@@ -428,6 +443,7 @@
 static void drop_transpose(gnx_graph *g) { static_cast<TransposedPart &>(*g) = TransposedPart(); }
 static void drop_relabel(gnx_graph *g) { static_cast<RelabelledPart &>(*g) = RelabelledPart(); }
 static void drop_gather_order(gnx_graph *g) { static_cast<GatherOrderPart &>(*g) = GatherOrderPart(); }
+static void drop_gather_hints(gnx_graph *g) { static_cast<GatherHintsPart &>(*g) = GatherHintsPart(); }
 
 int ensure_transpose(gnx_graph *g, hipStream_t s) {
     if (g->has_t) return GNX_OK;
@@ -553,6 +569,66 @@
     return GNX_OK;
 }
 
+static bool takes_gather_hints(const gnx_graph *g) {
+    return g->a.n_rows == g->a.n_cols && g->blk_col_gid == nullptr && g->a.order_window == 0 && g->a.nnz > 0;
+}
+
+static int64_t hint_hot_rows(const gnx_graph *g, int64_t C) {
+    if (!takes_gather_hints(g) || g->hint_setting == 0 || C * (int64_t)sizeof(float) < HINT_MIN_ROW_BYTES) return 0;
+    const int64_t n = g->a.n_rows;
+    if (g->hint_setting > 0) return std::min(g->hint_setting, n);
+    if (n < HINT_MIN_ROWS) return 0;
+    return std::min(n, std::max<int64_t>(1, HINT_HOT_BYTES / (C * (int64_t)sizeof(float))));
+}
+
+static int ensure_gather_hints(gnx_graph *g, int64_t hot, hipStream_t s) {
+    const Csr &a = g->a;
+    const dim3 threads(256);
+    if (g->hint_cols == nullptr) {
+        GNX_NOT_WHILE_CAPTURING(s, "the gather hints of this handle (GNX_RESERVE_GATHER_HINTS)");
+        GatherHintsPart part;
+        DevArray<uint64_t> k0, k1;
+        DevArray<int32_t> ids, order;
+        const size_t n = (size_t)a.n_rows;
+        hipError_t e = part.hint_cols.alloc(a.nnz);
+        if (e == hipSuccess) e = part.hint_rank.alloc(n);
+        if (e == hipSuccess) e = k0.alloc(n);
+        if (e == hipSuccess) e = k1.alloc(n);
+        if (e == hipSuccess) e = ids.alloc(n);
+        if (e == hipSuccess) e = order.alloc(n);
+        if (e != hipSuccess) {
+            (void)hipGetLastError();
+            g->hint_failed = true;
+            set_error("gather hints: %s while allocating %lld bytes for the hinted columns: this handle runs unhinted", hipGetErrorString(e),
+                      (long long)a.nnz * 4);
+            return GNX_OK;
+        }
+        hipLaunchKernelGGL(k_hint_keys, dim3(blocks_for(a.n_rows)), threads, 0, s, a.rowptr, a.n_rows, k0, ids);
+        GNX_TRY(sort_pairs<uint64_t, int32_t>(k0, k1, ids, order, a.n_rows, 31u, s));
+        hipLaunchKernelGGL(k_invert_order, dim3(blocks_for(a.n_rows)), threads, 0, s, order, a.n_rows, part.hint_rank);
+        GNX_HIP(hipStreamSynchronize(s));
+        GNX_HIP(hipGetLastError());
+        part.hint_hot = -1;
+        static_cast<GatherHintsPart &>(*g) = std::move(part);
+    }
+    if (g->hint_hot != hot && !stream_is_capturing(s)) {
+        hipLaunchKernelGGL(k_hint_columns, dim3(blocks_for(a.nnz)), threads, 0, s, a.colidx, g->hint_rank, a.nnz, hot, g->hint_cols);
+        GNX_HIP(hipGetLastError());
+        g->hint_hot = hot;
+    }
+    return GNX_OK;
+}
+
+int gather_hints_for(gnx_graph *g, const Csr &m, int64_t C, hipStream_t s, const int32_t **hint_cols) {
+    *hint_cols = nullptr;
+    if (&m != &g->a || g->hint_failed) return GNX_OK;
+    const int64_t hot = hint_hot_rows(g, C);
+    if (hot == 0) return GNX_OK;
+    if (g->hint_cols == nullptr || g->hint_hot != hot) GNX_TRY(ensure_gather_hints(g, hot, s));
+    *hint_cols = g->hint_cols;
+    return GNX_OK;
+}
+
 static int finish_graph(gnx_graph *g, hipStream_t s) {
     GNX_TRY(build_long_plan(g->a, s));
     GNX_HIP(hipGetLastError());
@@ -575,7 +651,7 @@
 
 int gnx_graph_reserve(gnx_graph_t g, int64_t C, int flags, void *stream) {
     GNX_CHECK_ARG(g != nullptr, "gnx_graph_reserve: NULL handle");
-    GNX_CHECK_ARG(C >= 1 && (flags & ~(GNX_RESERVE_TRANSPOSED | GNX_RESERVE_K_LOOP | GNX_RESERVE_TRAIN_GATHER)) == 0,
+    GNX_CHECK_ARG(C >= 1 && (flags & ~(GNX_RESERVE_TRANSPOSED | GNX_RESERVE_K_LOOP | GNX_RESERVE_TRAIN_GATHER | GNX_RESERVE_GATHER_HINTS)) == 0,
                   "gnx_graph_reserve: bad width / flags");
     if (flags & GNX_RESERVE_TRAIN_GATHER) flags |= GNX_RESERVE_TRANSPOSED;
     hipStream_t s = (hipStream_t)stream;
@@ -594,6 +670,10 @@
         chunks = std::max(chunks, g->r.n_chunks);
     }
     if (flags & GNX_RESERVE_TRAIN_GATHER) GNX_TRY(ensure_train_gather(g, "gnx_graph_reserve(GNX_RESERVE_TRAIN_GATHER)", s));
+    if (flags & GNX_RESERVE_GATHER_HINTS) {
+        const int32_t *unused;
+        GNX_TRY(gather_hints_for(g, g->a, C, s, &unused));
+    }
     if (chunks > 0) return ensure_partial(g, (size_t)chunks * (size_t)C * sizeof(float), s);
     return GNX_OK;
 }
@@ -607,6 +687,31 @@
     GNX_TRY(ensure_gather_order(g, nullptr));
     if (d_order) *d_order = g->go_order;
     if (d_rank) *d_rank = g->go_rank;
+    return GNX_OK;
+}
+
+int gnx_graph_set_gather_hints(gnx_graph_t g, int64_t hot_rows, void *stream) {
+    GNX_CHECK_ARG(g != nullptr, "gnx_graph_set_gather_hints: NULL handle");
+    GNX_CHECK_ARG(hot_rows >= -1, "gnx_graph_set_gather_hints: hot_rows %lld is neither -1 (automatic), 0 (off) nor a row count", (long long)hot_rows);
+    hipStream_t s = (hipStream_t)stream;
+    GNX_CHECK_ARG(!stream_is_capturing(s), "gnx_graph_set_gather_hints: the stream is being captured -- set the hints before the capture begins");
+    g->hint_setting = hot_rows;
+    g->hint_failed = false;
+    if (hot_rows == 0) {
+        GNX_HIP(hipDeviceSynchronize());
+        drop_gather_hints(g);
+    } else if (hot_rows > 0 && takes_gather_hints(g)) {
+        GNX_TRY(ensure_gather_hints(g, std::min(hot_rows, g->a.n_rows), s));
+    }
+    return GNX_OK;
+}
+
+int gnx_graph_gather_hints(gnx_graph_t g, const int32_t **d_hint_cols, int64_t *hot_rows, int64_t *last_launch_hot_rows) {
+    GNX_CHECK_ARG(g != nullptr, "gnx_graph_gather_hints: NULL handle");
+    const bool built = takes_gather_hints(g) && g->hint_cols != nullptr && g->hint_hot >= 0;
+    if (d_hint_cols) *d_hint_cols = built ? g->hint_cols.get() : nullptr;
+    if (hot_rows) *hot_rows = built ? g->hint_hot : 0;
+    if (last_launch_hot_rows) *last_launch_hot_rows = g->last_hint_hot;
     return GNX_OK;
 }
 
@@ -638,6 +743,7 @@
     }
     if (g->has_r) drop_relabel(g);
     drop_gather_order(g);
+    drop_gather_hints(g);
     GNX_HIP(hipGetLastError());
     return GNX_OK;
 }
diff --git a/gnn-tf_amd/csrc/gnx_internal.h b/gnn-tf_amd/csrc/gnx_internal.h
--- a/gnn-tf_amd/csrc/gnx_internal.h
+++ b/gnn-tf_amd/csrc/gnx_internal.h
@@ -42,6 +42,12 @@
 constexpr int SMALL_ROWS = 1 << 20;
 constexpr int TINY_ROWS = 1 << 15;
 constexpr int RELABEL_MAX_C = 16;
+constexpr int64_t HINT_HOT_BYTES = (int64_t)256 << 20;
+constexpr int64_t HINT_MIN_ROWS = 1 << 25;
+constexpr int64_t HINT_MIN_ROW_BYTES = 256;
+#ifndef GNX_GATHER_HINTS_DEFAULT
+#define GNX_GATHER_HINTS_DEFAULT (-1)
+#endif
 constexpr int SMALL_LONG_ROW = GNX_LONG_ROW < 128 ? GNX_LONG_ROW : 128;
 
 template <class T>
@@ -119,9 +125,16 @@
     DevArray<int32_t> t_gcol;
 };
 
-}
-
-struct gnx_graph : gnx::TransposedPart, gnx::RelabelledPart, gnx::GatherOrderPart {
+struct GatherHintsPart {
+    DevArray<int32_t> hint_cols;
+    DevArray<int32_t> hint_rank;
+    int64_t hint_hot = 0;
+    bool hint_failed = false;
+};
+
+}
+
+struct gnx_graph : gnx::TransposedPart, gnx::RelabelledPart, gnx::GatherOrderPart, gnx::GatherHintsPart {
     gnx::Csr a;
     gnx::DevArray<float> raw_vals;
     gnx::DevArray<int32_t> rowidx;
@@ -141,6 +154,8 @@
     gnx::DevArray<float> r_feat;
     size_t r_feat_bytes = 0;
     const char *last_kernel = "";
+    int64_t last_hint_hot = 0;
+    int64_t hint_setting = GNX_GATHER_HINTS_DEFAULT;
 };
 
 namespace gnx {
@@ -153,6 +168,7 @@
 int ensure_gather_order(gnx_graph *g, hipStream_t s);
 int ensure_train_gather(gnx_graph *g, const char *fn, hipStream_t s);
 int ensure_relabel_features(gnx_graph *g, size_t bytes, hipStream_t s);
+int gather_hints_for(gnx_graph *g, const Csr &m, int64_t C, hipStream_t s, const int32_t **hint_cols);
 
 inline unsigned blocks_for(int64_t n, int per_block = 256) { return (unsigned)((n + per_block - 1) / per_block); }
 
diff --git a/gnn-tf_amd/csrc/gnx_spmm.hip b/gnn-tf_amd/csrc/gnx_spmm.hip
--- a/gnn-tf_amd/csrc/gnx_spmm.hip
+++ b/gnn-tf_amd/csrc/gnx_spmm.hip
@@ -27,12 +27,22 @@
 #endif
 
 int launch_spmm(gnx_graph *g, const Csr &m, SpmmArgs &p, hipStream_t s) {
+    const int32_t *hint_cols = nullptr;
+    if (p.fuse.D == nullptr && F32Rows::vec(p) == 4) {
+        const int rc = gather_hints_for(g, m, p.C, s, &hint_cols);
+        if (rc != GNX_OK) return rc;
+    }
     return launch_bound(g, m, p, s, [&](SpmmArgs &q) {
 #ifdef GNX_TUNING
         static const int tune = [] { const char *e = getenv("GNX_TUNE"); return e ? atoi(e) : 0; }();
         q.tune = tune_override >= 0 ? tune_override : tune;
         if (q.tune & 16384) q.ldx = 0;
 #endif
+        if (hint_cols != nullptr) {
+            q.colidx = hint_cols;
+            g->last_hint_hot = g->hint_hot;
+            return launch_eval<F32Rows, true>(q, s);
+        }
         return q.fuse.D != nullptr ? launch_spmm_dropped(q, F32Rows::vec(q), s) : launch_eval<F32Rows>(q, s);
     });
 }
diff --git a/gnn-tf_amd/csrc/gnx_spmm_device.h b/gnn-tf_amd/csrc/gnx_spmm_device.h
--- a/gnn-tf_amd/csrc/gnx_spmm_device.h
+++ b/gnn-tf_amd/csrc/gnx_spmm_device.h
@@ -45,28 +45,47 @@
 template <> struct NatT<2> { using type = f32x2; };
 template <> struct NatT<4> { using type = f32x4; };
 
-template <int VEC>
-__device__ __forceinline__ void vload_nt(float (&x)[VEC], const float *__restrict__ p) {
-    if constexpr (VEC == 8) {
-        vload_nt<4>(*reinterpret_cast<float(*)[4]>(&x[0]), p);
-        vload_nt<4>(*reinterpret_cast<float(*)[4]>(&x[4]), p + 4);
-    } else {
-        using T = typename NatT<VEC>::type;
-        const T v = __builtin_nontemporal_load(reinterpret_cast<const T *>(p));
-        __builtin_memcpy(x, &v, sizeof(T));
-    }
-}
-template <int VEC>
-__device__ __forceinline__ void vstore_nt(float *__restrict__ p, const float (&x)[VEC]) {
-    if constexpr (VEC == 8) {
-        vstore_nt<4>(p, *reinterpret_cast<const float(*)[4]>(&x[0]));
-        vstore_nt<4>(p + 4, *reinterpret_cast<const float(*)[4]>(&x[4]));
-    } else {
-        using T = typename NatT<VEC>::type;
-        T v;
-        __builtin_memcpy(&v, x, sizeof(T));
-        __builtin_nontemporal_store(v, reinterpret_cast<T *>(p));
-    }
+constexpr int HINT_NONE = -1;
+__device__ __forceinline__ int hint_col(int j) { return j & 0x7fffffff; }
+
+__device__ __forceinline__ void gather16_hinted(f32x4 &x, const float *q, int j) {
+    uint64_t keep;
+    asm volatile("s_mov_b64 %[keep], exec\n\t"
+                 "v_cmp_gt_i32_e32 vcc, -1, %[j]\n\t"
+                 "s_and_b64 exec, %[keep], vcc\n\t"
+                 "s_cbranch_scc0 .Lgnx_nocold%=\n\t"
+                 "global_load_dwordx4 %[x], %[q], off nt\n"
+                 ".Lgnx_nocold%=:\n\t"
+                 "s_mov_b64 exec, %[keep]\n\t"
+                 "v_cmp_lt_i32_e32 vcc, -1, %[j]\n\t"
+                 "s_and_b64 exec, %[keep], vcc\n\t"
+                 "s_cbranch_scc0 .Lgnx_nohot%=\n\t"
+                 "global_load_dwordx4 %[x], %[q], off\n"
+                 ".Lgnx_nohot%=:\n\t"
+                 "s_mov_b64 exec, %[keep]"
+                 : [x] "+v"(x), [keep] "=&s"(keep)
+                 : [q] "v"(q), [j] "v"(j)
+                 : "vcc", "scc");
+}
+
+__device__ __forceinline__ void gather16_hinted_uniform(f32x4 &x, const float *q, int j) {
+    asm volatile("s_bitcmp1_b32 %[j], 31\n\t"
+                 "s_cbranch_scc1 .Lgnx_cold%=\n\t"
+                 "global_load_dwordx4 %[x], %[q], off\n\t"
+                 "s_branch .Lgnx_done%=\n"
+                 ".Lgnx_cold%=:\n\t"
+                 "global_load_dwordx4 %[x], %[q], off nt\n"
+                 ".Lgnx_done%=:"
+                 : [x] "+v"(x)
+                 : [q] "v"(q), [j] "s"(j)
+                 : "scc");
+}
+
+template <int U>
+__device__ __forceinline__ void gather_wait(f32x4 (&x)[U]) {
+    static_assert(U == 4 || U == 8, "batches of 4 or 8 gathers");
+    if constexpr (U == 4) asm volatile("s_waitcnt vmcnt(0)" : "+v"(x[0]), "+v"(x[1]), "+v"(x[2]), "+v"(x[3]));
+    else asm volatile("s_waitcnt vmcnt(0)" : "+v"(x[0]), "+v"(x[1]), "+v"(x[2]), "+v"(x[3]), "+v"(x[4]), "+v"(x[5]), "+v"(x[6]), "+v"(x[7]));
 }
 
 template <int VEC> struct BfRaw;
@@ -137,10 +156,7 @@
     __device__ static bool has_out2(const Args &p) { return p.out2 != nullptr; }
     __device__ static const float *out_scale(const Args &p) { return p.out_scale; }
     template <int VEC>
-    __device__ static void store(const Args &p, int64_t at, int c, const float (&o)[VEC], bool nt) {
-        if (nt) vstore_nt<VEC>(p.out + at + c, o);
-        else vstore<VEC>(p.out + at + c, o);
-    }
+    __device__ static void store(const Args &p, int64_t at, int c, const float (&o)[VEC]) { vstore<VEC>(p.out + at + c, o); }
     template <int VEC>
     __device__ static void store2(const Args &p, int64_t at, int c, const float (&o)[VEC]) { vstore<VEC>(p.out2 + at + c, o); }
     static int vec(const Args &p) { return pick_vec(p, MAX_VEC, p.X, 4, p.out, 4, nullptr, 0); }
@@ -187,7 +203,7 @@
     __device__ static bool has_out2(const Args &p) { return TRAIN && p.out2b != nullptr; }
     __device__ static const float *out_scale(const Args &p) { return TRAIN ? p.out_scale : nullptr; }
     template <int VEC>
-    __device__ static void store(const Args &p, int64_t at, int c, const float (&o)[VEC], bool) {
+    __device__ static void store(const Args &p, int64_t at, int c, const float (&o)[VEC]) {
         if (p.out_bf16) bstore<VEC>(static_cast<uint16_t *>(p.outv) + at + c, o);
         else vstore<VEC>(static_cast<float *>(p.outv) + at + c, o);
     }
@@ -210,7 +226,7 @@
     else return nullptr;
 }
 
-template <typename R, int VEC, int U, bool FUSE = false, bool ENTRIES = false, bool GCOL = false>
+template <typename R, int VEC, int U, bool FUSE = false, bool ENTRIES = false, bool GCOL = false, bool HINT = false>
 __device__ __forceinline__ void wave_accumulate(const int32_t *__restrict__ colidx, const float *__restrict__ vals,
                                                 const typename R::Elem *__restrict__ X, int64_t ldx, int64_t beg, int64_t end,
                                                 int c, int lane, float (&acc)[VEC], bool nt_index = false,
@@ -260,6 +276,46 @@
             }
             continue;
         }
+        if constexpr (HINT) {
+            static_assert(VEC == 4 && !FUSE && std::is_same_v<typename R::Elem, float>, "hinted gathers: f32 rows, 16 bytes per lane, eval");
+            for (; i + U <= n; i += U) {
+                f32x4 x[U];
+#pragma unroll
+                for (int u = 0; u < U; ++u) {
+                    const int j = readlane_i(mycol, i + u);
+                    x[u] = f32x4{0.f, 0.f, 0.f, 0.f};
+                    gather16_hinted_uniform(x[u], X + (int64_t)hint_col(j) * ldx + c, j);
+                }
+                gather_wait<U>(x);
+#pragma unroll
+                for (int u = 0; u < U; ++u) {
+                    const float w = readlane_f(myval, i + u);
+#pragma unroll
+                    for (int v = 0; v < VEC; ++v) acc[v] = fmaf(w, x[u][v], acc[v]);
+                }
+            }
+            if (i < n) {
+                f32x4 x[U];
+#pragma unroll
+                for (int u = 0; u < U; ++u) {
+                    x[u] = f32x4{0.f, 0.f, 0.f, 0.f};
+                    if (u < U - 1 && i + u < n) {
+                        const int j = readlane_i(mycol, i + u);
+                        gather16_hinted_uniform(x[u], X + (int64_t)hint_col(j) * ldx + c, j);
+                    }
+                }
+                gather_wait<U>(x);
+#pragma unroll
+                for (int u = 0; u < U - 1; ++u) {
+                    if (i + u < n) {
+                        const float w = readlane_f(myval, i + u);
+#pragma unroll
+                        for (int v = 0; v < VEC; ++v) acc[v] = fmaf(w, x[u][v], acc[v]);
+                    }
+                }
+            }
+            continue;
+        }
         for (; i + U <= n; i += U) {
             float x[U][VEC];
 #pragma unroll
@@ -296,8 +352,7 @@
 }
 
 template <typename R, int VEC>
-__device__ __forceinline__ void epilogue_store(const typename R::Args &p, int64_t row, int c, bool active, float (&acc)[VEC],
-                                               bool nt = false) {
+__device__ __forceinline__ void epilogue_store(const typename R::Args &p, int64_t row, int c, bool active, float (&acc)[VEC]) {
     if (!active) return;
     if (R::diag(p)) {
         const float d = R::diag(p)[row];
@@ -322,8 +377,7 @@
     if (p.H0) {
         const int64_t hrow = p.map_h0 ? orow : row;
         float h0[VEC];
-        if (nt) vload_nt<VEC>(h0, p.H0 + hrow * p.ldh0 + c);
-        else vload<VEC>(h0, p.H0 + hrow * p.ldh0 + c);
+        vload<VEC>(h0, p.H0 + hrow * p.ldh0 + c);
 #pragma unroll
         for (int v = 0; v < VEC; ++v) o[v] = fmaf(acc[v], p.beta, h0[v] * p.alpha);
     } else {
@@ -339,7 +393,7 @@
 #pragma unroll
         for (int v = 0; v < VEC; ++v) o[v] *= os;
     }
-    R::template store<VEC>(p, orow * p.ldo, c, o, nt);
+    R::template store<VEC>(p, orow * p.ldo, c, o);
 }
 
 __device__ __forceinline__ int64_t xcd_block(const SpmmArgs &p) {
@@ -445,6 +499,7 @@
     int rc = bind_csr(g, m, p, s);
     if (rc != GNX_OK) return rc;
     if (m.n_rows == 0) return GNX_OK;
+    g->last_hint_hot = 0;
     g->last_kernel = pick(p);
     GNX_HIP(hipGetLastError());
     return GNX_OK;
diff --git a/gnn-tf_amd/csrc/gnx_spmm_eval.h b/gnn-tf_amd/csrc/gnx_spmm_eval.h
--- a/gnn-tf_amd/csrc/gnx_spmm_eval.h
+++ b/gnn-tf_amd/csrc/gnx_spmm_eval.h
@@ -3,7 +3,7 @@
 
 namespace {
 
-template <typename R, int VEC, int U, int WPB>
+template <typename R, int VEC, int U, int WPB, bool HINT = false>
 __global__ __launch_bounds__(64 * WPB) void k_spmm_wave(const typename R::Args p) {
     const int lane = threadIdx.x & 63;
     const int wib = __builtin_amdgcn_readfirstlane((int)(threadIdx.x >> 6));
@@ -19,12 +19,12 @@
         float acc[VEC];
 #pragma unroll
         for (int v = 0; v < VEC; ++v) acc[v] = 0.f;
-        wave_accumulate<R, VEC, U>(p.colidx, p.vals, R::X(p), p.ldx, beg, end, active ? c : 0, lane, acc, (tune & 4) != 0);
-        epilogue_store<R, VEC>(p, row, c, active, acc, (tune & 2) != 0);
-    }
-}
-
-template <typename R, int VEC, int G, int U, bool PIPE>
+        wave_accumulate<R, VEC, U, false, false, false, HINT>(p.colidx, p.vals, R::X(p), p.ldx, beg, end, active ? c : 0, lane, acc);
+        epilogue_store<R, VEC>(p, row, c, active, acc);
+    }
+}
+
+template <typename R, int VEC, int G, int U, bool PIPE, bool HINT = false>
 __device__ __forceinline__ void group_rows(const typename R::Args &p, int64_t block) {
     constexpr int RPB = 256 / G;
     const int sub = threadIdx.x % G;
@@ -40,7 +40,30 @@
         float acc[VEC];
 #pragma unroll
         for (int v = 0; v < VEC; ++v) acc[v] = 0.f;
-        if (PIPE) {
+        if constexpr (HINT) {
+            static_assert(VEC == 4 && !PIPE && std::is_same_v<typename R::Elem, float>, "hinted gathers: f32 rows, 16 bytes per lane");
+            for (int64_t e = beg; e < end; e += U) {
+                int j[U];
+                float w[U];
+                f32x4 x[U];
+#pragma unroll
+                for (int u = 0; u < U; ++u) {
+                    const bool ok = e + u < end;
+                    j[u] = ok ? p.colidx[e + u] : HINT_NONE;
+                    w[u] = ok ? p.vals[e + u] : 0.f;
+                }
+#pragma unroll
+                for (int u = 0; u < U; ++u) {
+                    x[u] = f32x4{0.f, 0.f, 0.f, 0.f};
+                    gather16_hinted(x[u], Xc + (int64_t)hint_col(j[u]) * p.ldx, j[u]);
+                }
+                gather_wait<U>(x);
+#pragma unroll
+                for (int u = 0; u < U; ++u)
+#pragma unroll
+                    for (int v = 0; v < VEC; ++v) acc[v] = fmaf(w[u], x[u][v], acc[v]);
+            }
+        } else if (PIPE) {
             int jn[U];
             float wn[U];
 #pragma unroll
@@ -141,13 +164,13 @@
     }
 }
 
-template <typename R, int VEC, int G, int U, bool PIPE>
+template <typename R, int VEC, int G, int U, bool PIPE, bool HINT = false>
 __global__ __launch_bounds__(256) void k_spmm_group(const typename R::Args p) {
     if (G <= 8) group_rows_coop<R, VEC, G, 4>(p, xcd_block(p));
-    else group_rows<R, VEC, G, U, PIPE>(p, xcd_block(p));
-}
-
-template <typename R, int VEC, int U>
+    else group_rows<R, VEC, G, U, PIPE, HINT>(p, xcd_block(p));
+}
+
+template <typename R, int VEC, int U, bool HINT = false>
 __global__ __launch_bounds__(256) void k_spmm_long_partial(const typename R::Args p) {
     const int lane = threadIdx.x & 63;
     const int wib = __builtin_amdgcn_readfirstlane((int)(threadIdx.x >> 6));
@@ -160,12 +183,12 @@
         float acc[VEC];
 #pragma unroll
         for (int v = 0; v < VEC; ++v) acc[v] = 0.f;
-        wave_accumulate<R, VEC, U>(p.colidx, p.vals, R::X(p), p.ldx, beg, end, active ? c : 0, lane, acc);
+        wave_accumulate<R, VEC, U, false, false, false, HINT>(p.colidx, p.vals, R::X(p), p.ldx, beg, end, active ? c : 0, lane, acc);
         if (active) vstore<VEC>(p.partial + chunk * (int64_t)p.C + c, acc);
     }
 }
 
-template <typename R, int VEC, int G, int U>
+template <typename R, int VEC, int G, int U, bool HINT = false>
 __device__ __forceinline__ void long_chunks_group(const typename R::Args &p, int64_t block) {
     constexpr int NS = 64 / G;
     const int lane = threadIdx.x & 63;
@@ -181,6 +204,29 @@
 #pragma unroll
     for (int v = 0; v < VEC; ++v) acc[v] = 0.f;
     for (int64_t e = beg + sub; e < end; e += (int64_t)NS * U) {
+        if constexpr (HINT) {
+            static_assert(VEC == 4 && std::is_same_v<typename R::Elem, float>, "hinted gathers: f32 rows, 16 bytes per lane");
+            int j[U];
+            float w[U];
+            f32x4 x[U];
+#pragma unroll
+            for (int u = 0; u < U; ++u) {
+                const int64_t eu = e + (int64_t)u * NS;
+                j[u] = eu < end ? p.colidx[eu] : HINT_NONE;
+                w[u] = eu < end ? p.vals[eu] : 0.f;
+            }
+#pragma unroll
+            for (int u = 0; u < U; ++u) {
+                x[u] = f32x4{0.f, 0.f, 0.f, 0.f};
+                gather16_hinted(x[u], Xc + (int64_t)hint_col(j[u]) * p.ldx, j[u]);
+            }
+            gather_wait<U>(x);
+#pragma unroll
+            for (int u = 0; u < U; ++u)
+#pragma unroll
+                for (int v = 0; v < VEC; ++v) acc[v] = fmaf(w[u], x[u][v], acc[v]);
+            continue;
+        }
         float x[U][VEC];
         float w[U];
 #pragma unroll
@@ -208,19 +254,19 @@
     if (sub == 0 && active) vstore<VEC>(p.partial + chunk * (int64_t)p.C + c, acc);
 }
 
-template <typename R, int VEC, int G, int U>
+template <typename R, int VEC, int G, int U, bool HINT = false>
 __global__ __launch_bounds__(256) void k_spmm_long_partial_group(const typename R::Args p) {
-    long_chunks_group<R, VEC, G, U>(p, blockIdx.x);
-}
-
-template <typename R, int VEC, int G>
+    long_chunks_group<R, VEC, G, U, HINT>(p, blockIdx.x);
+}
+
+template <typename R, int VEC, int G, bool HINT = false>
 __global__ __launch_bounds__(256) void k_spmm_group_and_chunks(const typename R::Args p, int chunk_blocks) {
-    if ((int)blockIdx.x < chunk_blocks) long_chunks_group<R, VEC, G, 4>(p, blockIdx.x);
+    if ((int)blockIdx.x < chunk_blocks) long_chunks_group<R, VEC, G, 4, HINT>(p, blockIdx.x);
     else if (G <= 8) group_rows_coop<R, VEC, G, 4>(p, (int64_t)blockIdx.x - chunk_blocks);
-    else group_rows<R, VEC, G, 4, false>(p, (int64_t)blockIdx.x - chunk_blocks);
-}
-
-template <typename R, int VEC>
+    else group_rows<R, VEC, G, 4, false, HINT>(p, (int64_t)blockIdx.x - chunk_blocks);
+}
+
+template <typename R, int VEC, bool HINT = false>
 RowClass launch_rows(const typename R::Args &p0, hipStream_t s) {
     typename R::Args p = p0;
     const int lanes = (p.C + VEC - 1) / VEC;
@@ -231,8 +277,8 @@
     if (trim) trim_empty_rows(p, lanes);
     if (p.n_rows == 0) return ROWS_NONE;
     if (lanes > 32) {
-        if (p.C <= 64 * VEC) GNX_ROW_PIECES((k_spmm_wave<R, VEC, 8, 8>), 8, 512);
-        else                 GNX_ROW_PIECES((k_spmm_wave<R, VEC, 8, 4>), 4, 256);
+        if (p.C <= 64 * VEC) GNX_ROW_PIECES((k_spmm_wave<R, VEC, 8, 8, HINT>), 8, 512);
+        else                 GNX_ROW_PIECES((k_spmm_wave<R, VEC, 8, 4, HINT>), 4, 256);
         return ROWS_WAVE;
     }
     return with_group<false>(lanes, [&](auto G) {
@@ -244,37 +290,38 @@
             }
         }
 #endif
-        GNX_ROW_PIECES((k_spmm_group<R, VEC, G(), 4, false>), 256 / G(), 256);
+        GNX_ROW_PIECES((k_spmm_group<R, VEC, G(), 4, false, HINT && G() >= 16>), 256 / G(), 256);
     });
 }
 
-template <typename R, int VEC>
+template <typename R, int VEC, bool HINT = false>
 RowClass launch_rows_and_chunks(const typename R::Args &p, hipStream_t s) {
     const int lanes = (p.C + VEC - 1) / VEC;
     if (lanes > 32 || p.n_long == 0 || (p.n_rows >= SMALL_ROWS && !(p.tune & 65536)) || ((p.tune >> 8) & 3) != 0 || (p.tune & 4096)) return ROWS_NONE;
     const unsigned cb = blocks_for(p.n_chunks, 4);
     const RowClass rows = with_group<true>(lanes, [&](auto G) {
-        hipLaunchKernelGGL((k_spmm_group_and_chunks<R, VEC, G()>), dim3(cb + blocks_for(p.n_rows, 256 / G())), dim3(256), 0, s, p, (int)cb);
+        hipLaunchKernelGGL((k_spmm_group_and_chunks<R, VEC, G(), HINT && G() >= 16>), dim3(cb + blocks_for(p.n_rows, 256 / G())), dim3(256), 0, s, p, (int)cb);
     });
     GNX_LAUNCH((k_spmm_long_reduce<R, VEC>), blocks_for(p.n_long, 4), p);
     return rows;
 }
 
-template <typename R, int VEC>
+template <typename R, int VEC, bool HINT = false>
 void launch_long(const typename R::Args &p, hipStream_t s) {
     const int lanes = (p.C + VEC - 1) / VEC;
-    if (lanes > 32) GNX_LAUNCH((k_spmm_long_partial<R, VEC, 8>), blocks_for(p.n_chunks, 4), p);
-    else with_group<true>(lanes, [&](auto G) { GNX_LAUNCH((k_spmm_long_partial_group<R, VEC, G(), 4>), blocks_for(p.n_chunks, 4), p); });
+    if (lanes > 32) GNX_LAUNCH((k_spmm_long_partial<R, VEC, 8, HINT>), blocks_for(p.n_chunks, 4), p);
+    else with_group<true>(lanes, [&](auto G) { GNX_LAUNCH((k_spmm_long_partial_group<R, VEC, G(), 4, HINT && G() >= 16>), blocks_for(p.n_chunks, 4), p); });
     GNX_LAUNCH((k_spmm_long_reduce<R, VEC>), blocks_for(p.n_long, 4), p);
 }
 
-template <typename R>
+template <typename R, bool HINT = false>
 const char *launch_eval(const typename R::Args &p, hipStream_t s) {
     return with_vec<R>(R::vec(p), [&](auto V) {
-        RowClass rows = launch_rows_and_chunks<R, V()>(p, s);
+        constexpr bool H = HINT && V() == 4;
+        RowClass rows = launch_rows_and_chunks<R, V(), H>(p, s);
         if (rows != ROWS_NONE) return kernel_name<R>(rows, MODE_EVAL, HUBS_CHUNKS);
-        rows = launch_rows<R, V()>(p, s);
-        if (p.n_long > 0) launch_long<R, V()>(p, s);
+        rows = launch_rows<R, V(), H>(p, s);
+        if (p.n_long > 0) launch_long<R, V(), H>(p, s);
         return kernel_name<R>(rows, MODE_EVAL, p.n_long > 0 ? HUBS_LONG : HUBS_NONE);
     });
 }
diff --git a/gnn-tf_amd/gnntf/_native.py b/gnn-tf_amd/gnntf/_native.py
--- a/gnn-tf_amd/gnntf/_native.py
+++ b/gnn-tf_amd/gnntf/_native.py
@@ -12,7 +12,7 @@
 EYE = {"none": 0, "before": 1, "after": 2}
 ACT_NONE, ACT_RELU, ACT_SKIP_EMPTY = 0, 1, 256
 HALO_ALL, HALO_PULL, HALO_PUSH = 0, 1, 2
-RESERVE_TRANSPOSED, RESERVE_K_LOOP, RESERVE_TRAIN_GATHER = 1, 2, 4
+RESERVE_TRANSPOSED, RESERVE_K_LOOP, RESERVE_TRAIN_GATHER, RESERVE_GATHER_HINTS = 1, 2, 4, 8
 ORD_X, ORD_OUT = 1, 2
 
 SIGNATURES = {
@@ -30,6 +30,8 @@
     "gnx_graph_reserve": (c_int, [c_void_p, c_int64, c_int, c_void_p]),
     "gnx_graph_enable_entry_dropout": (c_int, [c_void_p, c_void_p]),
     "gnx_graph_set_row_window": (c_int, [c_void_p, c_int64, c_void_p]),
+    "gnx_graph_set_gather_hints": (c_int, [c_void_p, c_int64, c_void_p]),
+    "gnx_graph_gather_hints": (c_int, [c_void_p, POINTER(c_void_p), POINTER(c_int64), POINTER(c_int64)]),
     "gnx_graph_set_dropout_counter": (c_int, [c_void_p, c_void_p]),
     "gnx_graph_set_block": (c_int, [c_void_p, c_int64, c_int64, c_void_p, c_void_p]),
     "gnx_graph_colsum": (c_int, [c_void_p, c_float, c_uint64, c_uint64, c_void_p, c_void_p]),
diff --git a/gnn-tf_amd/gnntf/sparse.py b/gnn-tf_amd/gnntf/sparse.py
--- a/gnn-tf_amd/gnntf/sparse.py
+++ b/gnn-tf_amd/gnntf/sparse.py
@@ -116,9 +116,9 @@
     def last_kernel(self) -> str:
         return (nat.lib().gnx_graph_last_kernel(self._h) or b"").decode()
 
-    def reserve(self, C, transposed=False, k_loop=False, train_gather=False):
+    def reserve(self, C, transposed=False, k_loop=False, train_gather=False, gather_hints=False):
         flags = ((nat.RESERVE_TRANSPOSED if transposed else 0) | (nat.RESERVE_K_LOOP if k_loop else 0)
-                 | (nat.RESERVE_TRAIN_GATHER if train_gather else 0))
+                 | (nat.RESERVE_TRAIN_GATHER if train_gather else 0) | (nat.RESERVE_GATHER_HINTS if gather_hints else 0))
         with nat.on_device(self.device):
             nat.check(nat.lib().gnx_graph_reserve(self._h, int(C), flags, nat.current_stream()))
 
@@ -127,6 +127,24 @@
         with nat.on_device(self.device):
             nat.check(nat.lib().gnx_graph_gather_order(self._h, byref(order), byref(rank)))
             return tuple(torch.as_tensor(_BorrowedInt32(p.value, self.n_rows), device=self.device).clone() for p in (order, rank))
+
+    def set_gather_hints(self, hot_rows=-1):
+        with nat.on_device(self.device):
+            nat.check(nat.lib().gnx_graph_set_gather_hints(self._h, int(hot_rows), nat.current_stream()))
+
+    def gather_hints(self):
+        cols, hot = c_void_p(), c_int64()
+        with nat.on_device(self.device):
+            nat.check(nat.lib().gnx_graph_gather_hints(self._h, byref(cols), byref(hot), None))
+            if not cols.value:
+                return None, 0
+            torch.cuda.current_stream().synchronize()
+            return torch.as_tensor(_BorrowedInt32(cols.value, self.nnz), device=self.device).clone(), hot.value
+
+    def last_launch_hot_rows(self) -> int:
+        last = c_int64()
+        nat.check(nat.lib().gnx_graph_gather_hints(self._h, None, None, byref(last)))
+        return last.value
 
     def set_row_window(self, window_rows):
         with nat.on_device(self.device):
diff --git a/include/gnx.h b/include/gnx.h
--- a/include/gnx.h
+++ b/include/gnx.h
@@ -41,8 +41,11 @@
 int gnx_graph_normalize(gnx_graph_t g, int normalized, int add_eye, float dropout_p, uint64_t seed,
                         uint64_t stream_id, float *d_vals_out, float *d_diag_out, void *stream);
 
-enum { GNX_RESERVE_TRANSPOSED = 1, GNX_RESERVE_K_LOOP = 2, GNX_RESERVE_TRAIN_GATHER = 4 };
+enum { GNX_RESERVE_TRANSPOSED = 1, GNX_RESERVE_K_LOOP = 2, GNX_RESERVE_TRAIN_GATHER = 4, GNX_RESERVE_GATHER_HINTS = 8 };
 int gnx_graph_reserve(gnx_graph_t g, int64_t C, int flags, void *stream);
+
+int gnx_graph_set_gather_hints(gnx_graph_t g, int64_t hot_rows, void *stream);
+int gnx_graph_gather_hints(gnx_graph_t g, const int32_t **d_hint_cols, int64_t *hot_rows, int64_t *last_launch_hot_rows);
 
 int gnx_graph_enable_entry_dropout(gnx_graph_t g, void *stream);
 
```

Measured after the change: 13.88 billion edges/s, median of 6. 1.07x the previous value.
